# geloescht/mxnet-maintenance

Hardware: AMD Instinct MI355X
Metric: images/sec (whole node) ResNet-50 fp16 batch 256/GPU at 1/2/4/8 MI355X (higher is better)
Workload: dtype fp16; 1 GPU; model=ResNet-50 v1b, global_batch=256, per_gpu_batch=256, image_size=224, parallelism=dp1, layout=NHWC, optimizer=mp-SGD momentum 0.9, lr 0.1 (linear warm-up 40 steps), hip_graph=True, deterministic=True

## Files before the change

mxnet_maintenance_amd/_state.py:

```python
import threading


class _State(threading.local):
    def __init__(self):
        super().__init__()
        self.recording = False
        self.training = False
        self.np_shape = False
        self.np_array = False
        self.tape_leaves = {}


STATE = _State()

DIRECT_GRAD = [0]


def is_recording():
    return STATE.recording


def is_training():
    return STATE.training

GRAPH_RNG = [None]


GRAD_TOUCHED = set()
```

mxnet_maintenance_amd/autograd.py:

```python
from contextlib import contextmanager


import torch

from . import _state
from .base import MXNetError

__all__ = ['record', 'pause', 'train_mode', 'predict_mode', 'is_recording', 'is_training',
           'set_recording', 'set_training', 'mark_variables', 'backward', 'grad', 'Function',
           'get_symbol']


def set_recording(is_recording):
    prev = _state.STATE.recording
    _state.STATE.recording = bool(is_recording)
    return prev


def set_training(train_mode):
    prev = _state.STATE.training
    _state.STATE.training = bool(train_mode)
    return prev


# ... 105 lines not shown
            continue
        if not getattr(t, '_mxamd_touch_hook', False):
            _add_touch_hook(v, t)
        gbuf = v._grad._data
        if t.grad is not gbuf:
            t.grad = gbuf
        if v._grad_req == 'write':
            a = v._arena
            if a is not None and a.all_write:
                arenas.setdefault(id(a), (a, []))[1].append(gbuf)
            else:
                zero.append(gbuf)
    with torch.no_grad():
        for a, bufs in arenas.values():
            if len(bufs) == len(a.params):
                a.g.zero_()
            else:
                zero.extend(bufs)
        if zero:
            torch._foreach_zero_(zero)


def _finish_leaves(leaves):
    touched = _state.GRAD_TOUCHED
    for v in leaves:
        t = v._data
        if v._grad is None:
            continue
        g = t.grad
        if g is not None and g is not v._grad._data:
            v._grad._data = g
            t.grad = g
        if id(v) in touched or not getattr(t, '_mxamd_touch_hook', False):
            v._fresh_grad = True
        else:
            _state.STATE.tape_leaves.setdefault(id(v), v)
    touched.clear()


def _head_grad(g, t):
    if g.shape == t.shape:
        return g
    if g.numel() == t.numel() or (g.numel() > t.numel() and g.dim() == t.dim()
                                  and g.shape[1:] == t.shape[1:]):
        return g.reshape(-1)[:t.numel()].reshape(t.shape)
    try:
        return g.expand(t.shape)
    except RuntimeError:
        pass
    raise MXNetError(f'head gradient of shape {tuple(g.shape)} does not match output shape {tuple(t.shape)}')


def backward(heads, head_grads=None, retain_graph=False, train_mode=True, create_graph=False):
    from .ndarray.ndarray import NDArray
    if isinstance(heads, NDArray):
        heads = [heads]
    if head_grads is not None and isinstance(head_grads, NDArray):
        head_grads = [head_grads]
    tensors, grads = [], []
    for i, h in enumerate(heads):
        t = h._data
        if not t.requires_grad:
            continue
        tensors.append(t)
        hg = None if head_grads is None else head_grads[i]
        grads.append(torch.ones_like(t) if hg is None else _head_grad(hg._data.to(t.dtype), t))
    if not tensors and heads and all(getattr(h, '_recorded', False) for h in heads):
        _zero_marked_grads()
        return
    if not tensors:
        raise MXNetError('Cannot differentiate node because it is not in a computational graph. '
                         'You need to set is_recording to true or use autograd.record() to save '
                         'computational graphs for backward.')
    for h in heads:
        if getattr(getattr(h, '_data', None), _RELEASED_ATTR, False):
            raise MXNetError('Check failed: the graph of this output was already freed by a backward pass '
                             'without retain_graph=True; record it again or pass retain_graph=True')
    if not (retain_graph or create_graph):
        for h in heads:
            if getattr(h, '_data', None) is not None and h._data.grad_fn is not None:
                setattr(h._data, _RELEASED_ATTR, True)
    leaves = _collect_leaves(retain_graph)
    _prepare_leaves(leaves)
    prev_train = set_training(train_mode)
    prev_rec = set_recording(False)
    direct = not create_graph
    if direct:
        _state.DIRECT_GRAD[0] += 1
    try:
        with torch.enable_grad() if create_graph else torch.no_grad():
            torch.autograd.backward(tensors, grads, retain_graph=retain_graph or create_graph,
                                    create_graph=create_graph)
    finally:
        set_training(prev_train)
        set_recording(prev_rec)
        if direct:
            _state.DIRECT_GRAD[0] -= 1
    _finish_leaves(leaves)


def grad(heads, variables, head_grads=None, retain_graph=None, create_graph=False, train_mode=True):
    from .ndarray.ndarray import NDArray
    if isinstance(heads, NDArray):
        heads = [heads]
    if isinstance(variables, NDArray):
        variables = [variables]
    if head_grads is not None and isinstance(head_grads, NDArray):
        head_grads = [head_grads]
    hts = [h._data for h in heads]
    if head_grads is None:
        hgs = [torch.ones_like(h) for h in hts]
    else:
        hgs = [torch.ones_like(h) if g is None else g._data for h, g in zip(hts, head_grads)]
    if retain_graph is None:
        retain_graph = create_graph
    live = [(h, g) for h, g in zip(hts, hgs) if h.requires_grad]
    gs = [None] * len(variables)
    if live:
        prev_train = set_training(train_mode)
        prev_rec = set_recording(create_graph)
        try:
            with torch.enable_grad():
                gs = torch.autograd.grad([h for h, _ in live], [v._data for v in variables],
                                         grad_outputs=[g for _, g in live], retain_graph=retain_graph,
                                         create_graph=create_graph, allow_unused=True)
        finally:
            set_training(prev_train)
            set_recording(prev_rec)

    def dense(g, v):
        if g is None or g._is_zerotensor():
            return torch.zeros_like(v._data)
        return g
    return [NDArray(dense(g, v)) for g, v in zip(gs, variables)]


def get_symbol(x):
    sym = getattr(x, '_symbol', None)
    if isinstance(sym, tuple):
        block, i = sym
        return block._recorded_symbols()[i]
    if sym is not None:
        return sym
    if getattr(x, '_hist', None) is None:
        raise MXNetError('get_symbol: the array was not produced by a recorded operator')
    from .symbol.symbol import _op_func, var
    memo, nvars = {}, [0]

    def build(a):
        key = id(a)
        if key in memo:
            return memo[key]
        h = getattr(a, '_hist', None)
        if h is None:
            s = var('var%d' % nvars[0])
            nvars[0] += 1
        else:
            (opname, attrs, ins), i = h
            kw = {k: v for k, v in attrs.items() if v is not None}
            node = _op_func(opname)(*[build(b) for b in ins if b is not None], **kw)
            s = node[i] if len(node.list_outputs()) > 1 else node
        memo[key] = s
        return s
    return build(x)


# ... 57 lines not shown
```

mxnet_maintenance_amd/executor.py:

```python
import os

import numpy as np
import torch

from . import _state
from . import profiler as _profiler
from .ops import amp_dispatch as _amp
from .base import MXNetError, AsyncOpError
from .ops import registry


def _call_monitor(cb, name, arr):
    from .base import _HANDLES, NDArrayHandle
    key = id(arr)
    _HANDLES[key] = arr
    try:
        cb(name, NDArrayHandle(key))
    finally:
        _HANDLES.pop(key, None)


class GraphProgram:

    def __init__(self, sym):
        from .symbol.symbol import _aux_var_ids
        order = sym._topo()
        self.symbol = sym
        slot = {}
        nslots = 0
        self.var_names = []
        self.var_slots = []
        aux = _aux_var_ids(order)
        self.arg_names = []
        self.aux_names = []
        for n in order:
            if n.op is None:
                slot[(id(n), 0)] = nslots
                self.var_names.append(n.name)
                self.var_slots.append(nslots)
                (self.aux_names if id(n) in aux else self.arg_names).append(n.name)
                nslots += 1
        self.steps = []
        for n in order:
            if n.op is None:
                continue
            op = n.opdef()
            parsed = dict(n.parsed())
            k = op.get_num_outputs(parsed)
            outs = []
            for i in range(k):
                slot[(id(n), i)] = nslots
                outs.append(nslots)
                nslots += 1
            ins = [slot[(id(a), j)] for a, j in n.inputs]
            self.steps.append((op.fn, ins, parsed, outs, n.name, op.name))
        self.out_slots = [slot[(id(n), j)] for n, j in sym._outputs]
        self.nslots = nslots
        self._var_of_slot = {s: n for n, s in zip(self.var_names, self.var_slots)}
        self.name_to_slot = dict(zip(self.var_names, self.var_slots))

    _POSITIONAL_INPUTS = ('SoftmaxActivation', 'Activation')

    @staticmethod
    def _input_names(opname, attrs, n):
        op = registry.get(opname)
        if op.name in GraphProgram._POSITIONAL_INPUTS:
            return ['input%d' % j for j in range(n)]
        names = op.get_arg_names(attrs) + op.get_aux_names(attrs)
        return [names[j] if j < len(names) else 'input%d' % j for j in range(n)]

    def run(self, feed, monitor=None, monitor_all=False, record=None, int_dtypes=None):
        vals = [None] * self.nslots
        for name, s in self.name_to_slot.items():
            vals[s] = feed.get(name)
        islot = {}
        if int_dtypes:
            islot = {self.name_to_slot[n]: d for n, d in int_dtypes.items() if n in self.name_to_slot}
        self.failure = None
        sched = self._stream_sched(vals) if _GRAPH_STREAMS > 1 else None
        try:
            for si, (fn, ins, attrs, outs, name, opname) in enumerate(self.steps):
                args = [vals[i] for i in ins]
                if sched is not None:
                    sched.before(si, args)
                if _amp.active:
                    args = _amp.cast_inputs(opname, args, attrs)
                if record is not None:
                    record.append((name, args))
                if monitor is not None and monitor_all:
                    argn = self._input_names(opname, attrs, len(args))
                    for j, a in enumerate(args):
                        if a is None:
                            continue
                        var = self._var_of_slot.get(ins[j])
                        if var is not None:
                            monitor(var, a)
                        monitor('%s_%s' % (name, argn[j]), a)
                try:
                    if (islot and any(i in islot for i in ins)) or (attrs.get('dtype') is not None and
                                                                     _int_dtype_attr(attrs) and torch.is_grad_enabled()):
                        r = self._run_shadow(fn, args, attrs, ins, outs, islot, opname)
                    elif _profiler.active_symbolic:
                        with _profiler.op_span(_profiler.current_scope() + opname, symbolic=True):
                            r = fn(*args, **attrs)
                    else:
                        r = fn(*args, **attrs)
                except AsyncOpError as e:
                    from .ndarray.register import _placeholder
                    if self.failure is None:
                        self.failure = AsyncOpError('Error in operator %s (%s): %s' % (name, opname, e))
                    r = _placeholder(attrs, [])
                except MXNetError:
                    if self.failure is None:
                        raise
                    from .ndarray.register import _placeholder
                    r = _placeholder(attrs, [])
                except (RuntimeError, IndexError) as e:
                    if self.failure is not None:
                        from .ndarray.register import _placeholder
                        r = _placeholder(attrs, [])
                    else:
                        raise MXNetError('Error in operator %s (%s): %s' % (name, opname, e)) from e
                if sched is not None:
                    sched.after(si)
                if len(outs) == 1:
                    vals[outs[0]] = r[0] if isinstance(r, (tuple, list)) else r
                else:
                    for o, t in zip(outs, r):
                        vals[o] = t
                if monitor is not None:
                    op = registry.get(opname)
                    onames = op.output_names or (['output'] if len(outs) == 1 else
                                                 ['output%d' % k for k in range(len(outs))])
                    for o, on in zip(outs, onames):
                        if vals[o] is not None:
                            monitor('%s_%s' % (name, on), vals[o])
        finally:
            if sched is not None:
                torch.cuda.set_stream(sched.main)
        self.out_idts = [islot.get(s) for s in self.out_slots] if islot else None
        if sched is not None:
            sched.finish([vals[s] for s in self.out_slots])
        return [vals[s] for s in self.out_slots]

    def _stream_plan(self, nstreams):
        producer = {}
        for i, st in enumerate(self.steps):
            for o in st[3]:
                producer[o] = i
        n = len(self.steps)
        stream_of = [0] * n
        tail = [-1] * nstreams
        waits = [()] * n
        need_ev = set()
        rr = 1
        for i, (_fn, ins, _attrs, _outs, _name, opname) in enumerate(self.steps):
            prods = sorted({producer[x] for x in ins if x in producer})
            cands = prods or [-1]
            live = [stream_of[p] if p >= 0 else 0 for p in cands if tail[stream_of[p] if p >= 0 else 0] == p]
            choice = min(live) if live else None
            if choice is None:
                if opname in _BRANCH_OPS and nstreams > 1:
                    choice = rr
                    rr = 1 + rr % (nstreams - 1)
                else:
                    choice = stream_of[prods[-1]] if prods else 0
            stream_of[i] = choice
            tail[choice] = i
            w = tuple(p for p in prods if stream_of[p] != choice)
            waits[i] = w
            need_ev.update(w)
        return stream_of, waits, need_ev

    def _stream_sched(self, vals):
        dev = next((v.device for v in vals if isinstance(v, torch.Tensor) and v.is_cuda), None)
        if dev is None or torch.cuda.is_current_stream_capturing() and not _GRAPH_STREAMS_CAPTURE:
            return None
        plan = getattr(self, '_splan', None)
        if plan is None:
            plan = self._splan = self._stream_plan(_GRAPH_STREAMS)
        if max(plan[0], default=0) == 0:
            return None
        return _StreamSched(plan, dev)
    @staticmethod
    def _run_shadow(fn, args, attrs, ins, outs, islot, opname=None):
        from .ndarray.register import _merge_shadow, INT_ZERO_GRAD
        true_args = [a.detach().to(islot[i]) if (i in islot and a is not None) else a for a, i in zip(args, ins)]
        with torch.no_grad():
            res_t = fn(*true_args, **attrs)
        multi = isinstance(res_t, (tuple, list))
        if not torch.is_grad_enabled() or not any(a is not None and a.requires_grad for a in args) or \
                opname in INT_ZERO_GRAD:
            for o in outs:
                islot.pop(o, None)
            return res_t
        kw_f = dict(attrs, dtype='float64') if _int_dtype_attr(attrs) else attrs
        res_f = fn(*args, **kw_f)
        pairs = [_merge_shadow(f, t) for f, t in zip(res_f, res_t)] if multi else [_merge_shadow(res_f, res_t)]
        for o, (_, d) in zip(outs, pairs):
            if d is not None:
                islot[o] = d
            else:
                islot.pop(o, None)
        return [p[0] for p in pairs] if multi else pairs[0][0]


_GRAPH_STREAMS = int(os.environ.get('MXNET_GRAPH_STREAMS', '1') or 1)
_GRAPH_STREAMS_CAPTURE = os.environ.get('MXNET_GRAPH_STREAMS_CAPTURE', '0') == '1'
_BRANCH_OPS = frozenset(('Convolution', 'Deconvolution', 'FullyConnected', '_contrib_DeformableConvolution',
                         '_contrib_ModulatedDeformableConvolution', 'Pooling', 'dot', 'batch_dot', '_npi_matmul',
                         'RNN', '_FusedOp'))
_SIDE_STREAMS = {}


def _side_streams(dev, n):
    lst = _SIDE_STREAMS.get(dev)
    if lst is None or len(lst) < n:
        lst = _SIDE_STREAMS[dev] = [torch.cuda.Stream(device=dev) for _ in range(n)]
    return lst


class _StreamSched:
# ... 436 lines not shown
```

mxnet_maintenance_amd/gluon/model_zoo/vision/resnet.py:

```python
from ... import nn
from ...block import HybridBlock
from ...nn.basic_layers import _BatchNorm
from ....context import cpu

__all__ = ['ResNetV1', 'ResNetV2', 'BasicBlockV1', 'BasicBlockV2', 'BottleneckV1', 'BottleneckV2',
           'BottleneckV1b', 'resnet18_v1', 'resnet34_v1', 'resnet50_v1', 'resnet101_v1', 'resnet152_v1',
           'resnet18_v2', 'resnet34_v2', 'resnet50_v2', 'resnet101_v2', 'resnet152_v2', 'resnet50_v1b',
           'resnet101_v1b', 'resnet152_v1b', 'resnet18_v1b', 'resnet34_v1b', 'get_resnet']


def _bn_axis(layout):
    return 3 if layout == 'NHWC' else 1


def _conv(channels, k, stride, pad, in_channels, layout, use_bias=False):
    return nn.Conv2D(channels, kernel_size=k, strides=stride, padding=pad, use_bias=use_bias,
                     in_channels=in_channels, layout=layout)


def _bn(layout, relu=False, fuse=False, **kw):
    if relu and fuse:
        return nn.BatchNormReLU(axis=_bn_axis(layout), **kw)
    return nn.BatchNorm(axis=_bn_axis(layout), **kw)


class _StemBNReLUPool(nn.BatchNormReLU):

    def hybrid_forward(self, F, x, gamma, beta, running_mean, running_var):
        return F.contrib.BatchNormReLUMaxPool(x, gamma, beta, running_mean, running_var, name='fwd',
                                              kernel=(3, 3), stride=(2, 2), pad=(1, 1), **self._kwargs)


def _stem_tail(features, layout, fuse):
    if fuse and layout == 'NHWC':
        features.add(_StemBNReLUPool(axis=_bn_axis(layout)))
        return
    features.add(_bn(layout, True, fuse))
    if not fuse:
        features.add(nn.Activation('relu'))
    features.add(nn.MaxPool2D(3, 2, 1, layout=layout))


class _ResidualTail(_BatchNorm):

    def __init__(self, layout, fuse, **kwargs):
        super().__init__(axis=_bn_axis(layout), **kwargs)
        self._fuse_add = fuse

    def _alias(self):
        return 'batchnorm'

    def hybrid_forward(self, F, x, shortcut, gamma, beta, running_mean, running_var):
        if self._fuse_add:
            return F.contrib.BatchNormAddReLU(x, shortcut, gamma, beta, running_mean, running_var, name='fwd',
                                              **self._kwargs)
        return F.BatchNorm(x, gamma, beta, running_mean, running_var, name='fwd', **self._kwargs)


def _finish(F, tail, out, shortcut):
    y = tail(out, shortcut)
    return y if tail._fuse_add else F.Activation(y + shortcut, act_type='relu')


class BasicBlockV1(HybridBlock):

    def __init__(self, channels, stride, downsample=False, in_channels=0, layout='NCHW', fuse=False, **kwargs):
        super().__init__(**kwargs)
        self.body = nn.HybridSequential(prefix='')
        self.body.add(_conv(channels, 3, stride, 1, in_channels, layout),
                      _bn(layout, True, fuse))
        if not fuse:
            self.body.add(nn.Activation('relu'))
        self.body.add(_conv(channels, 3, 1, 1, channels, layout))
        self.tail = _ResidualTail(layout, fuse)
        self.downsample = None
        if downsample:
            self.downsample = nn.HybridSequential(prefix='')
            self.downsample.add(_conv(channels, 1, stride, 0, in_channels, layout), _bn(layout))

    def hybrid_forward(self, F, x):
        shortcut = self.downsample(x) if self.downsample is not None else x
        return _finish(F, self.tail, self.body(x), shortcut)


class BottleneckV1(HybridBlock):

    def __init__(self, channels, stride, downsample=False, in_channels=0, layout='NCHW', fuse=False,
                 stride_on_3x3=False, **kwargs):
        super().__init__(**kwargs)
        mid = channels // 4
        s1, s3 = (1, stride) if stride_on_3x3 else (stride, 1)
        self.body = nn.HybridSequential(prefix='')
        self.body.add(_conv(mid, 1, s1, 0, in_channels, layout), _bn(layout, True, fuse))
        if not fuse:
            self.body.add(nn.Activation('relu'))
        self.body.add(_conv(mid, 3, s3, 1, mid, layout), _bn(layout, True, fuse))
        if not fuse:
            self.body.add(nn.Activation('relu'))
        self.body.add(_conv(channels, 1, 1, 0, mid, layout))
        self.tail = _ResidualTail(layout, fuse)
        self.downsample = None
        if downsample:
            self.downsample = nn.HybridSequential(prefix='')
            self.downsample.add(_conv(channels, 1, stride, 0, in_channels, layout), _bn(layout))
        self._tee = fuse and s1 == 1 and layout == 'NHWC'
        if self._tee:
            self.body[0]._tee = True

    def hybrid_forward(self, F, x):
        if self._tee:
            blocks = list(self.body._children.values())
            out, passthrough = blocks[0](x)
            for b in blocks[1:]:
                out = b(out)
            shortcut = self.downsample(passthrough) if self.downsample is not None else passthrough
            return _finish(F, self.tail, out, shortcut)
        shortcut = self.downsample(x) if self.downsample is not None else x
        return _finish(F, self.tail, self.body(x), shortcut)


class BottleneckV1b(BottleneckV1):
    def __init__(self, channels, stride, downsample=False, in_channels=0, layout='NCHW', fuse=False, **kwargs):
        super().__init__(channels, stride, downsample, in_channels, layout, fuse, stride_on_3x3=True, **kwargs)


class BasicBlockV2(HybridBlock):

    def __init__(self, channels, stride, downsample=False, in_channels=0, layout='NCHW', fuse=False, **kwargs):
        super().__init__(**kwargs)
        self.bn1 = _bn(layout, True, fuse)
        self.conv1 = _conv(channels, 3, stride, 1, in_channels, layout)
        self.bn2 = _bn(layout, True, fuse)
        self.conv2 = _conv(channels, 3, 1, 1, channels, layout)
        self._fused = fuse
        self.downsample = _conv(channels, 1, stride, 0, in_channels, layout) if downsample else None

    def _act(self, F, x, bn):
        x = bn(x)
        return x if self._fused else F.Activation(x, act_type='relu')

    def hybrid_forward(self, F, x):
        shortcut = x
        x = self._act(F, x, self.bn1)
        if self.downsample is not None:
            shortcut = self.downsample(x)
        x = self.conv1(x)
        x = self.conv2(self._act(F, x, self.bn2))
        return x + shortcut


class BottleneckV2(HybridBlock):

    def __init__(self, channels, stride, downsample=False, in_channels=0, layout='NCHW', fuse=False, **kwargs):
        super().__init__(**kwargs)
        mid = channels // 4
        self.bn1 = _bn(layout, True, fuse)
        self.conv1 = _conv(mid, 1, 1, 0, 0, layout)
        self.bn2 = _bn(layout, True, fuse)
        self.conv2 = _conv(mid, 3, stride, 1, mid, layout)
        self.bn3 = _bn(layout, True, fuse)
        self.conv3 = _conv(channels, 1, 1, 0, 0, layout)
        self._fused = fuse
        self.downsample = _conv(channels, 1, stride, 0, in_channels, layout) if downsample else None

    def _act(self, F, x, bn):
        x = bn(x)
        return x if self._fused else F.Activation(x, act_type='relu')

    def hybrid_forward(self, F, x):
        shortcut = x
        x = self._act(F, x, self.bn1)
        if self.downsample is not None:
            shortcut = self.downsample(x)
        x = self.conv1(x)
        x = self.conv2(self._act(F, x, self.bn2))
        x = self.conv3(self._act(F, x, self.bn3))
        return x + shortcut


class _ResNetBase(HybridBlock):
    def _stage(self, block, n, channels, stride, index, in_channels, layout, fuse):
        stage = nn.HybridSequential(prefix='stage%d_' % index)
        with stage.name_scope():
            stage.add(block(channels, stride, channels != in_channels, in_channels=in_channels, layout=layout,
                            fuse=fuse, prefix=''))
            for _ in range(n - 1):
                stage.add(block(channels, 1, False, in_channels=channels, layout=layout, fuse=fuse, prefix=''))
        return stage


class ResNetV1(_ResNetBase):

    def __init__(self, block, layers, channels, classes=1000, thumbnail=False, layout='NCHW', fuse=False,
                 **kwargs):
        super().__init__(**kwargs)
        assert len(layers) == len(channels) - 1
        self._layout = layout
        with self.name_scope():
            self.features = nn.HybridSequential(prefix='')
            if thumbnail:
                self.features.add(_conv(channels[0], 3, 1, 1, 0, layout))
            else:
                self.features.add(_conv(channels[0], 7, 2, 3, 0, layout))
                _stem_tail(self.features, layout, fuse)
            for i, n in enumerate(layers):
                self.features.add(self._stage(block, n, channels[i + 1], 1 if i == 0 else 2, i + 1,
                                              channels[i], layout, fuse))
            self.features.add(nn.GlobalAvgPool2D(layout=layout))
            self.output = nn.Dense(classes, in_units=channels[-1])

    def hybrid_forward(self, F, x):
        return self.output(self.features(x))


class ResNetV2(_ResNetBase):

    def __init__(self, block, layers, channels, classes=1000, thumbnail=False, layout='NCHW', fuse=False,
                 **kwargs):
        super().__init__(**kwargs)
        assert len(layers) == len(channels) - 1
        with self.name_scope():
            self.features = nn.HybridSequential(prefix='')
            self.features.add(nn.BatchNorm(scale=False, center=False, axis=_bn_axis(layout)))
            if thumbnail:
                self.features.add(_conv(channels[0], 3, 1, 1, 0, layout))
            else:
                self.features.add(_conv(channels[0], 7, 2, 3, 0, layout))
                _stem_tail(self.features, layout, fuse)
            in_channels = channels[0]
            for i, n in enumerate(layers):
                self.features.add(self._stage(block, n, channels[i + 1], 1 if i == 0 else 2, i + 1,
                                              in_channels, layout, fuse))
                in_channels = channels[i + 1]
            self.features.add(_bn(layout, True, fuse))
            if not fuse:
                self.features.add(nn.Activation('relu'))
            self.features.add(nn.GlobalAvgPool2D(layout=layout))
            self.features.add(nn.Flatten())
            self.output = nn.Dense(classes, in_units=in_channels)

    def hybrid_forward(self, F, x):
        return self.output(self.features(x))


resnet_spec = {18: ('basic_block', [2, 2, 2, 2], [64, 64, 128, 256, 512]),
               34: ('basic_block', [3, 4, 6, 3], [64, 64, 128, 256, 512]),
               50: ('bottle_neck', [3, 4, 6, 3], [64, 256, 512, 1024, 2048]),
               101: ('bottle_neck', [3, 4, 23, 3], [64, 256, 512, 1024, 2048]),
               152: ('bottle_neck', [3, 8, 36, 3], [64, 256, 512, 1024, 2048])}
resnet_net_versions = [ResNetV1, ResNetV2]
resnet_block_versions = [{'basic_block': BasicBlockV1, 'bottle_neck': BottleneckV1},
                         {'basic_block': BasicBlockV2, 'bottle_neck': BottleneckV2}]


def get_resnet(version, num_layers, pretrained=False, ctx=cpu(), root='~/.mxnet/models', v1b=False, **kwargs):
    assert num_layers in resnet_spec, 'Invalid number of layers: %d. Options are %s' % (
        num_layers, str(resnet_spec.keys()))
    block_type, layers, channels = resnet_spec[num_layers]
    assert 1 <= version <= 2, 'Invalid resnet version: %d. Options are 1 and 2.' % version
    resnet_class = resnet_net_versions[version - 1]
    block_class = resnet_block_versions[version - 1][block_type]
    if v1b and block_type == 'bottle_neck':
        block_class = BottleneckV1b
    net = resnet_class(block_class, layers, channels, **kwargs)
    if pretrained:
        from ..model_store import get_model_file
        net.load_parameters(get_model_file('resnet%d_v%d' % (num_layers, version), root=root), ctx=ctx)
    return net


def resnet18_v1(**kwargs):
    return get_resnet(1, 18, **kwargs)


def resnet34_v1(**kwargs):
    return get_resnet(1, 34, **kwargs)


def resnet50_v1(**kwargs):
    return get_resnet(1, 50, **kwargs)


def resnet101_v1(**kwargs):
    return get_resnet(1, 101, **kwargs)


def resnet152_v1(**kwargs):
    return get_resnet(1, 152, **kwargs)


# ... 39 lines not shown
```

mxnet_maintenance_amd/ndarray/ndarray.py:

```python
import ctypes

import numpy as np
import torch

from .. import _state
from .. import engine as _engine
from ..base import (MXNetError, numeric_types, integer_types, torch_dtype, np_dtype,
                    dtype_name)
from ..context import Context, current_context, context_from_torch

def _shares_storage(a, b):
    try:
        return a.untyped_storage().data_ptr() == b.untyped_storage().data_ptr()
    except RuntimeError:
        return False


_STORAGE_TYPE_UNDEFINED = -1
_STORAGE_TYPE_DEFAULT = 0
_STORAGE_TYPE_ROW_SPARSE = 1
_STORAGE_TYPE_CSR = 2
_STORAGE_TYPE_STR_TO_ID = {'undefined': _STORAGE_TYPE_UNDEFINED, 'default': _STORAGE_TYPE_DEFAULT,
                           'row_sparse': _STORAGE_TYPE_ROW_SPARSE, 'csr': _STORAGE_TYPE_CSR}
_STORAGE_TYPE_ID_TO_STR = {v: k for k, v in _STORAGE_TYPE_STR_TO_ID.items()}
# ... 125 lines not shown
        shape_info = 'x'.join(str(x) for x in self.shape)
        return '\n%s\n<%s %s @%s>' % (str(self.asnumpy()), self.__class__.__name__, shape_info, self.context)

    def __str__(self):
        return self.__repr__()

    def __hash__(self):
        return id(self)

    def __bool__(self):
        n = self.size
        if n == 0:
            return False
        if n == 1:
            return bool(self._data.reshape(-1)[0].item())
        raise ValueError('The truth value of an NDArray with multiple elements is ambiguous.')

    __nonzero__ = __bool__

    def __float__(self):
        return float(self.asscalar())

    def __int__(self):
        return int(self.asscalar())

    def __index__(self):
        return int(self.asscalar())

    def __iter__(self):
        if self.ndim == 1:
            for i in range(self.shape[0]):
                yield self[i]
        else:
            box = getattr(self, '_exc', None)
            for i in range(self.shape[0]):
                v = NDArray(self._data[i])
                if box is not None:
                    v._exc = box
                yield v

    def __array__(self, dtype=None, copy=None):
        a = self.asnumpy()
        return a.astype(dtype) if dtype is not None else a

    def __getstate__(self):
        return {'data': self.asnumpy(), 'ctx': self.context}

    def __setstate__(self, state):
        if 'handle' in state:
            from .utils import _Reader, _read_array
            self._data = _read_array(_Reader(bytes(state['handle'])))._data
        else:
            self._data = torch.from_numpy(np.ascontiguousarray(state['data']))
        self._grad = None
        self._grad_req = None
        self._stype = 'default'
        self._fresh_grad = False
        self._arena = None

    def __reduce__(self):
        return (_rebuild, (self.asnumpy(),))

    def _rethrow(self):
        box = getattr(self, '_exc', None)
        if box is not None and box[0] is not None:
            from .. import engine
            engine.rethrow(box)

    def wait_to_read(self):
        _engine.join_workers()
        var = getattr(self, '_engine_var', None)
        if var is not None:
            from .. import engine
            engine.wait_for_var(var)
        if self._data.is_cuda:
            torch.cuda.current_stream(self._data.device).synchronize()
        self._rethrow()

    wait_to_write = wait_to_read

    def asnumpy(self):
        _engine.join_workers()
        self._rethrow()
        t = self._data.detach()
        idt = getattr(self, '_idt', None)
        if idt is not None:
            t = t.to(idt)
        if t.dtype == torch.bfloat16:
            t = t.float()
        return t.cpu().numpy().copy() if t.device.type == 'cpu' else t.cpu().numpy()

    def asscalar(self):
        if self.size != 1:
            raise ValueError('The current array is not a scalar')
        return self.asnumpy().reshape(-1)[0]

    def item(self):
        return self.asscalar()

    def tolist(self):
        return self.asnumpy().tolist()

    def astype(self, dtype, copy=True):
        td = torch_dtype(dtype)
        if not copy and td == self._data.dtype:
            return self
        return _invoke_unary(lambda t: t.to(td) if t.dtype != td else t.clone(), self)

    def copy(self):
        if self._stype != 'default' and type(self) is NDArray:
            from . import sparse
            cls = sparse.RowSparseNDArray if self._stype == 'row_sparse' else sparse.CSRNDArray
            return _tag_host_ctx(cls(self._data.detach().clone()), getattr(self, '_host_ctx', None))
        return _invoke_unary(lambda t: t.clone(), self)

    def __copy__(self):
        return self.copy()

    def __deepcopy__(self, memo):
        return NDArray(self._data.detach().clone())

    def copyto(self, other):
        _engine.join_workers()
        if isinstance(other, NDArray):
            if other is self:
                return other
            src = self._data.detach() if not _state.STATE.recording else self._data
            if other.shape != self.shape:
                raise MXNetError('copyto: shape mismatch %s vs %s' % (self.shape, other.shape))
            if _engine_copy(src, other._data.device) and other._data.is_contiguous() \
                    and other._data.dtype == src.dtype:
                from .. import engine
                _, other._engine_var = engine.host_to_device(src, other._data.device, out=other._data,
                                                             var=getattr(other, '_engine_var', None), name='copyto')
            else:
                with torch.no_grad():
                    other._data.copy_(src)
            _share_failure(self, other)
            return other
        if isinstance(other, Context):
            if _engine_copy(self._data, other.torch_device):
                return _share_failure(self, _async_upload(self._data, other))
            return _share_failure(self, _tag_host_ctx(NDArray(self._data.to(other.torch_device, copy=True)), other))
        raise TypeError('copyto does not support type ' + str(type(other)))

    def as_in_context(self, context):
        if self.context == context:
            return self
        _engine.join_workers()
        if context.device_typeid == 3:
            t = self._data.detach().cpu()
            if torch.cuda.is_available():
                return NDArray(t.pin_memory())
            out = NDArray(t.clone() if t.data_ptr() == self._data.data_ptr() else t)
            out._host_ctx = context
            return out
        if _engine_copy(self._data, context.torch_device):
            return _share_failure(self, _async_upload(self._data, context))
        return _tag_host_ctx(_invoke_unary(lambda t: t.to(context.torch_device), self), context)

    as_in_ctx = as_in_context

    def to_device(self, device):
        return self.as_in_context(device)

    def detach(self):
# ... 850 lines not shown
```

mxnet_maintenance_amd/ndarray/register.py:

```python
import contextlib

import sys

import torch

from .. import _state
from .. import engine as _engine
from .. import profiler as _profiler
from ..ops import amp_dispatch as _amp
from ..base import MXNetError, AsyncOpError
from ..ops import registry
from .ndarray import NDArray

_SKIP_KW = ('name', 'attr', 'out')
_NULL_CTX = contextlib.nullcontext()
_NP_CLS = [None]


def _np_wrap(inputs, outs):
    cls = _NP_CLS[0]
    if cls is None:
        return outs
    has_inputs = any(x is not None for x in inputs)
    if (_state.STATE.np_array and not has_inputs) or any(x is not None and x.__class__ is cls for x in inputs):
# ... 72 lines not shown

def _failed_input(inputs):
    for x in inputs:
        box = getattr(x, '_exc', None) if x is not None else None
        if box is not None and box[0] is not None:
            return box
    return None


_SAMPLER_NAMES = frozenset(('_npi_normal', '_npi_uniform', '_npi_gamma', '_npi_exponential', '_npi_multinomial',
                            '_shuffle', '_npi_bernoulli', '_npi_sampler', '_npi_uniform_like', '_npi_normal_like',
                            '_npi_choice', '_npi_shuffle', '_npi_laplace', '_npi_logistic', '_npi_gumbel',
                            '_npi_pareto', '_npi_power', '_npi_rayleigh', '_npi_weibull', '_npi_chisquare',
                            '_npi_f', '_npi_beta', '_npi_lognormal', '_npi_poisson'))


def _is_sampler(name):
    return name.startswith(('_random_', '_sample_', '_npi_random', 'random_', 'sample_')) or name in _SAMPLER_NAMES


def _placeholder(attrs, inputs):
    from ..base import torch_dtype
    shape = attrs.get('shape') or attrs.get('size') or (1,)
    shape = (shape,) if isinstance(shape, int) else tuple(shape)
    dt = attrs.get('dtype')
    try:
        td = torch_dtype(dt if dt not in (None, 'None') else 'float32')
    except Exception:
        td = torch.float32
    ctx = attrs.get('ctx')
    dev = getattr(ctx, 'torch_device', None)
    if dev is None:
        dev = next((x._data.device for x in inputs if x is not None), torch.device('cpu'))
    return torch.zeros(shape, dtype=td, device=dev)


def _int_dtype_attr(attrs):
    dt = attrs.get('dtype')
    return dt is not None and str(dt).replace('torch.', '').startswith(('int', 'uint', 'bool'))


def _shadowed(arrays, attrs=None):
    if any(x is not None and getattr(x, '_idt', None) is not None for x in arrays):
        return True
    return attrs is not None and _state.STATE.recording and _int_dtype_attr(attrs) and \
        any(x is not None and x._data.requires_grad for x in arrays)


def _true_inputs(arrays):
    return [None if x is None else (x._data.detach().to(x._idt) if getattr(x, '_idt', None) is not None
                                    else x._data) for x in arrays]


def _merge_shadow(res_f, res_t):
    if not isinstance(res_f, torch.Tensor) or not res_f.requires_grad or not res_f.is_floating_point():
        return res_t, None
    if res_t.is_floating_point() or res_t.is_complex():
        return res_f.to(res_t.dtype) + (res_t - res_f.to(res_t.dtype)).detach(), None
    return res_f + (res_t.to(res_f.dtype) - res_f).detach(), res_t.dtype


INT_ZERO_GRAD = frozenset(('_npi_mod', '_npi_mod_scalar', '_npi_fmod', '_npi_fmod_scalar', '_mod', 'broadcast_mod',
                           '_mod_scalar', '_rmod_scalar'))


def _run_shadow(fn, inputs, kw, opname=None):
    with torch.no_grad():
        res_t = fn(*_true_inputs(inputs), **kw)
    if not _state.STATE.recording or opname in INT_ZERO_GRAD:
        return res_t, None
    kw_f = kw
    if _int_dtype_attr(kw):
        kw_f = dict(kw, dtype='float64')
    res_f = _run(fn, [None if x is None else x._data for x in inputs], kw_f)
    if isinstance(res_t, (tuple, list)):
        pairs = [_merge_shadow(f, t) for f, t in zip(res_f, res_t)]
        return type(res_t)(p[0] for p in pairs), [p[1] for p in pairs]
    r, idt = _merge_shadow(res_f, res_t)
    return r, idt


def invoke(op, inputs, attrs, out=None):
    tin = [None if x is None else x._data for x in inputs]
    if _engine._JOIN_HOOKS and not _engine._workers.depth:
        _engine.run_join_hooks()
    _note_leaves(inputs)
    if _amp.active:
        tin = _amp.cast_inputs(op.name, tin, attrs)
    if op.name in _BN_OPS:
        _check_storage(op.name, [getattr(x, 'stype', 'default') for x in inputs], attrs)
    box = _failed_input(inputs)
    sampler = _is_sampler(op.name)
    if sampler and box is None:
        from .. import engine
        box = engine.rng_failure()
    idts = None
    ws_sid = ws_stream = None
    sctx = _NULL_CTX
    if _engine.GPU_WORKERS > 1 and not _engine._workers.depth:
        ws_sid, ws_stream = _engine.op_stream(tin)
        if ws_stream is not None:
            sctx = torch.cuda.stream(ws_stream)
            _engine._workers.depth += 1
    try:
        with sctx:
            if _shadowed(inputs, attrs) and not _amp.active:
                res, idts = _run_shadow(op.fn, inputs, attrs, op.name)
            elif _profiler.active_imperative:
                with _profiler.op_span(_profiler.current_scope() + op.name):
                    res = _run(op.fn, tin, attrs)
            else:
                res = _run(op.fn, tin, attrs)
    except AsyncOpError as e:
        from .. import engine
        if box is None:
            box = engine.record_failure(e)
        if sampler:
            engine.set_rng_failure(box)
        res = _placeholder(attrs, inputs)
    except MXNetError:
        if box is None:
            raise
        res = _placeholder(attrs, inputs)
    except (RuntimeError, IndexError) as e:
        if isinstance(e, IndexError):
            from ..base import MXNetIndexError
            raise MXNetIndexError('Error in operator %s: %s' % (op.name, e)) from e
        raise MXNetError('Error in operator %s: %s' % (op.name, e)) from e
    finally:
        if ws_stream is not None:
            _engine._workers.depth -= 1
            if sys.exc_info()[0] is not None:
                _engine._workers.pending.pop()
    nvis = op.get_num_visible_outputs(attrs)
    if isinstance(res, (tuple, list)):
        outs = [NDArray(r) for r in res[:nvis]]
    else:
        outs = [NDArray(res)]
    if ws_sid is not None:
        _engine.op_done([o._data for o in outs], ws_sid)
    st = _kept_stype(op.name, inputs, attrs) if out is None else None
    if st is not None and not _state.STATE.recording:
        from . import sparse
        outs = [sparse.cast_storage(o, st) for o in outs]
    _np_wrap(inputs, outs)
    if idts is not None:
        for o, d in zip(outs, idts if isinstance(idts, list) else [idts]):
            if d is not None:
                o._idt = d
    if _state.STATE.recording:
        hist = (op.name, attrs, list(inputs))
        for i, o in enumerate(outs):
            o._recorded = True
            o._hist = (hist, i)
    if _profiler.active_memory and out is None:
        for o in outs:
            _profiler.memory_alloc(o)
    if box is not None:
        for o in outs:
            o._exc = box
    hctx = attrs.get('ctx') if 'ctx' in attrs else next(
        (x._host_ctx for x in inputs if x is not None and getattr(x, '_host_ctx', None) is not None), None)
    if hctx is not None:
        from .ndarray import _tag_host_ctx
        for o in outs:
            _tag_host_ctx(o, hctx)
# ... 101 lines not shown
```

mxnet_maintenance_amd/ops/hip_ops.py:

```python
import os

import torch
import torch.nn.functional as F

from ..base import MXNetError
from . import kernels as _K

_ALLOW_FALLBACK = os.environ.get('MXAMD_ALLOW_TORCH_FALLBACK', '0') == '1'


def _acc(t):
    return t if t.dtype == torch.float64 else t.float()


def _use_hip(t):
    if not t.is_cuda:
        return False
    if _K.available():
        return _K.enabled()
    if _ALLOW_FALLBACK:
        return False
    raise MXNetError('HIP kernel extension not loaded on a GPU device: %s' % _K.load_error())


def _nd_to_ncx(x):
    nd = x.dim()
    return x.permute(0, nd - 1, *range(1, nd - 1))


def _ncx_to_nd(x):
    nd = x.dim()
    return x.permute(0, *range(2, nd), 1)



def linear(data, weight, bias):
    if _use_hip(data) and _K.gemm_ok(data, weight):
        return _K.Linear.apply(data, weight, bias)
    if data.dim() == 2:
        return F.linear(data, weight, bias)
    return F.linear(data, weight, bias)


def embedding(data, weight):
    if _use_hip(weight) and _K.embedding_ok(data, weight):
        return _K.Embedding.apply(data, weight)
    return None


def _as_nhwc_view(t):
    v = t.permute(0, 2, 3, 1)
    return v if v.is_contiguous() else v.contiguous()


def _nchw_on_hip(data):
    return (data.dim() == 4 and data.dtype in (torch.float16, torch.bfloat16) and _use_hip(data)
            and _NCHW_VIA_NHWC)


_NCHW_VIA_NHWC = os.environ.get('MXAMD_NCHW_VIA_NHWC', '1') == '1'


def _nhwc_weight(w):
    if w.shape[2] == 1 and w.shape[3] == 1 and w.is_contiguous():
        return w.view(w.shape[0], 1, 1, w.shape[1])
    return w.permute(0, 2, 3, 1).contiguous()


def conv(data, weight, bias, stride, pad, dilate, groups, channel_last):
    nsp = data.dim() - 2
    if groups > 1 and nsp == 2 and _use_hip(data):
        from .conv_dw import dw_ok, ConvDwNHWC
        xl = data if channel_last else (_as_nhwc_view(data) if _nchw_on_hip(data) else None)
        if xl is not None and dw_ok(xl, weight, groups, dilate):
            rs = tuple(weight.shape[1:3]) if channel_last else tuple(weight.shape[2:4])
            y = ConvDwNHWC.apply(xl, weight, bias, rs, tuple(stride), tuple(pad), tuple(dilate))
            return y if channel_last else y.permute(0, 3, 1, 2)
    if not channel_last and nsp == 2 and _nchw_on_hip(data):
        xl = _as_nhwc_view(data)
        wl = _nhwc_weight(weight)
        if _K.conv_ok(xl, wl, stride, pad, dilate, groups):
            if _K.kpad_ok(xl, wl):
                return _K.conv_kpad(xl, wl, bias, stride, pad, dilate).permute(0, 3, 1, 2)
            return _K.ConvNHWC.apply(xl, wl, bias, tuple(stride), tuple(pad), tuple(dilate)).permute(0, 3, 1, 2)
    if channel_last and _use_hip(data) and _K.conv_ok(data, weight, stride, pad, dilate, groups):
        if _K.kpad_ok(data, weight):
            return _K.conv_kpad(data, weight, bias, stride, pad, dilate)
        return _K.ConvNHWC.apply(data, weight, bias, tuple(stride), tuple(pad), tuple(dilate))
    if nsp == 2 and groups == 1 and _use_hip(data) and tuple(dilate) != (1, 1):
        xl = data if channel_last else (_as_nhwc_view(data) if _nchw_on_hip(data) else None)
        if xl is not None:
            wl = weight if channel_last else _nhwc_weight(weight)
            if _K.dil_ok(xl, wl, dilate):
                y = _K.ConvDilNHWC.apply(xl, wl, bias, tuple(stride), tuple(pad), tuple(dilate))
                return y if channel_last else y.permute(0, 3, 1, 2)
    if _use_hip(data):
        from . import conv_gen
        y = conv_gen.conv(data, weight, bias, tuple(stride), tuple(pad), tuple(dilate), groups, channel_last)
        if y is not None:
            return y
    if channel_last:
        x = _nd_to_ncx(data)
        w = _nd_to_ncx(weight)
    else:
        x, w = data, weight
    fn = {1: F.conv1d, 2: F.conv2d, 3: F.conv3d}[nsp]
    y = fn(x, w, bias, stride=stride, padding=pad, dilation=dilate, groups=groups)
    return _ncx_to_nd(y) if channel_last else y


def conv_tee(data, weight, inplace_grad=False):
    if _use_hip(data) and hasattr(_K, 'ConvTeeNHWC') and _K.conv_tee_ok(data, weight):
        return _K.ConvTeeNHWC.apply(data, weight, bool(inplace_grad))
    return conv(data, weight, None, (1, 1), (0, 0), (1, 1), 1, True), data



def batch_norm_relu_maxpool(data, gamma, beta, moving_mean, moving_var, eps, momentum, fix_gamma, training,
                            axis, kernel, stride, pad, invstd_out=False):
    nd = data.dim()
    if (nd == 4 and axis % nd == 3 and _use_hip(data) and _K.bnrelu_pool_ok(data, kernel, stride, pad)):
        g = torch.ones_like(gamma) if fix_gamma else gamma
        return _K.BatchNormNHWC.apply(data, g, beta, None, eps, training, True, moving_mean, moving_var, momentum,
                                      invstd_out, (tuple(kernel), tuple(stride), tuple(pad)))
    out, m, v = batch_norm(data, gamma, beta, moving_mean, moving_var, eps, momentum, fix_gamma, training, axis,
                           'relu', invstd_out=invstd_out)
    return pool(out, 'max', tuple(kernel), tuple(stride), tuple(pad), 'valid', True, axis % nd == nd - 1), m, v


def batch_norm(data, gamma, beta, moving_mean, moving_var, eps, momentum, fix_gamma, training,
               axis, act_type, addend=None, invstd_out=False):
    nd = data.dim()
    axis = axis % nd
    channel_last = (axis == nd - 1) and nd > 2
    g = torch.ones_like(gamma) if fix_gamma else gamma
    if axis == 1 and _nchw_on_hip(data) and data.permute(0, 2, 3, 1).is_contiguous():
        xl = data.permute(0, 2, 3, 1)
        al = _as_nhwc_view(addend) if addend is not None else None
        if _K.bn_ok(xl):
            out, m, v = _K.BatchNormNHWC.apply(xl, g, beta, al, eps, training, act_type == 'relu',
                                                moving_mean, moving_var, momentum, invstd_out)
            return out.permute(0, 3, 1, 2), m, v
    if channel_last and _use_hip(data) and _K.bn_ok(data):
        return _K.BatchNormNHWC.apply(data, g, beta, addend, eps, training, act_type == 'relu',
                                      moving_mean, moving_var, momentum, invstd_out)
    if channel_last:
        x = _nd_to_ncx(data)
    elif axis != 1:
        others = [i for i in range(nd) if i != axis]
        perm = [others[0], axis] + others[1:]
        x = data.permute(*perm)
    else:
        x = data
    if training:
        out, smean, sinvstd = torch.ops.aten.native_batch_norm(x, g, beta, None, None, True, 0.0, eps)
        with torch.no_grad():
            var = (1.0 / (sinvstd.float() ** 2) - eps).clamp_(min=0.0) if sinvstd.numel() else sinvstd
            moving_mean.mul_(momentum).add_(smean.detach().to(moving_mean.dtype), alpha=1 - momentum)
            moving_var.mul_(momentum).add_(var.to(moving_var.dtype), alpha=1 - momentum)
        mean_out, var_out = smean, (sinvstd if invstd_out else var)
    else:
        out = F.batch_norm(x, moving_mean, moving_var, g, beta, False, 0.0, eps)
        mean_out, var_out = moving_mean, moving_var
    if channel_last:
        out = _ncx_to_nd(out)
    elif axis != 1:
        inv = [0] * nd
        others = [i for i in range(nd) if i != axis]
        perm = [others[0], axis] + others[1:]
        for i, p in enumerate(perm):
            inv[p] = i
        out = out.permute(*inv)
    if addend is not None:
        out = out + addend
    if act_type == 'relu':
        out = torch.relu(out)
    return out, mean_out, var_out



def global_pool(data, pool_type, channel_last):
    nsp = data.dim() - 2
    if not channel_last and pool_type == 'avg' and _nchw_on_hip(data) and data.permute(0, 2, 3, 1).is_contiguous():
        xl = data.permute(0, 2, 3, 1)
        if _K.gap_ok(xl):
            return _K.GlobalAvgPoolNHWC.apply(xl).permute(0, 3, 1, 2)
    if channel_last:
        if _use_hip(data) and nsp == 2 and pool_type == 'avg' and _K.gap_ok(data):
            return _K.GlobalAvgPoolNHWC.apply(data)
        dims = tuple(range(1, 1 + nsp))
    else:
        dims = tuple(range(2, 2 + nsp))
    if pool_type == 'max':
        return torch.amax(data, dim=dims, keepdim=True)
    if pool_type == 'sum':
        return torch.sum(data, dim=dims, keepdim=True)
    if pool_type == 'lp':
        return torch.sqrt(torch.sum(data * data, dim=dims, keepdim=True))
    return torch.mean(data, dim=dims, keepdim=True)


def _pool_out(n, k, s, p, conv):
    if conv == 'full':
        return int(-(-(n + 2 * p - k) // s)) + 1
    return (n + 2 * p - k) // s + 1


def pool(data, pool_type, kernel, stride, pad, convention, count_include_pad, channel_last, p_value=None):
    nsp = data.dim() - 2
    if not channel_last and nsp == 2 and pool_type in ('max', 'avg') and convention != 'same' \
            and _nchw_on_hip(data) and data.permute(0, 2, 3, 1).is_contiguous():
        xl = data.permute(0, 2, 3, 1)
        if _K.pool_ok(xl, kernel, stride, pad):
            return _K.PoolNHWC.apply(xl, pool_type, tuple(kernel), tuple(stride), tuple(pad),
                                     convention == 'full', bool(count_include_pad)).permute(0, 3, 1, 2)
    if channel_last and _use_hip(data) and nsp == 2 and pool_type in ('max', 'avg') \
            and _K.pool_ok(data, kernel, stride, pad):
        return _K.PoolNHWC.apply(data, pool_type, tuple(kernel), tuple(stride), tuple(pad),
                                 convention == 'full', bool(count_include_pad))
    x = _nd_to_ncx(data) if channel_last else data
    if channel_last and x.is_cuda and pool_type != 'max':
        x = x.contiguous()
    ceil = convention == 'full'
    pad_r = list(pad)
    if convention == 'same':
        ceil = False
        for i in range(nsp):
            n = x.shape[2 + i]
# ... 93 lines not shown
```

mxnet_maintenance_amd/ops/kernel_fns.py:

```python
import os

import torch

from . import kernels as _K
from .. import _state
from ..utils import env as _env

__all__ = ['BatchNormNHWC', 'SoftmaxCE', 'GlobalAvgPoolNHWC', 'flat_sgd']

_DT = {torch.float32: 0, torch.float16: 1, torch.bfloat16: 2}


def _stream():
    return torch.cuda.current_stream().cuda_stream


def _p(t):
    return 0 if t is None else t.data_ptr()


def _f32(t):
    if t.dtype == torch.float32 and t.is_contiguous():
        return t
    m = getattr(t, '_mxamd_master', None)
    if m is not None and m[1] == t._version and m[0].shape == t.shape:
        return m[0]
    return t.float().contiguous()



def bn_ok(x):
    C = x.shape[-1] if x.dim() else 0
    return (x.dtype in _DT and x.dim() >= 2 and x.is_contiguous() and C % 8 == 0
            and x.numel() > 0 and x.data_ptr() % 16 == 0)


def ce_ok(x):
    return x.dim() == 2 and x.dtype in _DT and x.is_contiguous()




def _leaf_grad(t, numel=None, dtype=torch.float32):
    if t is None or _state.DIRECT_GRAD[0] <= 0 or torch.is_grad_enabled() or not t.is_leaf or not t.requires_grad:
        return None
    gb = t.grad
    if gb is None or gb.dtype != dtype or not gb.is_contiguous() or gb.shape != t.shape:
        return None
    if numel is not None and gb.numel() != numel:
        return None
    return gb


_RELU_FROM_X = [True]
_BN_BWD_FUSE = [os.environ.get('MXAMD_BN_BWD_FUSE', '1') != '0']
_BN_TAIL_DS = [os.environ.get('MXAMD_BN_TAIL_DS', '1') != '0']
_BN_POOL_BWD = [True]
_ZEROS = {}


def _zeros_f32(n, dev):
    z = _ZEROS.get((n, dev))
    if z is None:
        z = _ZEROS[(n, dev)] = torch.zeros(n, dtype=torch.float32, device=dev)
    return z


class _BnToken:
    __slots__ = ('lazy',)

    def __init__(self):
        self.lazy = None


class BatchNormNHWC(torch.autograd.Function):

    @staticmethod
    def forward(ctx, x, gamma, beta, addend, eps, training, relu, moving_mean, moving_var, momentum=None,
                invstd_out=False, pool=None):
        lib = _K.lib()
        C = x.shape[-1]
        R = x.numel() // C
        dev = x.device
        g = _f32(gamma)
        b = _f32(beta)
        mm = _f32(moving_mean)
        assert pool is None or (relu and addend is None)
        y = torch.empty_like(x) if pool is None else None
        if addend is not None:
            assert addend.shape == x.shape and addend.dtype == x.dtype
            addend = addend.contiguous()
        ext_nblk = 0
        center = mm
        if training:
            ext = getattr(x, '_mxamd_bn_part', None)
            if ext is not None and ext[0].numel() == 2 * C * ext[1] and ext[0].device == dev:
                part, ext_nblk = ext
                center = _zeros_f32(C, dev)
            else:
                nblk = lib.bn_partials_rows(R, C)
                part = torch.empty(2 * nblk * C, dtype=torch.float32, device=dev)
            stats = torch.empty(5, C, dtype=torch.float32, device=dev)
            mean, invstd, var, scale, shift = stats.unbind(0)
        else:
            part = None
            mean = mm
            invstd = torch.rsqrt(_f32(moving_var) + eps)
            var = _f32(moving_var)
            scale = g * invstd
            shift = b - mean * scale
        upd = (training and momentum is not None and mm is moving_mean and moving_var.dtype == torch.float32
               and moving_var.is_contiguous())
        mask = (torch.empty(x.numel() // 8, dtype=torch.uint8, device=dev)
                if (addend is not None and relu and _RELU_FROM_X[0]) else None)
        lib.bn_nhwc_forward(_DT[x.dtype], x.data_ptr(), _p(addend), _p(y), _p(mask), g.data_ptr(),
                            b.data_ptr(),
                            center.data_ptr(), _p(part), mean.data_ptr(), invstd.data_ptr(), var.data_ptr(),
                            scale.data_ptr(), shift.data_ptr(), R, C, float(eps), int(bool(training)),
                            int(bool(relu)), 0, float(momentum or 0.0), moving_mean.data_ptr() if upd else 0,
                            moving_var.data_ptr() if upd else 0, int(ext_nblk), _stream())
        if training and momentum is not None and not upd:
            with torch.no_grad():
                moving_mean.mul_(momentum).add_(mean.to(moving_mean.dtype), alpha=1 - momentum)
                moving_var.mul_(momentum).add_(var.to(moving_var.dtype), alpha=1 - momentum)
        ctx.pool = None
        if pool is not None:
            (kh, kw), (sh, sw), (ph, pw) = pool
            N, H, W = x.shape[:3]
            Ho, Wo = _pool_out(H, kh, sh, ph, False), _pool_out(W, kw, sw, pw, False)
            y = torch.empty((N, Ho, Wo, C), dtype=x.dtype, device=dev)
            arg = torch.empty((N, Ho, Wo, C), dtype=torch.uint8, device=dev)
            ctx.pool = (N, H, W, C, Ho, Wo, kh, kw, sh, sw, ph, pw, 1)
            lib.pool_nhwc_forward_bnrelu(_DT[x.dtype], x.data_ptr(), y.data_ptr(), arg.data_ptr(), *ctx.pool,
                                         _stream(), scale.data_ptr(), shift.data_ptr())
            mask = arg
        relu_mode = 0 if not relu else (1 if not _RELU_FROM_X[0] else (3 if addend is not None else 2))
        if pool is not None:
            relu_mode = 2
        ctx.save_for_backward(x, y if relu_mode == 1 else mask, g, mean, invstd,
                              scale if relu_mode == 2 else None, shift if relu_mode == 2 else None)
        ctx.cfg = (relu_mode, bool(training), addend is not None, gamma.dtype, beta.dtype)
        ctx.tee_key = getattr(addend, '_mxamd_tee_key', None) if (addend is not None and relu_mode == 3) else None
        ctx.bn_token = None
        if training and relu_mode in (0, 2, 3) and _BN_BWD_FUSE[0] and pool is None:
            ctx.bn_token = _BnToken()
            y._mxamd_bn_src = (x, mean, scale if relu_mode == 2 else None, shift if relu_mode == 2 else None,
                               mask if relu_mode == 3 else None, relu_mode, ctx.bn_token)
        ctx.refs = (gamma, beta)
        ctx.add_src = None
        if relu_mode == 3 and training and _BN_BWD_FUSE[0] and _BN_TAIL_DS[0]:
            src = getattr(addend, '_mxamd_bn_src', None)
            if (src is not None and src[5] == 0 and tuple(src[0].shape) == tuple(x.shape)
                    and src[0].dtype == x.dtype and src[0].is_contiguous()):
                ctx.add_src = src
        third = invstd if (invstd_out and training) else var
        ctx.mark_non_differentiable(mean, third)
        ctx.set_materialize_grads(False)
        return y, mean, third

    @staticmethod
    def backward(ctx, gy, _gm, _gv):
        lib = _K.lib()
        x, y, g, mean, invstd, fscale, fshift = ctx.saved_tensors
        relu_mode, training, has_add, gdt, bdt = ctx.cfg
        gamma_ref, beta_ref = ctx.refs
        if gy is None:
            return (None,) * 12
        gy = gy.contiguous()
        C = x.shape[-1]
        R = x.numel() // C
        dev = x.device
        fused_pool = False
        if ctx.pool is not None:
            fused_pool = (x.dtype in (torch.float16, torch.bfloat16) and 256 % (C // 8) == 0
                          and hasattr(lib, 'bn_pool_backward') and _BN_POOL_BWD[0])
            if not fused_pool:
                gyd = torch.empty_like(x)
                lib.pool_nhwc_backward(_DT[x.dtype], 1, gy.data_ptr(), y.data_ptr(), gyd.data_ptr(), *ctx.pool,
                                       _stream())
                gy, y = gyd, None
        lazy_mask = None
        tok = ctx.bn_token
        if tok is not None and tok.lazy is not None:
            dy_l, mask_l, ver_l = tok.lazy
            tok.lazy = None
            if gy is dy_l and gy._version == ver_l and relu_mode == 0 and not has_add and ctx.pool is None:
                lazy_mask = mask_l
            else:
                gy = (gy - dy_l + _materialize_dz(dy_l, mask_l)).contiguous()
        dx = torch.empty_like(x)
        dz = torch.empty_like(x) if has_add else None
        ext = getattr(gy, '_mxamd_bn_bwd', None)
        ext_nblk = 0
        if (ext is not None and ctx.bn_token is not None and ext[2] is ctx.bn_token
                and ext[3] == gy._version):
            part, ext_nblk = ext[0], ext[1]
        else:
            nblk = lib.bn_partials_rows(R, C)
            part = torch.empty(2 * nblk * C, dtype=torch.float32, device=dev)
        out = torch.empty(5, C, dtype=torch.float32, device=dev)
        need_g, need_b = ctx.needs_input_grad[1], ctx.needs_input_grad[2]
        tg = _leaf_grad(gamma_ref, C) if need_g else None
        tb = _leaf_grad(beta_ref, C) if need_b else None
        direct = tb is not None and (tg is not None or not need_g) and (tg is not None or tb is not None)
        if direct:
            dg_buf = tg if tg is not None else torch.zeros(C, dtype=torch.float32, device=dev)
            dg_ptr, db_ptr, accum = dg_buf.data_ptr(), tb.data_ptr(), 1
        else:
            dg_ptr, db_ptr, accum = out[0].data_ptr(), out[1].data_ptr(), 0
        if fused_pool:
            N_, H_, W_, C_, Ho_, Wo_, kh, kw, sh, sw, ph, pw, _ = ctx.pool
            ppart = torch.empty(2 * lib.bn_pool_bwd_blocks() * C, dtype=torch.float32, device=dev)
            lib.bn_pool_backward(_DT[x.dtype], x.data_ptr(), gy.data_ptr(), y.data_ptr(), dx.data_ptr(), g.data_ptr(),
                                 mean.data_ptr(), invstd.data_ptr(), fscale.data_ptr(), fshift.data_ptr(),
                                 ppart.data_ptr(), dg_ptr, db_ptr, out[2].data_ptr(), N_, H_, W_, C_, Ho_, Wo_, kh, kw,
                                 sh, sw, ph, pw, 0, int(training), accum, _stream())
            if direct:
                return dx, None, None, None, None, None, None, None, None, None, None, None
            return (dx, out[0].to(gdt) if need_g else None, out[1].to(bdt) if need_b else None,
                    None, None, None, None, None, None, None, None, None)
        ymask = y if relu_mode == 3 else None
        y = y if relu_mode == 1 else None
        ds = ctx.add_src if dz is not None else None
        lazy = (dz is not None and ds is None and ymask is not None and ctx.tee_key is not None
                and lazy_shortcut_ok(ctx.tee_key))
        lazy_ds = (dz is not None and ds is not None and ymask is not None and _LAZY_DZ[0]
                   and isinstance(ds[6], _BnToken))
        if lazy or lazy_ds:
            dz = None
        kmode = relu_mode
        if lazy_mask is not None:
            kmode, ymask = 3, lazy_mask
        dkw = {}
        if ds is not None:
            ds_nblk = lib.bn_tail_ds_rows(R, C)
            ds_part = torch.empty(2 * ds_nblk * C, dtype=torch.float32, device=dev)
            dkw = dict(ds_z=ds[0].data_ptr(), ds_mean=ds[1].data_ptr(), ds_part=ds_part.data_ptr())
        lib.bn_nhwc_backward(_DT[x.dtype], x.data_ptr(), gy.data_ptr(), _p(y), _p(ymask), dx.data_ptr(), _p(dz),
                             g.data_ptr(),
                             mean.data_ptr(), invstd.data_ptr(), _p(fscale), _p(fshift), part.data_ptr(), dg_ptr,
                             db_ptr, out[2].data_ptr(), R, C, kmode, 0, int(training), accum, _stream(),
                             ext_nblk, **dkw)
        if ds is not None:
            if lazy_ds:
                gy._mxamd_bn_bwd = (ds_part, ds_nblk, ds[6], gy._version)
                ds[6].lazy = (gy, ymask, gy._version)
                dz = gy
            else:
                dz._mxamd_bn_bwd = (ds_part, ds_nblk, ds[6], dz._version)
        if lazy:
            gy._mxamd_lazy_mask = (ymask, gy._version)
            dz = gy
        if direct:
            dgamma = None
            dbeta = None
        else:
            dgamma = out[0].to(gdt) if need_g else None
            dbeta = out[1].to(bdt) if need_b else None
        return dx, dgamma, dbeta, dz, None, None, None, None, None, None, None, None


def bnrelu_pool_ok(x, kernel, stride, pad):
    return (bn_ok(x) and tuple(kernel) == (3, 3) and pool_ok(x, kernel, stride, pad)
            and x.numel() + 256 * 32 * 256 * 8 < 2 ** 31 and hasattr(_K.lib(), 'pool_nhwc_forward_bnrelu'))


class SoftmaxCE(torch.autograd.Function):

    @staticmethod
    def forward(ctx, logits, label):
        lib = _K.lib()
        N, K = logits.shape
        lab = label.reshape(-1)
        is_int = not lab.is_floating_point()
        lab = lab.to(torch.int64).contiguous() if is_int else lab.float().contiguous()
        loss = torch.empty(N, dtype=torch.float32, device=logits.device)
        lse = torch.empty(N, dtype=torch.float32, device=logits.device)
        lib.softmax_ce_forward(_DT[logits.dtype], int(is_int), logits.data_ptr(), lab.data_ptr(), loss.data_ptr(),
                               lse.data_ptr(), N, K, _stream())
        ctx.save_for_backward(logits, lab, lse)
        ctx.is_int = is_int
        return loss

    @staticmethod
    def backward(ctx, gout):
        lib = _K.lib()
        logits, lab, lse = ctx.saved_tensors
        N, K = logits.shape
        g = gout.float().contiguous()
        dl = torch.empty_like(logits)
        lib.softmax_ce_backward(_DT[logits.dtype], int(ctx.is_int), logits.data_ptr(), lab.data_ptr(),
                                lse.data_ptr(), g.data_ptr(), dl.data_ptr(), N, K, _stream())
        return dl, None


class GlobalAvgPoolNHWC(torch.autograd.Function):
    @staticmethod
    def forward(ctx, x):
        lib = _K.lib()
        x = x.contiguous()
        N, C = x.shape[0], x.shape[-1]
        HW = x.numel() // (N * C)
        y = torch.empty((N,) + (1,) * (x.dim() - 2) + (C,), dtype=x.dtype, device=x.device)
        lib.gap_nhwc_forward(_DT[x.dtype], x.data_ptr(), y.data_ptr(), N, HW, C, _stream())
        ctx.shape = x.shape
        return y

    @staticmethod
    def backward(ctx, gy):
        lib = _K.lib()
        shape = ctx.shape
        N, C = shape[0], shape[-1]
        HW = int(torch.tensor(shape[1:-1]).prod())
        gy = gy.contiguous()
        dx = torch.empty(shape, dtype=gy.dtype, device=gy.device)
        lib.gap_nhwc_backward(_DT[gy.dtype], gy.data_ptr(), dx.data_ptr(), N, HW, C, _stream())
        return dx


def gap_ok(x):
    return x.dtype in _DT and x.is_contiguous() and x.shape[-1] % 8 == 0


class ReluHip(torch.autograd.Function):

    @staticmethod
    def forward(ctx, x):
        x = x.contiguous()
        y = torch.empty_like(x)
        _K.lib().relu_forward(_DT[x.dtype], x.data_ptr(), y.data_ptr(), x.numel(), _stream())
        ctx.save_for_backward(y)
        return y

    @staticmethod
    def backward(ctx, gy):
        y, = ctx.saved_tensors
        gy = gy.contiguous()
        dx = torch.empty_like(y)
        _K.lib().relu_backward(_DT[y.dtype], y.data_ptr(), gy.data_ptr(), dx.data_ptr(), y.numel(), _stream())
        return dx


# ... 622 lines not shown

_FILE_ALGO = {}
_FILE_STATE = {'loaded': False}


def _tuning_file():
    return os.environ.get('MXAMD_AUTOTUNE_FILE', '')


def _load_tuning_file():
    if _FILE_STATE['loaded']:
        return
    _FILE_STATE['loaded'] = True
    path = _tuning_file()
    if path and os.path.exists(path):
        import json
        try:
            with open(path) as f:
                _FILE_ALGO.update(json.load(f))
        except (OSError, ValueError):
            pass


def _save_tuning_file(key, name):
    path = _tuning_file()
    if not path or name is None:
        return
    from ..parallel import dist
    if dist.rank() != 0:
        return
    import json
    _FILE_ALGO[repr(key)] = name
    tmp = path + '.tmp'
    try:
        with open(tmp, 'w') as f:
            json.dump(_FILE_ALGO, f, indent=0, sort_keys=True)
        os.replace(tmp, path)
    except OSError:
        pass


def _select(key, cands, default, timing=None):
    key = _akey(key)
    cands = _det_filter(cands)
    timing = _det_filter(timing)
    _load_tuning_file()
    name = _ALGO.get(key)
    if name is None:
        name = _FILE_ALGO.get(repr(key))
        if name is not None and name in dict(cands):
            _ALGO[key] = name
    if name is None:
        if _AUTOTUNE and not torch.cuda.is_current_stream_capturing() and len(cands) > 1:
            name, out = _time_candidates(timing or cands, key=key)
            _ALGO[key] = name
            _save_tuning_file(key, name)
            return out
        name = default
    table = dict(cands)
    return (table[name] if name in table else cands[0][1])()


_NCU = {}


def _num_cus(dev):
    n = _NCU.get(dev)
    if n is None:
        n = _NCU[dev] = torch.cuda.get_device_properties(dev).multi_processor_count
    return n


def pw_ok(x, kin, nout):
    return (_CONV_HIP and x.is_cuda and x.dtype in (torch.float16, torch.bfloat16) and x.is_contiguous()
            and x.data_ptr() % 16 == 0 and hasattr(_K.lib(), 'conv_pw_stream')
            and bool(_K.lib().conv_pw_stream_ok(int(kin), int(nout))))


def pw_bnb_ok(kin, nout, add, bn_src):
    return (bn_src is not None and int(bn_src[5]) in (2, 3) and hasattr(_K.lib(), 'conv_pw_stream_bnb_ok')
            and bool(_K.lib().conv_pw_stream_bnb_ok(int(kin), int(nout), int(bool(add)), int(bn_src[5]))))


def conv_pw(x, w2, bn_stats=False, addend=None, bn_bwd=None, addend_mask=None):
    C = x.shape[-1]
    K = w2.shape[0]
    M = x.numel() // C
    wt = int(w2.dim() == 2 and w2.stride() == (1, K) and not w2.is_contiguous() and w2.data_ptr() % 16 == 0
             and K % 8 == 0)
    if not wt:
        w2 = w2.contiguous()
    y = torch.empty(x.shape[:-1] + (K,), dtype=x.dtype, device=x.device)
    if addend is not None:
        addend = addend.contiguous()
        if tuple(addend.shape) != tuple(y.shape) or addend.dtype != y.dtype or addend.data_ptr() % 16:
            raise ValueError('conv_pw: addend must match the output (shape, dtype, 16-byte alignment)')
    lib = _K.lib()
    grid = lib.conv_pw_stream_grid(M, C, K, _num_cus(x.device), int(addend is not None or bn_bwd is not None))
    nparts = grid // max(1, lib.conv_pw_stream_slices(C, K))
    part = torch.empty(2 * K * nparts, dtype=torch.float32, device=x.device) if (bn_stats or bn_bwd) else None
    bkw = {}
    if bn_bwd is not None:
        assert not bn_stats, 'conv_pw: forward and backward statistics are exclusive'
        z, bmean, bscale, bshift, bmask, bmode, _token = bn_bwd
        assert z.shape == y.shape and z.dtype == y.dtype and z.is_contiguous() and z.data_ptr() % 16 == 0
        bkw = dict(bn_z=z.data_ptr(), bn_mask=_p(bmask), bn_mean=bmean.data_ptr(), bn_scale=_p(bscale),
                   bn_shift=_p(bshift), bn_mode=int(bmode))
    if addend_mask is not None:
        assert bn_bwd is not None and addend is not None and addend_mask.dtype == torch.uint8
        assert addend_mask.numel() * 8 == addend.numel() and addend_mask.is_contiguous()
        bkw['addend_mask'] = addend_mask.data_ptr()
    lib.conv_pw_stream(_DT[x.dtype], x.data_ptr(), w2.data_ptr(), y.data_ptr(), _zero_page(x.device).data_ptr(), M, C,
                       K, _p(part), grid, _stream(), _p(addend), wt, **bkw)
    if bn_bwd is not None:
        y._mxamd_bn_bwd = (part, nparts, bn_bwd[6], y._version)
    elif part is not None:
        y._mxamd_bn_part = (part, nparts)
    return y


def _fwd_candidates(x, w, stride, pad, bias):
    c = []
    K, R, S, C = w.shape
    if (R == 1 and S == 1 and tuple(stride) == (1, 1) and tuple(pad) == (0, 0) and bias is None
            and pw_ok(x, C, K)):
        c.append(('pw', lambda: conv_pw(x, w.reshape(K, C), bn_stats=bool(_state.STATE.training))))
    if stem_ok(x, w, stride, pad, bias):
        c.append(('stem', lambda: conv_stem_fwd(x, w, pad, bn_stats=bool(_state.STATE.training))))
    if bias is None and halo_ok(x, w, stride, pad):
        c.append(('halo', lambda: conv_halo(x, w, bn_stats=bool(_state.STATE.training))))
    if conv_ok_shape(x, w, stride, pad):
        c.append(('hip', lambda: conv_fwd(x, w, stride, pad, bias)))
        stats = bool(_state.STATE.training)
        for v in _fwd_variants(C, K, bias is not None, ktot=R * S * C):
            c.append(('hip%d' % v, lambda v=v: conv_fwd(x, w, stride, pad, bias, v, bn_stats=stats)))
    if R == 1 and S == 1 and tuple(stride) == (1, 1) and tuple(pad) == (0, 0):
        x2, w2 = x.reshape(-1, C), w.reshape(K, C)
        for name, fn in _gemm().candidates(x2, w2, bias=bias):
            c.append((name, lambda fn=fn: fn().view(x.shape[0], x.shape[1], x.shape[2], K)))

        def mm():
            y = torch.mm(x.reshape(-1, C), w.reshape(K, C).t())
            if bias is not None:
                y = y + bias.to(y.dtype)
            return y.view(x.shape[0], x.shape[1], x.shape[2], K)
        c.append(('mm', mm))

    def miopen():
        y = torch.nn.functional.conv2d(x.permute(0, 3, 1, 2), w.permute(0, 3, 1, 2), bias, tuple(stride), tuple(pad))
        return y.permute(0, 2, 3, 1).contiguous()
    c.append(('miopen', miopen))
    return c


_STATS_SCRATCH = {}


def _bn_stats_pass(y):
    C = y.shape[-1]
    R = y.numel() // C
    lib = _K.lib()
    n = 2 * lib.bn_partials_rows(R, C) * C
    buf = _STATS_SCRATCH.get(y.device)
    if buf is None or buf.numel() < n:
        buf = _STATS_SCRATCH[y.device] = torch.empty(n, dtype=torch.float32, device=y.device)
    lib.bn_nhwc_stats(_DT[y.dtype], y.data_ptr(), _zeros_f32(C, y.device).data_ptr(), buf.data_ptr(), R, C,
                      _stream())


def _fwd_timing(cands):
    if not _state.STATE.training:
        return None

    def charged(fn):
        def run():
            y = fn()
            if getattr(y, '_mxamd_bn_part', None) is None and y.shape[-1] % 8 == 0 and y.is_contiguous():
                _bn_stats_pass(y)
            return y
        return run
    return [(n, charged(fn)) for n, fn in cands]


def _fwd_default(x, w, stride):
    K, R, S, C = w.shape
    if C <= 4 and K == 64 and tuple(stride) == (2, 2) and R <= 8 and S <= 8:
        return 'stem'
    if R == 1 and S == 1 and tuple(stride) == (1, 1) and (K >= 256 or x.shape[1] * x.shape[2] <= 784):
        return 'mm'
    return 'hip'


def _dgrad_candidates(dy, x, w, stride, pad):
    c = []
# ... 150 lines not shown


def _bmm_f32(a, b):
    if _BMM_OUT_DTYPE[0] is not False:
        try:
            r = torch.bmm(a, b, out_dtype=torch.float32)
            _BMM_OUT_DTYPE[0] = True
            return r
        except (RuntimeError, TypeError):
            _BMM_OUT_DTYPE[0] = False
    return torch.bmm(a, b).float()


def _wgrad(dy, x, w, w_ref, stride, pad):
    key = ('wgrad', tuple(x.shape), tuple(w.shape), tuple(stride), tuple(pad), x.dtype)
    algo = _ALGO.get(_akey(key))
    if algo == 'stem':
        tgt = _leaf_grad(w_ref, dtype=w.dtype)
        if tgt is not None:
            conv_stem_wgrad(x, dy, w.shape, pad, out=tgt, accum=True)
            return None
    if algo in ('hip', 'hipreg') or (algo or '').startswith('ring'):
        tgt = _leaf_grad(w_ref, dtype=w.dtype)
        if tgt is not None:
            conv_wgrad(x, dy, w.shape, stride, pad, out=tgt, accum=True, dma=algo == 'hip',
                       ring=int(algo[4:]) if algo.startswith('ring') else 0)
            return None
    elif algo is not None and algo.startswith('splitk'):
        tgt = _leaf_grad(w_ref, dtype=w.dtype)
        if tgt is not None:
            _splitk_wgrad(dy, x, int(algo[6:]), out=tgt)
            return None
    default = 'stem' if stem_ok(x, w, stride, pad) else ('hip' if conv_wgrad_ok(x, w) else 'miopen')
    dw = _select(key, _wgrad_candidates(dy, x, w, stride, pad), default)
    if dw.dtype != w.dtype:
        tgt = _leaf_grad(w_ref, dtype=w.dtype)
        if tgt is not None:
            tgt.add_(dw)
            return None
        dw = dw.to(w.dtype)
    return dw


_WGRAD_SIDE = [os.environ.get('MXAMD_WGRAD_STREAM', '0') == '1']
_SIDE_STREAMS = {}
_SIDE_KEEP = []
_SIDE_DIRTY = set()


def join_side_streams():
    if not _SIDE_DIRTY:
        return
    for dev in list(_SIDE_DIRTY):
        torch.cuda.current_stream(dev).wait_stream(_SIDE_STREAMS[dev])
    _SIDE_DIRTY.clear()
    del _SIDE_KEEP[:]


def _wgrad_maybe_side(dy, x, w, w_ref, stride, pad):
    if not (_WGRAD_SIDE[0] and dy.is_cuda):
        return _wgrad(dy, x, w, w_ref, stride, pad)
    dev = dy.device.index
    side = _SIDE_STREAMS.get(dev)
    if side is None:
        side = _SIDE_STREAMS[dev] = torch.cuda.Stream(device=dev)
        from .. import engine
        engine.add_join_hook(join_side_streams)
    main = torch.cuda.current_stream(dev)
    side.wait_stream(main)
    with torch.cuda.stream(side):
        dw = _wgrad(dy, x, w, w_ref, stride, pad)
    _SIDE_KEEP.append((dy, x))
    _SIDE_DIRTY.add(dev)
    if dw is not None:
        main.wait_stream(side)
        dw.record_stream(main)
    return dw


class ConvNHWC(torch.autograd.Function):

    @staticmethod
    def forward(ctx, x, w, bias, stride, pad, dilate):
        key = ('fwd', tuple(x.shape), tuple(w.shape), tuple(stride), tuple(pad), x.dtype, bias is not None)
        cands = _fwd_candidates(x, w, stride, pad, bias)
        y = _select(key, cands, _fwd_default(x, w, stride), timing=_fwd_timing(cands))
        ctx.save_for_backward(x, w)
        ctx.stride, ctx.pad = stride, pad
        ctx.has_bias = bias is not None
        ctx.b_ref = bias
        ctx.w_ref = w
        ctx.bn_src = getattr(x, '_mxamd_bn_src', None)
        return y

    @staticmethod
    def backward(ctx, dy):
        x, w = ctx.saved_tensors
        dy = dy.contiguous()
        stride, pad = ctx.stride, ctx.pad
        dx = dw = db = None
        if ctx.needs_input_grad[1] and _WGRAD_SIDE[0]:
            dw = _wgrad_maybe_side(dy, x, w, ctx.w_ref, stride, pad)
        if ctx.needs_input_grad[0]:
            key = ('dgrad', tuple(x.shape), tuple(w.shape), tuple(stride), tuple(pad), x.dtype)
            if _bn_bwd_fusable(ctx.bn_src, x.shape):
                cands, timing = _dgrad_bn_candidates(dy, x, w, stride, pad, ctx.bn_src)
                dx = _select(key + ('bnbwd',), cands, _dgrad_default(w, stride), timing=timing)
            else:
                dx = _select(key, _dgrad_candidates(dy, x, w, stride, pad), _dgrad_default(w, stride))
        if ctx.needs_input_grad[1] and not _WGRAD_SIDE[0]:
            dw = _wgrad(dy, x, w, ctx.w_ref, stride, pad)
        if ctx.has_bias and ctx.needs_input_grad[2]:
            db = _conv_bias_grad(dy, ctx.b_ref)
        return dx, dw, db, None, None, None


def _conv_bias_grad(dy, b_ref):
    from .nlp_fns import bias_grad
    return bias_grad(dy.reshape(-1, dy.shape[-1]), b_ref, b_ref.dtype)


class ConvTeeNHWC(torch.autograd.Function):

    @staticmethod
    def forward(ctx, x, w, inplace_grad=False):
        stride, pad = (1, 1), (0, 0)
        key = ('fwd', tuple(x.shape), tuple(w.shape), stride, pad, x.dtype, False)
        cands = _fwd_candidates(x, w, stride, pad, None)
        y = _select(key, cands, _fwd_default(x, w, stride), timing=_fwd_timing(cands))
        ctx.save_for_backward(x, w)
        ctx.w_ref = w
        ctx.inplace_grad = inplace_grad
        ctx.bn_src = getattr(x, '_mxamd_bn_src', None)
        xp = x.view_as(x)
        xp._mxamd_tee_key = _tee_key(x, w, ctx.bn_src)
        return y, xp

    @staticmethod
    def backward(ctx, gy, gpass):
        x, w = ctx.saved_tensors
        K, C = w.shape[0], w.shape[3]
        dx = dw = None
        if gy is None:
            return gpass, None, None
        gy = gy.contiguous()
        if ctx.needs_input_grad[1] and _WGRAD_SIDE[0]:
            dw = _wgrad_maybe_side(gy, x, w, ctx.w_ref, (1, 1), (0, 0))
        if ctx.needs_input_grad[0]:
            dx = _tee_dgrad(gy, x, w, gpass, ctx.inplace_grad, ctx.bn_src)
        if ctx.needs_input_grad[1] and not _WGRAD_SIDE[0]:
            dw = _wgrad(gy, x, w, ctx.w_ref, (1, 1), (0, 0))
        return dx, dw, None


def _tee_key(x, w, bn_src):
    return ('teedgrad', tuple(x.shape), tuple(w.shape), x.dtype) + (('bnbwd',) if _bn_bwd_fusable(bn_src, x.shape)
                                                                     else ())


_LAZY_DZ = [os.environ.get('MXAMD_LAZY_SHORTCUT_GRAD', '1') != '0']
_LAZY_USED = [0]


def lazy_shortcut_ok(tee_key):
    return _LAZY_DZ[0] and tee_key is not None and _ALGO.get(_akey(tee_key)) == 'pw+bn'


def _unpack_lazy_dz(gpass):
    lz = getattr(gpass, '_mxamd_lazy_mask', None) if gpass is not None else None
    if lz is None or lz[1] != gpass._version:
        return None
    return lz[0]


def _materialize_dz(gpass, mask):
    bits = (mask.view(-1, 1) >> torch.arange(8, device=mask.device, dtype=torch.uint8)) & 1
    return gpass * bits.view(gpass.shape).to(gpass.dtype)


def _tee_dgrad(gy, x, w, gpass, inplace, bn_src=None):
    K, C = w.shape[0], w.shape[3]
    g2 = gy.reshape(-1, K)
    w2 = w.reshape(K, C)
    amask = _unpack_lazy_dz(gpass)
    if amask is not None:
        key = _tee_key(x, w, bn_src)
        if (_ALGO.get(_akey(key)) == 'pw+bn' and _bn_bwd_fusable(bn_src, x.shape) and pw_ok(gy, K, C)
                and pw_bnb_ok(K, C, True, bn_src) and gpass.is_contiguous() and gpass.data_ptr() % 16 == 0):
            _LAZY_USED[0] += 1
            return conv_pw(gy, w2.t(), addend=gpass, bn_bwd=bn_src, addend_mask=amask)
        gpass, inplace = _materialize_dz(gpass, amask), True

    def mm():
        if gpass is not None and inplace and gpass.is_contiguous():
            return gpass.view(-1, C).addmm_(g2, w2).view(x.shape)
        if gpass is not None:
            return torch.addmm(gpass.contiguous().reshape(-1, C), g2, w2).view(x.shape)
        return torch.mm(g2, w2).view(x.shape)

    cands = []
    fused = []
    fuse_bn = _bn_bwd_fusable(bn_src, x.shape)
    if _CONV_HIP and K % 64 == 0 and gy.dtype in (torch.float16, torch.bfloat16) and gy.numel() < 2 ** 31:
        wt = None
        for v, (bco, _bpix) in sorted(_BIG_VARIANTS.items()):
            if C % bco or (v in _BIG_SKINNY and not (_SKINNY_ON and K == 64)):
                continue
            if wt is None:
                wt = _dgrad_weight(w.contiguous())

            def big(v=v, wt=wt, bn=None):
                add = gpass.contiguous() if gpass is not None else None
# ... 173 lines not shown
```

mxnet_maintenance_amd/ops/nn.py:

```python
import math
import os

import torch
import torch.nn.functional as F

from .. import _state
from ..base import torch_dtype, MXNetError
from .registry import register
from . import hip_ops



def _acc(t):
    return t if t.dtype == torch.float64 else t.float()


def _is_channel_last(layout):
    return layout is not None and layout.endswith('C') and len(layout) > 2


def _to_ncx(x, layout):
    if _is_channel_last(layout):
        nd = x.dim()
        return x.permute(0, nd - 1, *range(1, nd - 1))
# ... 134 lines not shown
    pad = list(_tup(pad, nsp, 0))
    adj = list(_tup(adj, nsp, 0))
    x = _to_ncx(data, layout)
    w = _to_ncx(weight, layout)
    if target_shape:
        for i in range(nsp):
            full = (x.shape[2 + i] - 1) * stride[i] + dilate[i] * (kernel[i] - 1) + 1
            tot = full - target_shape[i]
            pad[i] = (tot + 1) // 2
            adj[i] = tot % 2
    if data.is_cuda and hip_ops._use_hip(data):
        from . import conv_gen
        y = conv_gen.deconv(data, weight, bias, stride, pad, dilate, adj, num_group, _is_channel_last(layout))
        if y is not None:
            return y
    fn = {1: F.conv_transpose1d, 2: F.conv_transpose2d, 3: F.conv_transpose3d}[nsp]
    y = fn(x, w, bias, stride=stride, padding=pad, output_padding=adj, groups=num_group, dilation=dilate)
    return _from_ncx(y, layout)



def _bn_infer(in_shapes, a):
    d = in_shapes[0]
    if d is None:
        return {}
    c = d[a.get('axis', 1) % len(d)]
    return {1: (c,), 2: (c,), 3: (c,), 4: (c,)}


_BN_PARAMS = {'eps': ('float', 1e-3), 'momentum': ('float', 0.9), 'fix_gamma': ('bool', True),
              'use_global_stats': ('bool', False), 'output_mean_var': ('bool', False),
              'axis': ('int', 1), 'cudnn_off': ('bool', False), 'act_type': ('str?', None),
              'min_calib_range': ('float?', None), 'max_calib_range': ('float?', None)}


def _bn_nvis(a):
    o = a.get('output_mean_var', False)
    o = o if isinstance(o, bool) else str(o) in ('True', 'true', '1')
    return 3 if o else 1


@register('BatchNorm', aliases=('BatchNorm_v1', 'CuDNNBatchNorm'),
          arg_names=('data', 'gamma', 'beta'), aux_names=('moving_mean', 'moving_var'),
          num_outputs=3, num_visible_outputs=_bn_nvis, infer_params=_bn_infer, params=_BN_PARAMS,
          output_names=('output', 'mean', 'var'))
def batch_norm(data, gamma, beta, moving_mean, moving_var, eps=1e-3, momentum=0.9, fix_gamma=True,
               use_global_stats=False, output_mean_var=False, axis=1, cudnn_off=False, act_type=None,
               min_calib_range=None, max_calib_range=None):
    training = _state.STATE.training and not use_global_stats
    return hip_ops.batch_norm(data, gamma, beta, moving_mean, moving_var, eps, momentum, fix_gamma,
                              training, axis, act_type, invstd_out=True)


@register('_contrib_BatchNormWithReLU', aliases=('BatchNormWithReLU',),
          arg_names=('data', 'gamma', 'beta'), aux_names=('moving_mean', 'moving_var'),
          num_outputs=3, num_visible_outputs=_bn_nvis, infer_params=_bn_infer, params=_BN_PARAMS)
def batch_norm_relu(data, gamma, beta, moving_mean, moving_var, eps=1e-3, momentum=0.9, fix_gamma=True,
                    use_global_stats=False, output_mean_var=False, axis=1, cudnn_off=False, act_type=None,
                    min_calib_range=None, max_calib_range=None):
    training = _state.STATE.training and not use_global_stats
    return hip_ops.batch_norm(data, gamma, beta, moving_mean, moving_var, eps, momentum, fix_gamma,
                              training, axis, 'relu', invstd_out=True)


_BNPOOL_PARAMS = dict(_BN_PARAMS, kernel=('shape', (3, 3)), stride=('shape', (2, 2)), pad=('shape', (1, 1)))


@register('_contrib_BatchNormReLUMaxPool', aliases=('BatchNormReLUMaxPool',),
          arg_names=('data', 'gamma', 'beta'), aux_names=('moving_mean', 'moving_var'),
          num_outputs=3, num_visible_outputs=_bn_nvis, infer_params=_bn_infer, params=_BNPOOL_PARAMS)
def batch_norm_relu_maxpool(data, gamma, beta, moving_mean, moving_var, eps=1e-3, momentum=0.9, fix_gamma=True,
                            use_global_stats=False, output_mean_var=False, axis=1, cudnn_off=False, act_type=None,
                            min_calib_range=None, max_calib_range=None, kernel=(3, 3), stride=(2, 2), pad=(1, 1)):
    training = _state.STATE.training and not use_global_stats
    return hip_ops.batch_norm_relu_maxpool(data, gamma, beta, moving_mean, moving_var, eps, momentum, fix_gamma,
                                           training, axis, _tup(kernel, 2, 1), _tup(stride, 2, 1), _tup(pad, 2, 0),
                                           invstd_out=True)


@register('_contrib_BatchNormAddReLU', aliases=('BatchNormAddReLU',),
          arg_names=('data', 'addend', 'gamma', 'beta'), aux_names=('moving_mean', 'moving_var'),
          num_outputs=3, num_visible_outputs=_bn_nvis,
          infer_params=lambda s, a: {k + 1: v for k, v in _bn_infer(s, a).items() if k + 1 <= 5 and k > 0},
          params=_BN_PARAMS)
def batch_norm_add_relu(data, addend, gamma, beta, moving_mean, moving_var, eps=1e-3, momentum=0.9,
                        fix_gamma=True, use_global_stats=False, output_mean_var=False, axis=1,
                        cudnn_off=False, act_type=None, min_calib_range=None, max_calib_range=None):
    training = _state.STATE.training and not use_global_stats
    return hip_ops.batch_norm(data, gamma, beta, moving_mean, moving_var, eps, momentum, fix_gamma,
                              training, axis, 'relu', addend=addend)



_POOL_PARAMS = {'kernel': ('shape', ()), 'pool_type': ('str', 'max'), 'global_pool': ('bool', False),
                'cudnn_off': ('bool', False), 'pooling_convention': ('str', 'valid'),
                'stride': ('shape', ()), 'pad': ('shape', ()), 'p_value': ('int?', None),
                'count_include_pad': ('bool?', None), 'layout': ('str?', None)}


@register('Pooling', aliases=('Pooling_v1',), params=_POOL_PARAMS)
def pooling(data, kernel=(), pool_type='max', global_pool=False, cudnn_off=False,
            pooling_convention='valid', stride=(), pad=(), p_value=None, count_include_pad=None,
            layout=None):
    nsp = data.dim() - 2
    if count_include_pad is None:
        count_include_pad = True
    if global_pool:
        return hip_ops.global_pool(data, pool_type, _is_channel_last(layout))
    kernel = _tup(kernel, nsp, 1)
    stride = _tup(stride, nsp, 1)
    if pooling_convention == 'same':
        if any(int(p) != 0 for p in (pad or ())):
            raise MXNetError('Pooling: pad must be 0 with pooling_convention=same, got %s' % (tuple(pad),))
        pad = (0,) * nsp
    pad = _tup(pad, nsp, 0)
    return hip_ops.pool(data, pool_type, kernel, stride, pad, pooling_convention,
                        count_include_pad, _is_channel_last(layout), p_value)


@register('_contrib_AdaptiveAvgPooling2D', aliases=('AdaptiveAvgPooling2D',), params={'output_size': ('shape', ())})
def adaptive_avg_pool2d(data, output_size=()):
    os_ = tuple(output_size) if output_size else (1, 1)
    if len(os_) == 1:
        os_ = os_ * 2
    return F.adaptive_avg_pool2d(data, os_)


@register('_contrib_BilinearResize2D', aliases=('BilinearResize2D',), arg_names=lambda a: ['data'] if a.get('mode', 'size') != 'like' else ['data', 'like'],
          params={'height': ('int', 1), 'width': ('int', 1), 'scale_height': ('float?', None),
                  'scale_width': ('float?', None), 'mode': ('str', 'size'), 'align_corners': ('bool', True)})
def bilinear_resize2d(data, like=None, height=1, width=1, scale_height=None, scale_width=None, mode='size',
                      align_corners=True):
    if mode == 'like' and like is not None:
        height, width = like.shape[2], like.shape[3]
    elif scale_height is not None:
        height, width = int(data.shape[2] * scale_height), int(data.shape[3] * (scale_width or scale_height))
    elif mode == 'odd_scale':
        pass
    return F.interpolate(data, size=(height, width), mode='bilinear', align_corners=align_corners)



_ACTS = {
    'relu': torch.relu, 'sigmoid': torch.sigmoid, 'tanh': torch.tanh,
    'softrelu': F.softplus, 'softsign': F.softsign, 'log_sigmoid': F.logsigmoid,
    'mish': F.mish,
}


@register('Activation', params={'act_type': ('str', 'relu')})
def activation(data, act_type='relu'):
    if act_type == 'relu':
        return hip_ops.relu(data)
    return _ACTS[act_type](data)


def _lrelu_args(a):
    return ['data', 'gamma'] if a.get('act_type', 'leaky') == 'prelu' else ['data']


def _lrelu_infer(in_shapes, a):
    if a.get('act_type') != 'prelu' or in_shapes[0] is None:
        return {}
    d = in_shapes[0]
    return {1: (d[1] if len(d) > 1 else 1,)}


@register('LeakyReLU', arg_names=_lrelu_args, infer_params=_lrelu_infer, num_outputs=1,
          params={'act_type': ('str', 'leaky'), 'slope': ('float', 0.25), 'lower_bound': ('float', 0.125),
                  'upper_bound': ('float', 0.334)})
def leaky_relu(data, gamma=None, act_type='leaky', slope=0.25, lower_bound=0.125, upper_bound=0.334):
    if act_type == 'leaky':
        return F.leaky_relu(data, slope)
# ... 847 lines not shown
```

mxnet_maintenance_amd/symbol/symbol.py:

```python
import copy
import json
import math
import warnings

import numpy as np
import torch

from ..attribute import AttrScope
from ..base import NotImplementedForSymbol, MXNetError, numeric_types, torch_dtype, np_dtype, dtype_name
from ..name import NameManager
from ..ops import registry

__all__ = ['Symbol', 'var', 'Variable', 'Group', 'load', 'load_json', 'zeros', 'ones', 'full', 'arange',
           'pow', 'power', 'maximum', 'minimum', 'hypot', 'eye', 'linspace', 'histogram', 'split_v2']

_MXNET_VERSION = 10901


class _Node:
    __slots__ = ('op', 'name', 'attrs', 'inputs', '_parsed', '__weakref__')

    def __init__(self, op, name, attrs=None, inputs=None):
        self.op = op
        self.name = name
        self.attrs = dict(attrs or {})
        self.inputs = list(inputs or [])
        self._parsed = None

    def is_var(self):
        return self.op is None

    def opdef(self):
        return registry.get(self.op)

    def parsed(self):
        if self._parsed is None:
            op = self.opdef()
            params = {k: v for k, v in self.attrs.items()
                      if k in op.params or (op.extra_params and not (k.startswith('__') and k.endswith('__')))}
            self._parsed = op.parse_attrs(params)
        return self._parsed

    def num_outputs(self):
        if self.op is None:
            return 1
        return self.opdef().get_num_outputs(self.parsed())

    def num_visible_outputs(self):
        if self.op is None:
            return 1
        return self.opdef().get_num_visible_outputs(self.parsed())


def _topo(entries):
    order, seen = [], set()
    stack = [(e[0], False) for e in reversed(entries)]
    while stack:
        node, done = stack.pop()
        if done:
            order.append(node)
            continue
        if id(node) in seen:
            continue
        seen.add(id(node))
        stack.append((node, True))
        for inp, _ in reversed(node.inputs):
            if id(inp) not in seen:
                stack.append((inp, False))
    return order


def _aux_var_ids(order):
    aux = set()
    for n in order:
        if n.op is None:
            continue
        if n.op == '_CachedOp':
            for i in (int(x) for x in n.attrs.get('aux_indices', '').split(',') if x != ''):
                if i < len(n.inputs) and n.inputs[i][0].op is None:
                    aux.add(id(n.inputs[i][0]))
            continue
        op = n.opdef()
        nargs = len(op.get_arg_names(n.parsed()))
        for i, (inp, _) in enumerate(n.inputs):
            if i >= nargs and inp.op is None:
                aux.add(id(inp))
    return aux


def _attr_lookup(attrs, key):
    if key in attrs:
        return attrs[key]
    dk = '__%s__' % key
    if dk in attrs:
        return attrs[dk]
    if key.startswith('__') and key.endswith('__') and key[2:-2] in attrs:
        return attrs[key[2:-2]]
    return None


class Symbol:
    __array_priority__ = 1000.0

    def __init__(self, outputs):
        import ctypes
        if isinstance(outputs, ctypes.c_void_p):
            from ..base import _handle_object
            outputs = _handle_object(outputs)._outputs
        self._outputs = list(outputs)

    @property
    def name(self):
        if len(self._outputs) != 1:
            return None
        node, idx = self._outputs[0]
        return node.name

    @property
    def handle(self):
        return self

    def __repr__(self):
        name = self.name
        if name is None:
            return '<Symbol group [%s]>' % ', '.join(s.name for s in self)
        return '<Symbol %s>' % name

    def __iter__(self):
        return (Symbol([o]) for o in self._outputs)

    def __len__(self):
        return len(self._outputs)

    def __copy__(self):
        return self.__deepcopy__(None)

    def __deepcopy__(self, memo):
        return load_json(self.tojson())

    def __getstate__(self):
        return {'json': self.tojson()}

    def __setstate__(self, state):
        self._outputs = load_json(state['json'])._outputs

    def _output(self, i):
        return Symbol([self._outputs[i]])

    def __getitem__(self, index):
        if isinstance(index, str):
            names = self.list_outputs()
            idx = [i for i, n in enumerate(names) if n == index]
            if len(idx) != 1:
                raise ValueError('There are multiple outputs with name "%s"' % index if idx else
                                 'Cannot find output that matches name "%s"' % index)
            index = idx[0]
        from .. import util as _util
        if (_util.is_np_array() and not getattr(self, '_legacy', False)
                and (not isinstance(index, (int, np.integer)) or len(self._outputs) == 1)):
            from ..ops.tensor import encode_basic_index
            return _create('_npi_basic_index', [self], {'key': encode_basic_index(index)})
        if isinstance(index, slice):
            return Symbol(self._outputs[index])
        return Symbol([self._outputs[index]])

    def _topo(self):
        return _topo(self._outputs)

    def list_arguments(self):
        order = self._topo()
        aux = _aux_var_ids(order)
        return [n.name for n in order if n.op is None and id(n) not in aux]

    def list_auxiliary_states(self):
        order = self._topo()
        aux = _aux_var_ids(order)
        return [n.name for n in order if n.op is None and id(n) in aux]

    def list_inputs(self):
        return [n.name for n in self._topo() if n.op is None]

    def list_outputs(self):
# ... 201 lines not shown
                    'slice', 'swapaxes', 'diag'):
            opname = {'reshape': 'Reshape', 'flatten': 'Flatten', 'astype': 'Cast', 'split': 'SliceChannel'}.get(name, name)
            if name != 'astype' and registry.has(name) and registry.get(name) is registry.get(opname):
                opname = name

            from .. import util as _util
            if name == 'flatten' and _util.is_np_array() and not getattr(self, '_legacy', False):
                return lambda *a, **k: _op_func('_npi_ravel')(self)

            def f(*a, **k):
                if name == 'reshape' and a:
                    k['shape'] = a[0] if len(a) == 1 and isinstance(a[0], (tuple, list)) else a
                    a = ()
                if name == 'transpose' and a:
                    k['axes'] = a[0] if len(a) == 1 and isinstance(a[0], (tuple, list)) else a
                    a = ()
                if name == 'astype' and a:
                    k['dtype'] = a[0]
                    a = ()
                return _op_func(opname)(self, *a, **k)
            return f
        if name.startswith('_'):
            raise AttributeError(name)
        if not vars(self).get('_legacy', False):
            from .. import numpy as _mnp
            meth = _mnp.ndarray.__dict__.get(name)
            fn = getattr(_mnp, name, None) if callable(meth) and not isinstance(meth, property) else None
            if callable(fn) and not isinstance(fn, type):
                return lambda *a, **k: fn(self, *a, **k)
        raise AttributeError("'Symbol' object has no attribute '%s'" % name)

    def infer_shape(self, *args, **kwargs):
        res = self._infer(args, kwargs, partial=False, what='shape')
        return res

    def infer_shape_partial(self, *args, **kwargs):
        return self._infer(args, kwargs, partial=True, what='shape')

    def infer_type(self, *args, **kwargs):
        return self._infer(args, kwargs, partial=False, what='type')

    def infer_type_partial(self, *args, **kwargs):
        return self._infer(args, kwargs, partial=True, what='type')

    def _infer(self, args, kwargs, partial, what):
        arg_names = self.list_arguments()
        known = {}
        if args:
            for n, v in zip(arg_names, args):
                if v is not None:
                    known[n] = v
        names = set(arg_names) | set(self.list_auxiliary_states())
        for k, v in kwargs.items():
            if v is not None and k in names:
                known[k] = v
        if what == 'shape':
            shapes, dtypes = {k: tuple(v) for k, v in known.items()}, {}
        else:
            shapes, dtypes = {}, {k: torch_dtype(v) for k, v in known.items()}
        res = infer_graph(self, shapes, dtypes, what=what, partial=partial)
        arg_res, out_res, aux_res = res
        if what == 'shape':
            complete = all(s is not None for s in arg_res + out_res + aux_res)
            if not complete and not partial:
                warnings.warn('Cannot decide shape for some arguments', stacklevel=2)
                return None, None, None
            from ..util import is_np_shape
            empty = None if is_np_shape() else ()
            fix = lambda l: [s if s is not None else empty for s in l]
            return fix(arg_res), fix(out_res), fix(aux_res)
        complete = all(s is not None for s in arg_res + out_res + aux_res)
        if not complete and not partial:
            return None, None, None
        conv = lambda l: [np_dtype(d) if d is not None else None for d in l]
        return conv(arg_res), conv(out_res), conv(aux_res)

    def tojson(self, remove_amp_cast=True):
        order = self._topo()
        index = {id(n): i for i, n in enumerate(order)}
        nodes, arg_nodes, row_ptr = [], [], [0]
        for i, n in enumerate(order):
            d = {'op': 'null' if n.op is None else n.op, 'name': n.name,
                 'inputs': [[index[id(a)], j, 0] for a, j in n.inputs]}
            if n.attrs:
                d['attrs'] = {k: str(v) for k, v in n.attrs.items()}
            nodes.append(d)
            if n.op is None:
                arg_nodes.append(i)
            row_ptr.append(row_ptr[-1] + (n.num_outputs() if n.op is not None else 1))
        heads = [[index[id(n)], j, 0] for n, j in self._outputs]
        from ..util import is_np_shape
        gattrs = {'mxnet_version': ['int', _MXNET_VERSION]}
        if is_np_shape():
            gattrs['is_np_shape'] = ['int', 1]
        return json.dumps({'nodes': nodes, 'arg_nodes': arg_nodes, 'node_row_ptr': row_ptr,
                           'heads': heads, 'attrs': gattrs}, indent=2)

    def save(self, fname, remove_amp_cast=True):
        with open(fname, 'w') as f:
            f.write(self.tojson())

    def bind(self, ctx, args, args_grad=None, grad_req='write', aux_states=None, group2ctx=None,
             shared_exec=None):
        from ..executor import Executor
        from . import subgraph
        return Executor(subgraph.env_partition(self), ctx, args, args_grad, grad_req, aux_states)

    def _bind(self, *a, **k):
        return self.bind(*a, **k)

    def simple_bind(self, ctx, grad_req='write', type_dict=None, stype_dict=None, group2ctx=None,
                    shared_arg_names=None, shared_exec=None, shared_buffer=None, force_rebind=False, **kwargs):
        from ..executor import Executor
        from .. import ndarray as nd
        arg_shapes, _, aux_shapes = self.infer_shape(**kwargs)
        if arg_shapes is None:
            raise MXNetError('simple_bind: cannot infer shapes from %s' % kwargs)
        arg_names = self.list_arguments()
        type_dict = type_dict or {}
        arg_types, _, aux_types = self.infer_type(**{k: v for k, v in type_dict.items() if k in arg_names})
        if arg_types is None:
            arg_types = [np.float32] * len(arg_names)
            aux_types = [np.float32] * len(aux_shapes)
        args = []
        var_nodes = self._var_nodes()

        def place(name):
            va = var_nodes[name].attrs if name in var_nodes else {}
            g = va.get('__ctx_group__', va.get('ctx_group'))
            return group2ctx[g] if (group2ctx and g in group2ctx) else ctx
        for n, s, t in zip(arg_names, arg_shapes, arg_types):
            if shared_buffer is not None and n in shared_buffer and shared_buffer[n].shape == tuple(s):
                args.append(shared_buffer[n])
            else:
                st = (stype_dict or {}).get(n, 'default')
                a = nd.zeros(s, ctx=place(n), dtype=t or np.float32, stype=st) if st != 'default' else \
                    nd.zeros(s, ctx=place(n), dtype=t or np.float32)
                if shared_buffer is not None:
                    shared_buffer[n] = a
                args.append(a)
        if isinstance(grad_req, str):
            reqs = {n: grad_req for n in arg_names}
        elif isinstance(grad_req, (list, tuple)):
            reqs = dict(zip(arg_names, grad_req))
        else:
            reqs = {n: grad_req.get(n, 'null') for n in arg_names}
        rsp_grads = self._row_sparse_grad_args()
        grads = {n: (nd.zeros(s, ctx=place(n), dtype=t or np.float32, stype='row_sparse') if n in rsp_grads else
                     nd.zeros(s, ctx=place(n), dtype=t or np.float32))
                 for n, s, t in zip(arg_names, arg_shapes, arg_types) if reqs.get(n, 'null') != 'null'}
        aux = [nd.zeros(s, ctx=ctx, dtype=t or np.float32) for s, t in zip(aux_shapes, aux_types)]
        from . import subgraph
        return Executor(subgraph.env_partition(self), ctx, args, grads, reqs, aux)

    def _row_sparse_grad_args(self):
        rsp, dense = set(), set()
        for n in self._topo():
            if n.op is None:
                continue
            sparse_w = n.op in ('Embedding', '_contrib_SparseEmbedding') and \
                (n.op == '_contrib_SparseEmbedding' or str(n.attrs.get('sparse_grad', 'False')) in ('True', 'true', '1'))
            for k, (src, _j) in enumerate(n.inputs):
                if src.op is not None:
                    continue
                (rsp if (sparse_w and k == 1) else dense).add(src.name)
        return rsp - dense

    def eval(self, ctx=None, **kwargs):
# ... 870 lines not shown
```

src/kernels/bindings.cc:

```cpp
#include <hip/hip_runtime.h>
#include <pybind11/pybind11.h>
#include <pybind11/stl.h>

#include <cstdint>
#include <stdexcept>
#include <vector>

namespace py = pybind11;

namespace mxamd {
void bn_nhwc_forward(int dtype, const void* x, const void* addend, void* y, uint8_t* mask, const float* gamma,
                     const float* beta,
                     const float* center, float* part, float* mean, float* invstd, float* var, float* scale,
                     float* shift, int64_t R, int C, float eps, int training, int relu, int fix_gamma,
                     float momentum, float* mm_upd, float* mv_upd, int ext_nblk, hipStream_t s);
void bn_nhwc_backward(int dtype, const void* x, const void* dy, const void* y, const uint8_t* mask, void* dx,
                      void* dz,
                      const float* gamma, const float* mean, const float* invstd, const float* fscale,
                      const float* fshift, float* part, float* dgamma, float* dbeta, float* coef, int64_t R, int C,
                      int relu_mode, int fix_gamma, int training, int accum, hipStream_t s, int ext_nblk, const void* ds_z, const float* ds_mean, float* ds_part);
int bn_partials_rows(int64_t R, int C);
int bn_tail_ds_rows(int64_t R, int C);
void gemm_nt(int dtype, const void* a, const void* b, const void* bias, const void* addend, void* c, int out_f32,
             int M, int N, int K, int lda, int ldb, int ldc, int act, int cfg, int splits, float* ws, hipStream_t s,
// ... 83 lines not shown
                            float p, uint64_t seed, const uint64_t* seed_base, hipStream_t s);
void add_dropout_ln_backward(int dtype, const void* s_in, const void* dy, const void* gamma, int pt, const float* mean,
                             const float* rstd, const uint8_t* mask, float p, void* ds, void* dh, float* part,
                             float* hpart, void* dgamma, void* dbeta, int gdtype, int accum, int M, int D,
                             hipStream_t s);
void column_sum_partials(int gdtype, const float* part, int nb, int ncol, void* out, int accum, hipStream_t s);
void gelu_forward(int dtype, const void* x, void* y, int64_t n, hipStream_t s);
void gelu_backward(int dtype, const void* x, const void* dy, void* dx, int64_t n, hipStream_t s);
void gelu_backward_colpart(int dtype, const void* x, const void* dy, void* dx, float* part, int M, int N,
                           hipStream_t s);
int gelu_colpart_blocks(int M, int N);
void softmax_forward(int dtype, int log, const void* x, void* y, int M, int L, float scale, hipStream_t s);
void softmax_backward(int dtype, int log, const void* y, const void* dy, void* dx, int M, int L, float scale,
                      hipStream_t s);
void dropout_forward(int dtype, const void* x, void* y, uint8_t* mask, int64_t n, float p, uint64_t seed,
                     const uint64_t* seed_base, hipStream_t s);
void dropout_backward(int dtype, const void* dy, const uint8_t* mask, void* dx, int64_t n, float p, hipStream_t s);
int attention_max_seq();
void attention_forward(int dtype, const void* qkv, const float* kmask, void* out, float* lse, int S, int B, int H,
                       int D, float scale, float p, uint64_t seed, const uint64_t* seed_base, hipStream_t s);
void attention_backward(int dtype, const void* qkv, const float* kmask, const void* out, const void* dout,
                        const float* lse, float* delta, void* dqkv, int S, int B, int H, int D, float scale, float p,
                        uint64_t seed, const uint64_t* seed_base, hipStream_t s);
void flat_adam(int dtype, int mode, void* w, const void* g, float* mean, float* var, float* w32, int64_t n, float lr,
               float beta1, float beta2, float eps, float wd, float eta, float rescale, float clip, const float* hp,
               hipStream_t s);
void lamb_update(int dtype, void* w, const void* g, float* mean, float* var, float* w32, float* upd,
                 const void* chunks, int nchunks, float* nrm, int nseg, float lr, float beta1, float beta2, float eps,
                 float bc1, float bc2, float wd, float rescale, float clip, float lb, float ub, const float* hp,
                 hipStream_t s);
void seg_sumsq(int dtype, const void* x, const void* chunks, int nchunks, float* out, int nseg, hipStream_t s);
void all_finite(int dtype, const void* x, int64_t n, float scale, int* flag, int init, hipStream_t s);
void pool_nhwc_forward(int dtype, int is_max, const void* x, void* y, uint8_t* arg, int N, int H, int W, int C,
                       int Ho, int Wo, int kh, int kw, int sh, int sw, int ph, int pw, int cip, hipStream_t s,
                       const float* scale, const float* shift);
int bn_pool_bwd_blocks();
void bn_pool_backward(int dtype, const void* x, const void* dy, const uint8_t* arg, void* dx, const float* gamma,
                      const float* mean, const float* invstd, const float* fscale, const float* fshift, float* part,
                      float* dgamma, float* dbeta, float* coef, int N, int H, int W, int C, int Ho, int Wo, int kh,
                      int kw, int sh, int sw, int ph, int pw, int fix_gamma, int training, int accum,
                      hipStream_t s);
void pool_nhwc_backward(int dtype, int is_max, const void* dy, const uint8_t* arg, void* dx, int N, int H, int W,
                        int C, int Ho, int Wo, int kh, int kw, int sh, int sw, int ph, int pw, int cip,
                        hipStream_t s);
void deform_im2col(int dtype, const void* x, const void* off, const void* msk, void* cols, int N, int C, int H, int W,
                   int Ho, int Wo, int kh, int kw, int sh, int sw, int ph, int pw, int dh, int dw, int dg,
                   int rows, hipStream_t s);
void deform_col2im(int dtype, const void* off, const void* msk, const void* gcols, float* gx, int N, int C, int H,
                   int W, int Ho, int Wo, int kh, int kw, int sh, int sw, int ph, int pw, int dh, int dw, int dg,
                   int rows, hipStream_t s);
void deform_col2im_coord(int dtype, const void* x, const void* off, const void* msk, const void* gcols, void* goff,
                         void* gmsk, int N, int C, int H, int W, int Ho, int Wo, int kh, int kw, int sh, int sw,
                         int ph, int pw, int dh, int dw, int dg, int rows, hipStream_t s);
void deform_im2col_nhwc(int dtype, const void* x, const void* off, const void* msk, void* cols, const int* g,
                        int ld_off, int ld_msk, hipStream_t s);
void deform_bwd_nhwc(int dtype, const void* x, const void* off, const void* msk, const void* gcols, float* gx,
                     void* goff, void* gmsk, const int* g, int ld_off, int ld_msk, hipStream_t s);
void conv_dw_fwd(int dtype, const void* x, const void* wt, const float* bias, void* y, const int* gm, hipStream_t s);
void conv_dw_dgrad(int dtype, const void* dy, const void* wt, void* dx, const int* gm, hipStream_t s);
void conv_dw_wgrad(int dtype, const void* x, const void* dy, float* slab, int nslice, int out_dtype, void* out,
                   int accum, const int* gm, hipStream_t s);
int ssd_loss_blocks(int rows);
void ssd_loss_fwd(int dtype, const void* cls, const void* loc, const float* cls_t, const float* loc_t,
                  const float* loc_m, int rows, int C1, float lambd, float* part, float* out, hipStream_t s);
void ssd_loss_bwd(int dtype, const void* cls, const void* loc, const float* cls_t, const float* loc_t,
                  const float* loc_m, const float* stats, const float* gout, int rows, int C1, float lambd, void* dcls,
                  void* dloc, hipStream_t s);
void multibox_target(int dtype, const float* anchors, const float* labels, const void* cls_pred, float* loc_target,
                     float* loc_mask, float* cls_target, float* match_iou, int* match_gt, uint32_t* key, int B, int A,
                     int L, int W, int C, float thr, float ignore_label, float neg_ratio, float neg_thresh,
                     int min_neg, float v0, float v1, float v2, float v3, hipStream_t s);
void slab_reduce(int out_dtype, float* slab, int splits, int64_t n, void* out, int accum, hipStream_t s);
void twobit_quantize(int dtype, const void* g, float* res, void* packed, int64_t n, float thr, hipStream_t s);
void twobit_dequantize_sum(const void* packed, int64_t row_bytes, int nrows, int64_t n, float thr, float* out,
                           hipStream_t s);
int conv_pw_stream_ok(int kin, int nout);
int conv_pw_stream_grid(int M, int kin, int nout, int ncu, int add);
int conv_pw_stream_slices(int kin, int nout);
void weight_taps_t(int elem_bytes, const void* w, void* out, int K, int RS, int C, int n, const int* src,
                   const int64_t* base, const int64_t* rstride, hipStream_t s);
void conv_pw_stream(int dtype, const void* x, const void* w, void* y, const void* zero, int M, int kin, int nout,
                    float* part, int grid, hipStream_t s, const void* addend, int wt, const void* bn_z,
                    const uint8_t* bn_mask, const float* bn_mean, const float* bn_scale, const float* bn_shift,
                    int bn_mode, const uint8_t* addend_mask);
int conv_pw_stream_bnb_ok(int kin, int nout, int add, int mode);
void conv_gen(int dtype, int mode, const void* src, const void* wsrc, const float* bias, void* dst, const int* geom,
              int splits, hipStream_t s);
void rnn_fwd_seq(int dtype, int mode, const float* gx, const void* h0, const float* c0, const void* whh,
                 const float* bhh, void* out, int ldo, float* cseq, float* save, int Tn, int N, int H, int reverse,
                 hipStream_t s);
void rnn_bwd_seq(int dtype, int mode, const void* whhT, const void* dy, int ldy, const float* dhT,
                 const float* save, const float* cseq, const float* c0, const void* h0, const void* out, int ldo,
                 void* dgh, void* dgx, float* dc, float* dhd, float* dh0, int Tn, int N, int H, int reverse,
                 hipStream_t s);
}

using namespace mxamd;

template <typename T>
static inline T* P(uintptr_t p) {
  return reinterpret_cast<T*>(p);
}
static inline hipStream_t S(uintptr_t s) { return reinterpret_cast<hipStream_t>(s); }
static inline hipStream_t S_(uintptr_t s) { return reinterpret_cast<hipStream_t>(s); }

static void check_launch(const char* name) {
  hipError_t e = hipGetLastError();
  if (e != hipSuccess) throw std::runtime_error(std::string(name) + ": " + hipGetErrorString(e));
}

PYBIND11_MODULE(_hip_kernels, m) {
  m.doc() = "gfx950 HIP kernels for mxnet_maintenance_amd";
  m.attr("arch") = "gfx950";

  m.def("bn_partials_rows", &bn_partials_rows);
  m.def("bn_tail_ds_rows", &bn_tail_ds_rows);
  m.def("bn_nhwc_stats", [](int dt, uintptr_t x, uintptr_t center, uintptr_t part, int64_t R, int C, uintptr_t s) {
    int nblk = bn_nhwc_stats(dt, P<const void>(x), P<const float>(center), P<float>(part), R, C, S(s), 512);
    check_launch("bn_nhwc_stats");
    return nblk;
  });
  m.def("embedding_forward", [](int dt, int it, uintptr_t idx, uintptr_t w, uintptr_t y, int64_t n, int V, int C,
                                uintptr_t s) {
    embedding_forward(dt, it, P<const void>(idx), P<const void>(w), P<void>(y), n, V, C, S(s));
    check_launch("embedding_forward");
  });
  m.def("embedding_backward", [](int dt, int it, uintptr_t idx, uintptr_t dy, uintptr_t acc, uintptr_t touched,
                                 int odt, uintptr_t grad, int accum, int64_t n, int V, int C, uintptr_t s) {
    embedding_backward(dt, it, P<const void>(idx), P<const void>(dy), P<float>(acc), P<uint8_t>(touched), odt,
                       P<void>(grad), accum, n, V, C, S(s));
    check_launch("embedding_backward");
  });
  m.def("csr_dot_dense", [](int dt, uintptr_t indptr, uintptr_t indices, uintptr_t vals, uintptr_t rhs, uintptr_t out,
                            int64_t M, int64_t K, int N, uintptr_t s) {
    csr_dot_dense(dt, P<const int64_t>(indptr), P<const int64_t>(indices), P<const void>(vals), P<const void>(rhs),
                  P<void>(out), M, K, N, S(s));
    check_launch("csr_dot_dense");
  });
  m.def("csrT_dot_dense", [](int dt, uintptr_t indptr, uintptr_t indices, uintptr_t vals, uintptr_t rhs,
                             uintptr_t slot, uintptr_t out32, int64_t M, int64_t K, int N, uintptr_t s) {
    csrT_dot_dense(dt, P<const int64_t>(indptr), P<const int64_t>(indices), P<const void>(vals), P<const void>(rhs),
                   P<const int64_t>(slot), P<float>(out32), M, K, N, S(s));
    check_launch("csrT_dot_dense");
  });
  m.def("int8_gemm", [](uintptr_t a, uintptr_t b, uintptr_t c, int M, int N, int K, uintptr_t s) {
    int8_gemm(P<const int8_t>(a), P<const int8_t>(b), P<int32_t>(c), M, N, K, S(s));
    check_launch("int8_gemm");
  });
  m.def("colsum_partials", [](int64_t R, int C) { return colsum_partials(R, C); });
  m.def("colsum_rows", [](int dt, uintptr_t x, uintptr_t zeros, uintptr_t part, int64_t R, int C, int odt,
                          uintptr_t out, int accum, uintptr_t s) {
    colsum_rows(dt, P<const void>(x), P<const float>(zeros), P<float>(part), R, C, odt, P<void>(out), accum, S(s));
    check_launch("colsum_rows");
  });
  m.def("twobit_quantize", [](int dt, uintptr_t g, uintptr_t res, uintptr_t packed, int64_t n, float thr,
                              uintptr_t s) {
    twobit_quantize(dt, P<void>(g), P<float>(res), P<void>(packed), n, thr, S(s));
    check_launch("twobit_quantize");
  });
  m.def("twobit_dequantize_sum", [](uintptr_t packed, int64_t row_bytes, int nrows, int64_t n, float thr,
                                    uintptr_t out, uintptr_t s) {
    twobit_dequantize_sum(P<void>(packed), row_bytes, nrows, n, thr, P<float>(out), S(s));
    check_launch("twobit_dequantize_sum");
  });
  m.def("gemm_nt", [](int dt, uintptr_t a, uintptr_t b, uintptr_t bias, uintptr_t addend, uintptr_t c, int out_f32,
                      int M, int N, int K, int lda, int ldb, int ldc, int act, int cfg, int splits, uintptr_t ws,
                      uintptr_t s, int bias_lowp) {
    gemm_nt(dt, P<void>(a), P<void>(b), P<void>(bias), P<void>(addend), P<void>(c), out_f32, M, N, K, lda, ldb, ldc,
            act, cfg, splits, P<float>(ws), S(s), bias_lowp);
    check_launch("gemm_nt");
  }, py::arg("dt"), py::arg("a"), py::arg("b"), py::arg("bias"), py::arg("addend"), py::arg("c"), py::arg("out_f32"),
     py::arg("M"), py::arg("N"), py::arg("K"), py::arg("lda"), py::arg("ldb"), py::arg("ldc"), py::arg("act"),
     py::arg("cfg"), py::arg("splits"), py::arg("ws"), py::arg("s"), py::arg("bias_lowp") = 0);
  m.def("weight_taps_t", [](int eb, uintptr_t w, uintptr_t out, int K, int RS, int C, std::vector<int> src,
                            std::vector<int64_t> base, std::vector<int64_t> rstride, uintptr_t s) {
    if (src.size() != base.size() || src.size() != rstride.size()) throw std::runtime_error("weight_taps_t: table sizes");
    weight_taps_t(eb, P<const void>(w), P<void>(out), K, RS, C, static_cast<int>(src.size()), src.data(), base.data(),
                  rstride.data(), S(s));
    check_launch("weight_taps_t");
  });
  m.def("conv_pw_stream_ok", &conv_pw_stream_ok);
  m.def("conv_pw_stream_slices", &conv_pw_stream_slices);
  m.def("conv_pw_stream_grid", [](int M, int kin, int nout, int ncu, int add) {
    return conv_pw_stream_grid(M, kin, nout, ncu, add);
  }, pybind11::arg("M"), pybind11::arg("kin"), pybind11::arg("nout"), pybind11::arg("ncu"), pybind11::arg("add") = 0);
  m.def("conv_pw_stream", [](int dt, uintptr_t x, uintptr_t w, uintptr_t y, uintptr_t zero, int M, int kin, int nout,
                             uintptr_t part, int grid, uintptr_t s, uintptr_t addend, int wt, uintptr_t bn_z,
                             uintptr_t bn_mask, uintptr_t bn_mean, uintptr_t bn_scale, uintptr_t bn_shift, int bn_mode,
                             uintptr_t addend_mask) {
    conv_pw_stream(dt, P<const void>(x), P<const void>(w), P<void>(y), P<const void>(zero), M, kin, nout,
                   P<float>(part), grid, S(s), P<const void>(addend), wt, P<const void>(bn_z), P<const uint8_t>(bn_mask),
                   P<const float>(bn_mean), P<const float>(bn_scale), P<const float>(bn_shift), bn_mode,
                   P<const uint8_t>(addend_mask));
    check_launch("conv_pw_stream");
  }, pybind11::arg("dt"), pybind11::arg("x"), pybind11::arg("w"), pybind11::arg("y"), pybind11::arg("zero"),
     pybind11::arg("M"), pybind11::arg("kin"), pybind11::arg("nout"), pybind11::arg("part"), pybind11::arg("grid"),
     pybind11::arg("s"), pybind11::arg("addend"), pybind11::arg("wt") = 0, pybind11::arg("bn_z") = 0,
     pybind11::arg("bn_mask") = 0, pybind11::arg("bn_mean") = 0, pybind11::arg("bn_scale") = 0,
     pybind11::arg("bn_shift") = 0, pybind11::arg("bn_mode") = 0, pybind11::arg("addend_mask") = 0);
  m.def("conv_pw_stream_bnb_ok", &conv_pw_stream_bnb_ok);
  m.def("conv_gen", [](int dt, int mode, uintptr_t src, uintptr_t wsrc, uintptr_t bias, uintptr_t dst,
                       std::vector<int> geom, int splits, uintptr_t s) {
    if (geom.size() != 22) throw std::runtime_error("conv_gen: geometry needs 22 ints");
    conv_gen(dt, mode, P<const void>(src), P<const void>(wsrc), P<const float>(bias), P<void>(dst), geom.data(),
             splits, S(s));
    check_launch("conv_gen");
  });
  m.def("rnn_fwd_seq", [](int dt, int mode, uintptr_t gx, uintptr_t h0, uintptr_t c0, uintptr_t whh, uintptr_t bhh,
                          uintptr_t out, int ldo, uintptr_t cseq, uintptr_t save, int T, int N, int H, int reverse,
                          uintptr_t s) {
    rnn_fwd_seq(dt, mode, P<const float>(gx), P<const void>(h0), P<const float>(c0), P<const void>(whh),
                P<const float>(bhh), P<void>(out), ldo, P<float>(cseq), P<float>(save), T, N, H, reverse, S(s));
    check_launch("rnn_fwd_seq");
  });
  m.def("rnn_bwd_seq", [](int dt, int mode, uintptr_t whhT, uintptr_t dy, int ldy, uintptr_t dhT, uintptr_t save,
                          uintptr_t cseq, uintptr_t c0, uintptr_t h0, uintptr_t out, int ldo, uintptr_t dgh,
                          uintptr_t dgx, uintptr_t dc, uintptr_t dhd, uintptr_t dh0, int T, int N, int H, int reverse,
                          uintptr_t s) {
    rnn_bwd_seq(dt, mode, P<const void>(whhT), P<const void>(dy), ldy, P<const float>(dhT), P<const float>(save),
                P<const float>(cseq), P<const float>(c0), P<const void>(h0), P<const void>(out), ldo, P<void>(dgh),
                P<void>(dgx), P<float>(dc), P<float>(dhd), P<float>(dh0), T, N, H, reverse, S(s));
    check_launch("rnn_bwd_seq");
  });
  m.def("gemm_nt_tile_n", &gemm_nt_tile_n);
  m.def("gemm_nt_tile_m", &gemm_nt_tile_m);
  m.def("slab_reduce", [](int odt, uintptr_t slab, int splits, int64_t n, uintptr_t out, int accum, uintptr_t s) {
    slab_reduce(odt, P<float>(slab), splits, n, P<void>(out), accum, S(s));
    check_launch("slab_reduce");
  });
  m.def("deform_im2col", [](int dt, uintptr_t x, uintptr_t off, uintptr_t msk, uintptr_t cols, std::vector<int> g,
                            uintptr_t s) {
    if (g.size() != 15 && g.size() != 16) throw std::runtime_error("deform_im2col: geometry needs 15 or 16 ints");
    const int rows = g.size() == 16 ? g[15] : 0;
    deform_im2col(dt, P<void>(x), P<void>(off), P<void>(msk), P<void>(cols), g[0], g[1], g[2], g[3], g[4], g[5], g[6],
                  g[7], g[8], g[9], g[10], g[11], g[12], g[13], g[14], rows, S(s));
    check_launch("deform_im2col");
  });
  m.def("deform_col2im", [](int dt, uintptr_t off, uintptr_t msk, uintptr_t gcols, uintptr_t gx, std::vector<int> g,
                            uintptr_t s) {
    if (g.size() != 15 && g.size() != 16) throw std::runtime_error("deform_col2im: geometry needs 15 or 16 ints");
    const int rows = g.size() == 16 ? g[15] : 0;
    deform_col2im(dt, P<void>(off), P<void>(msk), P<void>(gcols), P<float>(gx), g[0], g[1], g[2], g[3], g[4], g[5],
                  g[6], g[7], g[8], g[9], g[10], g[11], g[12], g[13], g[14], rows, S(s));
    check_launch("deform_col2im");
  });
  m.def("deform_col2im_coord", [](int dt, uintptr_t x, uintptr_t off, uintptr_t msk, uintptr_t gcols, uintptr_t goff,
                                  uintptr_t gmsk, std::vector<int> g, uintptr_t s) {
    if (g.size() != 15 && g.size() != 16) throw std::runtime_error("deform_col2im_coord: geometry needs 15 or 16 ints");
    const int rows = g.size() == 16 ? g[15] : 0;
    deform_col2im_coord(dt, P<void>(x), P<void>(off), P<void>(msk), P<void>(gcols), P<void>(goff), P<void>(gmsk),
                        g[0], g[1], g[2], g[3], g[4], g[5], g[6], g[7], g[8], g[9], g[10], g[11], g[12], g[13], g[14],
                        rows, S(s));
    check_launch("deform_col2im_coord");
  });
  m.def("deform_im2col_nhwc", [](int dt, uintptr_t x, uintptr_t off, uintptr_t msk, uintptr_t cols, std::vector<int> g,
                                 int ld_off, int ld_msk, uintptr_t s) {
    if (g.size() != 15) throw std::runtime_error("deform_im2col_nhwc: geometry needs 15 ints");
    deform_im2col_nhwc(dt, P<void>(x), P<void>(off), P<void>(msk), P<void>(cols), g.data(), ld_off, ld_msk, S(s));
    check_launch("deform_im2col_nhwc");
  });
  m.def("deform_bwd_nhwc", [](int dt, uintptr_t x, uintptr_t off, uintptr_t msk, uintptr_t gcols, uintptr_t gx,
                              uintptr_t goff, uintptr_t gmsk, std::vector<int> g, int ld_off, int ld_msk, uintptr_t s) {
    if (g.size() != 15) throw std::runtime_error("deform_bwd_nhwc: geometry needs 15 ints");
    deform_bwd_nhwc(dt, P<void>(x), P<void>(off), P<void>(msk), P<void>(gcols), P<float>(gx), P<void>(goff),
                    P<void>(gmsk), g.data(), ld_off, ld_msk, S(s));
    check_launch("deform_bwd_nhwc");
  });
  m.def("conv_dw_fwd", [](int dt, uintptr_t x, uintptr_t wt, uintptr_t bias, uintptr_t y, std::vector<int> g,
                          uintptr_t s) {
    if (g.size() != 14) throw std::runtime_error("conv_dw_fwd: geometry needs 14 ints");
    conv_dw_fwd(dt, P<void>(x), P<void>(wt), P<float>(bias), P<void>(y), g.data(), S(s));
    check_launch("conv_dw_fwd");
  });
  m.def("conv_dw_dgrad", [](int dt, uintptr_t dy, uintptr_t wt, uintptr_t dx, std::vector<int> g, uintptr_t s) {
    if (g.size() != 14) throw std::runtime_error("conv_dw_dgrad: geometry needs 14 ints");
    conv_dw_dgrad(dt, P<void>(dy), P<void>(wt), P<void>(dx), g.data(), S(s));
    check_launch("conv_dw_dgrad");
  });
  m.def("conv_dw_wgrad", [](int dt, uintptr_t x, uintptr_t dy, uintptr_t slab, int nslice, int out_dt, uintptr_t out,
                            int accum, std::vector<int> g, uintptr_t s) {
    if (g.size() != 14) throw std::runtime_error("conv_dw_wgrad: geometry needs 14 ints");
    conv_dw_wgrad(dt, P<void>(x), P<void>(dy), P<float>(slab), nslice, out_dt, P<void>(out), accum, g.data(), S(s));
    check_launch("conv_dw_wgrad");
// ... 388 lines not shown
```

src/kernels/bn_nhwc.hip:

```cpp
#include <cstdlib>
#include <stdexcept>

#include <algorithm>

#include "common.h"

namespace mxamd {

constexpr int kBnThreads = 256;

struct BnGeom {
  int tpr;
  int cb;
  int rpi;
};

static inline BnGeom bn_geom(int C) {
  BnGeom g;
  int v = C / 8;
  g.tpr = v;
  if (v > kBnThreads)
    for (g.tpr = kBnThreads; v % g.tpr != 0; --g.tpr) {
    }
  g.cb = g.tpr * 8;
  g.rpi = kBnThreads / g.tpr;
  return g;
}

constexpr int kReluNone = 0;
constexpr int kReluFromY = 1;
constexpr int kReluFromX = 2;
constexpr int kReluFromMask = 3;

template <typename T, int MODE, int RELU>
__global__ void __launch_bounds__(kBnThreads) bn_reduce_kernel(
    const T* __restrict__ x, const T* __restrict__ dy, const T* __restrict__ y, const uint8_t* __restrict__ mask,
    const float* __restrict__ center, const float* __restrict__ fscale, const float* __restrict__ fshift,
    float* __restrict__ part1, float* __restrict__ part2, int64_t R, int C, int tpr, int rpi,
    int64_t rows_per_block) {
  const int tid = threadIdx.x;
  const int lane_c = tid % tpr;
  const int lane_r = tid / tpr;
  const int cbase = blockIdx.y * tpr * 8 + lane_c * 8;
  float s1[8], s2[8], k[8], fs[8], fh[8];
#pragma unroll
  for (int i = 0; i < 8; ++i) {
    s1[i] = 0.f;
    s2[i] = 0.f;
    k[i] = center[cbase + i];
    if (RELU == kReluFromX) {
      fs[i] = fscale[cbase + i];
      fh[i] = fshift[cbase + i];
    }
  }
  const int64_t r0 = static_cast<int64_t>(blockIdx.x) * rows_per_block;
  int64_t r1 = r0 + rows_per_block;
  if (r1 > R) r1 = R;
  const bool spare = lane_r >= rpi;
  if (spare) r1 = r0;
  constexpr int UNR = 4;
  auto accum = [&](const Vec8<T>& vx, const Vec8<T>& vdy, const Vec8<T>& vy, uint32_t mb) {
#pragma unroll
    for (int i = 0; i < 8; ++i) {
      if (MODE == 0) {
        float d = vx.get(i) - k[i];
        s1[i] += d;
        s2[i] += d * d;
      } else {
        float dz = vdy.get(i);
        const float xi = vx.get(i);
        if (RELU == kReluFromY) dz = vy.get(i) > 0.f ? dz : 0.f;
        if (RELU == kReluFromX) dz = fmaf(xi, fs[i], fh[i]) > 0.f ? dz : 0.f;
        if (RELU == kReluFromMask) dz = ((mb >> i) & 1u) ? dz : 0.f;
        s1[i] += dz;
        s2[i] += dz * (xi - k[i]);
      }
    }
  };
  int64_t r = r0 + lane_r;
  for (; r + (UNR - 1) * rpi < r1; r += UNR * rpi) {
    Vec8<T> vx[UNR], vdy[UNR], vy[UNR];
    uint32_t vm[UNR];
#pragma unroll
    for (int u = 0; u < UNR; ++u) {
      const int64_t off = (r + u * rpi) * C + cbase;
      vx[u].load(x + off);
      if (MODE == 1) vdy[u].load(dy + off);
// ... 70 lines not shown
  const double n = static_cast<double>(R);
  const float g = fix_gamma ? 1.f : gamma[c];
  if (MODE == 0) {
    double m1 = a / n;
    double var = b / n - m1 * m1;
    if (var < 0) var = 0;
    double mean = center[c] + m1;
    float inv = static_cast<float>(1.0 / sqrt(var + eps));
    o0[c] = static_cast<float>(mean);
    o1[c] = inv;
    o2[c] = static_cast<float>(var);
    float sc = g * inv;
    o3[c] = sc;
    o4[c] = beta[c] - static_cast<float>(mean) * sc;
    if (mm_upd) mm_upd[c] = mm_upd[c] * momentum + static_cast<float>(mean) * (1.f - momentum);
    if (mv_upd) mv_upd[c] = mv_upd[c] * momentum + static_cast<float>(var) * (1.f - momentum);
  } else {
    const float inv = invstd_in[c];
    const double dbeta = a;
    const double dgamma = b * inv;
    if (accum) {
      o0[c] += static_cast<float>(dgamma);
      o1[c] += static_cast<float>(dbeta);
    } else {
      o0[c] = static_cast<float>(dgamma);
      o1[c] = static_cast<float>(dbeta);
    }
    const double A = static_cast<double>(g) * inv;
    const double B = training ? -A * inv * dgamma / n : 0.0;
    const double Cc = training ? A * (static_cast<double>(center[c]) * inv * dgamma / n - dbeta / n) : 0.0;
    o2[c] = static_cast<float>(A);
    o3[c] = static_cast<float>(B);
    o4[c] = static_cast<float>(Cc);
  }
}

typedef unsigned int bn_u32x4 __attribute__((ext_vector_type(4)));

template <typename T>
__device__ __forceinline__ void vload(Vec8<T>& v, const T* p, int nt) {
  if constexpr (sizeof(T) == 2) {
    if (nt) {
      const bn_u32x4 r = __builtin_nontemporal_load(reinterpret_cast<const bn_u32x4*>(p));
      v.raw = make_uint4(r.x, r.y, r.z, r.w);
      return;
    }
  }
  v.load(p);
}

template <typename T>
__device__ __forceinline__ void vstore(const Vec8<T>& v, T* p, int nt) {
  if constexpr (sizeof(T) == 2) {
    if (nt > 1) {
      const bn_u32x4 r = {v.raw.x, v.raw.y, v.raw.z, v.raw.w};
      __builtin_nontemporal_store(r, reinterpret_cast<bn_u32x4*>(p));
      return;
    }
  }
  v.store(p);
}

__device__ __forceinline__ void load8f(const float* __restrict__ p, float* o) {
  const float4 a = *reinterpret_cast<const float4*>(p);
  const float4 b = *reinterpret_cast<const float4*>(p + 4);
  o[0] = a.x; o[1] = a.y; o[2] = a.z; o[3] = a.w; o[4] = b.x; o[5] = b.y; o[6] = b.z; o[7] = b.w;
}


template <typename T, bool ADD, bool RELU, bool MASK>
__global__ void __launch_bounds__(kBnThreads) bn_apply_kernel(
    const T* __restrict__ x, const T* __restrict__ addend, const float* __restrict__ scale,
    const float* __restrict__ shift, T* __restrict__ y, uint8_t* __restrict__ mask, int64_t nvec, int C, int nt) {
  const int64_t stride = static_cast<int64_t>(gridDim.x) * blockDim.x;
  int64_t v = static_cast<int64_t>(blockIdx.x) * blockDim.x + threadIdx.x;
  int c = static_cast<int>((v * 8) % C);
  const int cstep = static_cast<int>((stride * 8) % C);
  float sc[8], sh[8];
  auto compute = [&](const Vec8<T>& vx, const Vec8<T>& va, int64_t vv) {
    Vec8<T> out;
    uint32_t bits = 0;
#pragma unroll
    for (int i = 0; i < 8; ++i) {
      float r = vx.get(i) * sc[i] + sh[i];
      if (ADD) r += va.get(i);
      if (MASK) bits |= (r > 0.f ? 1u : 0u) << i;
      if (RELU) r = r > 0.f ? r : 0.f;
      out.set(i, r);
    }
    vstore(out, y + vv * 8, nt == 2 ? 2 : 0);
    if (MASK) mask[vv] = static_cast<uint8_t>(bits);
  };
  if (cstep == 0) {
    load8f(scale + c, sc);
    load8f(shift + c, sh);
    for (; v + stride < nvec; v += 2 * stride) {
      Vec8<T> vx0, vx1, va0, va1;
      vload(vx0, x + v * 8, nt);
      vload(vx1, x + (v + stride) * 8, nt);
      if (ADD) {
        vload(va0, addend + v * 8, nt);
        vload(va1, addend + (v + stride) * 8, nt);
      }
      compute(vx0, va0, v);
      compute(vx1, va1, v + stride);
    }
    if (v < nvec) {
      Vec8<T> vx, va;
      vload(vx, x + v * 8, nt);
      if (ADD) vload(va, addend + v * 8, nt);
      compute(vx, va, v);
    }
    return;
  }
  for (; v < nvec; v += stride, c = (c + cstep >= C) ? c + cstep - C : c + cstep) {
    Vec8<T> vx, va;
    vload(vx, x + v * 8, nt);
    if (ADD) vload(va, addend + v * 8, nt);
    load8f(scale + c, sc);
    load8f(shift + c, sh);
    compute(vx, va, v);
  }
}

template <typename T, int RELU, bool WRITE_DZ>
__global__ void __launch_bounds__(kBnThreads) bn_bwd_apply_kernel(
    const T* __restrict__ x, const T* __restrict__ dy, const T* __restrict__ y, const uint8_t* __restrict__ mask,
    const float* __restrict__ A, const float* __restrict__ B, const float* __restrict__ Cc,
    const float* __restrict__ fscale, const float* __restrict__ fshift,
    T* __restrict__ dx, T* __restrict__ dz_out, int64_t nvec, int C, int nt) {
  const int64_t stride = static_cast<int64_t>(gridDim.x) * blockDim.x;
  int64_t v = static_cast<int64_t>(blockIdx.x) * blockDim.x + threadIdx.x;
  int c = static_cast<int>((v * 8) % C);
  const int cstep = static_cast<int>((stride * 8) % C);
  float fs[8], fh[8], ka[8], kb[8], kc[8];
  auto coef = [&](int cc) {
    if (RELU == kReluFromX) {
      load8f(fscale + cc, fs);
      load8f(fshift + cc, fh);
    }
    load8f(A + cc, ka);
    load8f(B + cc, kb);
    load8f(Cc + cc, kc);
  };
  struct In {
    Vec8<T> x, dy, y;
    uint32_t mb;
  };
  auto load = [&](In& in, int64_t vv) {
    vload(in.x, x + vv * 8, nt);
    vload(in.dy, dy + vv * 8, nt);
    if (RELU == kReluFromY) vload(in.y, y + vv * 8, nt);
    in.mb = RELU == kReluFromMask ? mask[vv] : 0u;
  };
  auto compute = [&](const In& in, int64_t vv) {
    Vec8<T> out, dz;
#pragma unroll
    for (int i = 0; i < 8; ++i) {
      float d = in.dy.get(i);
      if (RELU == kReluFromY) d = in.y.get(i) > 0.f ? d : 0.f;
      if (RELU == kReluFromX) d = fmaf(in.x.get(i), fs[i], fh[i]) > 0.f ? d : 0.f;
      if (RELU == kReluFromMask) d = ((in.mb >> i) & 1u) ? d : 0.f;
      if (WRITE_DZ) dz.set(i, d);
      out.set(i, ka[i] * d + kb[i] * in.x.get(i) + kc[i]);
    }
    vstore(out, dx + vv * 8, nt == 2 ? 2 : 0);
    if (WRITE_DZ) vstore(dz, dz_out + vv * 8, nt >= 2 ? 2 : 0);
  };
  if (cstep == 0) {
    coef(c);
    for (; v + stride < nvec; v += 2 * stride) {
// ... 430 lines not shown
```

src/kernels/conv_pw.hip:

```cpp
#include <stdexcept>

#include "common.h"
#include "mfma.h"

namespace mxamd {

namespace {

typedef _Float16 half8_t __attribute__((ext_vector_type(8)));
typedef __bf16 bf16x8_t __attribute__((ext_vector_type(8)));
typedef float f4_t __attribute__((ext_vector_type(4)));
typedef uint32_t u32x4 __attribute__((ext_vector_type(4)));
typedef __attribute__((address_space(3))) void lds_void;
typedef __attribute__((address_space(1))) void gbl_void;

template <typename T>
struct PwM : mfma::Op<T> {
  template <typename V>
  static __device__ __forceinline__ f4_t mma(const V& a, const V& b, f4_t c) {
    return mfma::Op<T>::run(a, b, c);
  }
};

template <int N>
__device__ __forceinline__ void vm_wait() {
  static_assert(N >= 0 && N < 64, "vmcnt range");
  __builtin_amdgcn_s_waitcnt((N & 15) | (7 << 4) | (15 << 8) | ((N >> 4) << 14));
}

__device__ __forceinline__ void lds_barrier() { asm volatile("s_waitcnt lgkmcnt(0)\n\ts_barrier" ::: "memory"); }

__device__ __forceinline__ uint32_t lds_byte(const char* p) {
  const uintptr_t a = reinterpret_cast<uintptr_t>(p);
  return (*reinterpret_cast<const uint32_t*>(a & ~static_cast<uintptr_t>(3)) >> ((a & 3u) * 8)) & 0xffu;
}

constexpr int pw_bm(int kin, int nout, bool add) {
  const int in_rows = (8192 / kin) > 16 ? (8192 / kin) : 16;
  const int bm0 = (16384 / nout) < in_rows ? (16384 / nout) : in_rows;
  if (!add) return bm0;
  const int wp = 8 / ((nout / 16) < 8 ? (nout / 16) : 8);
  int bm = bm0 < 32 ? bm0 : 32;
  if (bm > 8192 / nout) bm = 8192 / nout;
  if (bm < 16 * wp) bm = 16 * wp;
  return bm;
}

constexpr int kPwBnbNone = 0;
constexpr int kPwBnbPlain = 1;
constexpr int kPwBnbFromZ = 2;
constexpr int kPwBnbMask = 3;

struct PwBnb {
  const void* z;
  const uint8_t* mask;
  const float* mean;
  const float* scale;
  const float* shift;
  const uint8_t* amask;
};

template <int KIN, int NOUT, int WPC = 2, bool ADD = false, int BNB = kPwBnbNone, bool AMK = false>
struct PwCfg {
  static constexpr bool EXT = ADD || BNB != kPwBnbNone;
  static constexpr int BM = pw_bm(KIN, NOUT, EXT);
  static constexpr int WC = NOUT / 16 < 8 ? NOUT / 16 : 8;
  static constexpr int WP = 8 / WC;
  static constexpr int FC = NOUT / WC / 16;
  static constexpr int FP = BM / WP / 16;
  static constexpr int KS = KIN / 32;
  static constexpr int ROWB = KIN * 2;
  static constexpr int STAGE_IN = BM * ROWB;
  static constexpr int STAGE_ADD = ADD ? BM * NOUT * 2 : 0;
  static constexpr int STAGE_Z = BNB ? BM * NOUT * 2 : 0;
  static constexpr int STAGE_M = BNB == kPwBnbMask ? (BM * NOUT / 8 + 1023) / 1024 * 1024 : 0;
  static constexpr int STAGE_AM = AMK ? (BM * NOUT / 8 + 1023) / 1024 * 1024 : 0;
  static constexpr int STAGE = STAGE_IN + STAGE_ADD + STAGE_Z + STAGE_M + STAGE_AM;
  static constexpr int LPT = STAGE_IN / (512 * 16);
  static constexpr int APT = STAGE_ADD / (512 * 16);
  static constexpr int TI = STAGE_IN / 1024;
  static constexpr int TA = STAGE_ADD / 1024;
  static constexpr int TZ = STAGE_Z / 1024;
  static constexpr int TM = STAGE_M / 1024;
  static constexpr int TAM = STAGE_AM / 1024;
  static constexpr int PITCH = NOUT * 2 + 16;
  static constexpr int EPI = BM * PITCH;
  static constexpr int OCH = NOUT / 8;
  static constexpr int SPT = (BM * OCH + 511) / 512;
  static constexpr int LDS = WPC == 1 ? 156 * 1024 : 80 * 1024;
  static constexpr int NMAX = EXT ? 6 : 4;
  static constexpr int NST = (NMAX * STAGE + EPI <= LDS) ? NMAX
                           : ((NMAX - 1) * STAGE + EPI <= LDS) ? NMAX - 1
                           : ((NMAX - 2) * STAGE + EPI <= LDS) ? NMAX - 2 : 2;
  static constexpr int D = NST - 1;
  static constexpr int SMEM = NST * STAGE + EPI;
  static_assert(FC >= 1 && FP >= 1, "at least one fragment pair per wave");
  static_assert(EXT || (LPT >= 1 && STAGE_IN % (512 * 16) == 0), "whole LDS-DMA instructions per tile");
  static_assert(!EXT || (STAGE_IN % 1024 == 0 && STAGE_ADD % 1024 == 0 && STAGE_Z % 1024 == 0),
                "whole 1 KB LDS-DMA instructions");
  static_assert(!EXT || WPC == 1, "the extra stages need the LDS of a whole CU");
  static_assert(BNB != kPwBnbMask || (NOUT / 8) % 16 == 0, "mask rows of whole 16-byte chunks");
  static_assert((BM * OCH) % 512 == 0 || BM * OCH < 512, "whole store rounds, or a single partial one");
  static_assert(512 % OCH == 0, "a thread keeps one output chunk");
  static_assert(D * ((TI + 7) / 8 + (TA + 7) / 8 + (TZ + 7) / 8 + (TM + 7) / 8 + (TAM + 7) / 8 + SPT) <
                    (EXT ? 40 : 64),
                "vmcnt range (vm_wait_n covers < 40)");
  static_assert(!AMK || (ADD && (NOUT / 8) % 16 == 0), "the addend mask rides with an addend, whole 16-byte rows");
  static_assert(FC * KS * 4 <= (WPC == 1 ? 128 : 64), "resident weights exceed the register budget");
  static_assert(ROWB % 128 == 0, "rows of whole 128-byte swizzle groups");
};

__device__ __forceinline__ void vm_wait_n(int n) {
  switch (n) {
#define MXAMD_VMW(K) \
  case K:            \
    vm_wait<K>();    \
    break;
    MXAMD_VMW(0) MXAMD_VMW(1) MXAMD_VMW(2) MXAMD_VMW(3) MXAMD_VMW(4) MXAMD_VMW(5) MXAMD_VMW(6) MXAMD_VMW(7)
    MXAMD_VMW(8) MXAMD_VMW(9) MXAMD_VMW(10) MXAMD_VMW(11) MXAMD_VMW(12) MXAMD_VMW(13) MXAMD_VMW(14) MXAMD_VMW(15)
    MXAMD_VMW(16) MXAMD_VMW(17) MXAMD_VMW(18) MXAMD_VMW(19) MXAMD_VMW(20) MXAMD_VMW(21) MXAMD_VMW(22)
    MXAMD_VMW(23) MXAMD_VMW(24) MXAMD_VMW(25) MXAMD_VMW(26) MXAMD_VMW(27) MXAMD_VMW(28) MXAMD_VMW(29)
    MXAMD_VMW(30) MXAMD_VMW(31) MXAMD_VMW(32) MXAMD_VMW(33) MXAMD_VMW(34) MXAMD_VMW(35) MXAMD_VMW(36)
    MXAMD_VMW(37) MXAMD_VMW(38) MXAMD_VMW(39)
#undef MXAMD_VMW
    default:
      vm_wait<39>();
  }
}

__device__ __forceinline__ void vm_wait_le(int n) {
  if (n >= 48) vm_wait<48>();
  else if (n >= 32) vm_wait<32>();
  else if (n >= 24) vm_wait<24>();
  else if (n >= 16) vm_wait<16>();
  else if (n >= 12) vm_wait<12>();
  else if (n >= 8) vm_wait<8>();
  else if (n >= 6) vm_wait<6>();
  else if (n >= 4) vm_wait<4>();
  else if (n >= 3) vm_wait<3>();
  else if (n >= 2) vm_wait<2>();
  else if (n >= 1) vm_wait<1>();
  else vm_wait<0>();
}

template <typename T, int KIN, int NOUT, bool STATS, bool ADD, int WPC, int S, int BNB, bool AMK = false>
__global__ void __launch_bounds__(512) __attribute__((amdgpu_waves_per_eu(2 * WPC))) conv_pw_stream_kernel(
    const T* __restrict__ x, const T* __restrict__ w, T* __restrict__ y, const T* __restrict__ zero, int M, int ntiles,
    float* __restrict__ part, const T* __restrict__ addend, int wt, PwBnb bnb) {
  using C = PwCfg<KIN, NOUT, WPC, ADD, BNB, AMK>;
  constexpr bool EXT = C::EXT;
  extern __shared__ __attribute__((aligned(1024))) char smem[];
  const int tid = threadIdx.x;
  const int lane = tid & 63;
  const int wid = tid >> 6;
  const int wc = wid % C::WC, wp = wid / C::WC;
  const int grid = gridDim.x;
  const int xcd = blockIdx.x & 7;
  const int q8 = grid >> 3, r8 = grid & 7;
  const int wg0 = (xcd < r8 ? xcd * (q8 + 1) : r8 * (q8 + 1) + (xcd - r8) * q8) + (blockIdx.x >> 3);
  constexpr int NT = NOUT * S;
  const int slice = S > 1 ? wg0 % S : 0;
  const int wg = S > 1 ? wg0 / S : wg0;
  const int gs = grid / S;

  u32x4 wa[C::FC][C::KS];
  if (!wt) {
#pragma unroll
    for (int f = 0; f < C::FC; ++f)
#pragma unroll
      for (int s = 0; s < C::KS; ++s) {
        const int co = slice * NOUT + wc * C::FC * 16 + f * 16 + (lane & 15);
        wa[f][s] = *reinterpret_cast<const u32x4*>(w + static_cast<int64_t>(co) * KIN + s * 32 + (lane >> 4) * 8);
      }
  } else {
#pragma unroll
    for (int f = 0; f < C::FC; ++f)
#pragma unroll
      for (int s = 0; s < C::KS; ++s) {
        const int k = s * 32 + (lane >> 1);
        const int co = slice * NOUT + wc * C::FC * 16 + f * 16 + (lane & 1) * 8;
        wa[f][s] = *reinterpret_cast<const u32x4*>(w + static_cast<int64_t>(k) * NT + co);
      }
  }

  vm_wait<0>();
  if (wt) {
    uint16_t* scr = reinterpret_cast<uint16_t*>(smem + wid * 1280);
#pragma unroll
    for (int f = 0; f < C::FC; ++f)
#pragma unroll
      for (int s = 0; s < C::KS; ++s) {
        const uint4 v = __builtin_bit_cast(uint4, wa[f][s]);
        const uint32_t wv[4] = {v.x, v.y, v.z, v.w};
#pragma unroll
        for (int q = 0; q < 8; ++q)
          scr[((lane & 1) * 8 + q) * 40 + (lane >> 1)] = static_cast<uint16_t>(wv[q >> 1] >> ((q & 1) * 16));
        asm volatile("s_waitcnt lgkmcnt(0)" ::: "memory");
        wa[f][s] = *reinterpret_cast<const u32x4*>(scr + (lane & 15) * 40 + (lane >> 4) * 8);
        asm volatile("s_waitcnt lgkmcnt(0)" ::: "memory");
      }
    __syncthreads();
  }
#pragma unroll
  for (int f = 0; f < C::FC; ++f)
#pragma unroll
    for (int s = 0; s < C::KS; ++s) asm volatile("" ::"v"(wa[f][s]));

  auto issue = [&](int t, int st) {
    char* sb = smem + st * C::STAGE;
    constexpr int NI = EXT ? (C::TI + 7) / 8 : C::LPT;
#pragma unroll
    for (int j = 0; j < NI; ++j) {
      const int i = j * 8 + wid;
      if (EXT && i >= C::TI) break;
      const int byte = (i * 64 + lane) * 16;
      const int row = byte / C::ROWB;
      const int slot = (byte % C::ROWB) / 16;
      const int chunk = slot ^ (row & 7);
      const int p = t * C::BM + row;
      const T* src = p < M ? x + static_cast<int64_t>(p) * KIN + chunk * 8 : zero + (chunk & 7) * 8;
      __builtin_amdgcn_global_load_lds((gbl_void*)src, (lds_void*)(sb + i * 1024), 16, 0, 0);
    }
#pragma unroll
    for (int j = 0; j < (C::TA + 7) / 8; ++j) {
      const int i = j * 8 + wid;
      if (i >= C::TA) break;
      const int byte = (i * 64 + lane) * 16;
      const int row = byte / (NOUT * 2);
      const int p = t * C::BM + row;
      const T* src = p < M ? addend + static_cast<int64_t>(p) * NT + slice * NOUT + (byte % (NOUT * 2)) / 2 : zero;
      __builtin_amdgcn_global_load_lds((gbl_void*)src, (lds_void*)(sb + C::STAGE_IN + i * 1024), 16, 0, 0);
    }
#pragma unroll
    for (int j = 0; j < (C::TZ + 7) / 8; ++j) {
      const int i = j * 8 + wid;
      if (i >= C::TZ) break;
      const int byte = (i * 64 + lane) * 16;
      const int row = byte / (NOUT * 2);
      const int p = t * C::BM + row;
      const T* src = p < M ? static_cast<const T*>(bnb.z) + static_cast<int64_t>(p) * NT + slice * NOUT +
                                 (byte % (NOUT * 2)) / 2
                           : zero;
      __builtin_amdgcn_global_load_lds((gbl_void*)src, (lds_void*)(sb + C::STAGE_IN + C::STAGE_ADD + i * 1024), 16, 0,
                                       0);
    }
#pragma unroll
    for (int j = 0; j < (C::TM + 7) / 8; ++j) {
      const int i = j * 8 + wid;
      if (i >= C::TM) break;
      const int byte = (i * 64 + lane) * 16;
      const int row = byte / (NOUT / 8);
      const int p = t * C::BM + row;
      const void* src = (row < C::BM && p < M)
                            ? static_cast<const void*>(bnb.mask + (static_cast<int64_t>(p) * NT + slice * NOUT) / 8 +
                                                       byte % (NOUT / 8))
                            : static_cast<const void*>(zero);
      __builtin_amdgcn_global_load_lds((gbl_void*)src,
                                       (lds_void*)(sb + C::STAGE_IN + C::STAGE_ADD + C::STAGE_Z + i * 1024), 16, 0, 0);
    }
#pragma unroll
    for (int j = 0; j < (C::TAM + 7) / 8; ++j) {
      const int i = j * 8 + wid;
      if (i >= C::TAM) break;
      const int byte = (i * 64 + lane) * 16;
      const int row = byte / (NOUT / 8);
      const int p = t * C::BM + row;
      const void* src = (row < C::BM && p < M)
                            ? static_cast<const void*>(bnb.amask + (static_cast<int64_t>(p) * NT + slice * NOUT) / 8 +
                                                       byte % (NOUT / 8))
                            : static_cast<const void*>(zero);
      __builtin_amdgcn_global_load_lds(
          (gbl_void*)src, (lds_void*)(sb + C::STAGE_IN + C::STAGE_ADD + C::STAGE_Z + C::STAGE_M + i * 1024), 16, 0, 0);
    }
  };
  const int ops_per_tile = EXT ? (C::TI - wid + 7) / 8 + (C::TA - wid + 7) / 8 + (C::TZ - wid + 7) / 8 +
                                      (C::TM - wid + 7) / 8 + (C::TAM - wid + 7) / 8
                                : C::LPT;

  const int my_tiles = wg < ntiles ? (ntiles - wg + gs - 1) / gs : 0;
  for (int j = 0; j < C::D && j < my_tiles; ++j) issue(wg + j * gs, j);

  float s1[8], s2[8];
#pragma unroll
  for (int e = 0; e < 8; ++e) {
    s1[e] = 0.f;
    s2[e] = 0.f;
  }
  const int my_c8 = tid % C::OCH;
  char* epi = smem + C::NST * C::STAGE;
  float bmean[8], bsc[8], bsh[8];
#pragma unroll
  for (int q = 0; q < 8; ++q) {
    const int ch = slice * NOUT + my_c8 * 8 + q;
    bmean[q] = BNB ? bnb.mean[ch] : 0.f;
    bsc[q] = BNB == kPwBnbFromZ ? bnb.scale[ch] : 0.f;
    bsh[q] = BNB == kPwBnbFromZ ? bnb.shift[ch] : 0.f;
  }

  for (int it = 0; it < my_tiles; ++it) {
    const int t = wg + it * gs;
    const int st = it % C::NST;
    if (!EXT) {
      if (it + C::D < my_tiles) issue(wg + (it + C::D) * gs, (it + C::D) % C::NST);
      const int later = (my_tiles - 1 - it) < C::D ? (my_tiles - 1 - it) : C::D;
      const int epis = it < C::D ? it : C::D;
      if (later == C::D && epis == C::D) vm_wait<C::D*(C::LPT + C::SPT)>();
      else vm_wait_le(later * C::LPT + epis * C::SPT);
      lds_barrier();
    } else {
      const int later = (my_tiles - 1 - it) < C::D - 1 ? (my_tiles - 1 - it) : C::D - 1;
      const int epis = it < C::D ? it : C::D;
      vm_wait_n(later * ops_per_tile + epis * C::SPT);
      lds_barrier();
      if (it + C::D < my_tiles) issue(wg + (it + C::D) * gs, (it + C::D) % C::NST);
    }

    const char* sb = smem + st * C::STAGE;
    f4_t acc[C::FC][C::FP];
#pragma unroll
    for (int f = 0; f < C::FC; ++f)
#pragma unroll
      for (int p = 0; p < C::FP; ++p) acc[f][p] = f4_t{0.f, 0.f, 0.f, 0.f};
#pragma unroll
    for (int s = 0; s < C::KS; ++s) {
      u32x4 bf[C::FP];
#pragma unroll
      for (int p = 0; p < C::FP; ++p) {
        const int row = wp * C::FP * 16 + p * 16 + (lane & 15);
        const int chunk = s * 4 + (lane >> 4);
        bf[p] = *reinterpret_cast<const u32x4*>(sb + row * C::ROWB + ((chunk ^ (row & 7)) * 16));
      }
#pragma unroll
      for (int f = 0; f < C::FC; ++f)
#pragma unroll
        for (int p = 0; p < C::FP; ++p) acc[f][p] = PwM<T>::mma(wa[f][s], bf[p], acc[f][p]);
    }
#pragma unroll
    for (int f = 0; f < C::FC; ++f)
#pragma unroll
      for (int p = 0; p < C::FP; ++p) {
        const int pix = wp * C::FP * 16 + p * 16 + (lane & 15);
        const int co = wc * C::FC * 16 + f * 16 + (lane >> 4) * 4;
        const f4_t v = acc[f][p];
        *reinterpret_cast<uint2*>(epi + pix * C::PITCH + co * 2) = PwM<T>::pack4(v[0], v[1], v[2], v[3]);
      }
    lds_barrier();
    const __amdgpu_buffer_rsrc_t yrs = __builtin_amdgcn_make_buffer_rsrc(
        y, 0, static_cast<int>(static_cast<uint32_t>(M) * NT * sizeof(T)), 0x00020000);
#pragma unroll
    for (int k = 0; k < C::SPT; ++k) {
      const int e = tid + k * 512;
      const bool in_tile = e < C::BM * C::OCH;
      const int pix = in_tile ? e / C::OCH : 0;
      const int c8 = e % C::OCH;
      const int p = t * C::BM + pix;
      Vec8<T> v;
      v.raw = *reinterpret_cast<const uint4*>(epi + pix * C::PITCH + c8 * 16);
      if (ADD) {
        Vec8<T> a;
        a.raw = *reinterpret_cast<const uint4*>(sb + C::STAGE_IN + pix * (NOUT * 2) + c8 * 16);
        if (AMK) {
          const uint32_t amb = lds_byte(sb + C::STAGE_IN + C::STAGE_ADD + C::STAGE_Z + C::STAGE_M + pix * (NOUT / 8) + c8);
          auto m2 = [&](int j) -> uint32_t {
            const uint32_t b = (amb >> (2 * j)) & 3u;
            return (b & 1u) * 0xFFFFu | (b >> 1) * 0xFFFF0000u;
          };
          a.raw.x &= m2(0);
          a.raw.y &= m2(1);
          a.raw.z &= m2(2);
          a.raw.w &= m2(3);
        }
#pragma unroll
        for (int q = 0; q < 8; ++q) v.set(q, v.get(q) + a.get(q));
      }
      const bool live = in_tile && p < M;
      if (BNB && live) {
        Vec8<T> zv;
        zv.raw = *reinterpret_cast<const uint4*>(sb + C::STAGE_IN + C::STAGE_ADD + pix * (NOUT * 2) + c8 * 16);
        const uint32_t mb =
            BNB == kPwBnbMask ? lds_byte(sb + C::STAGE_IN + C::STAGE_ADD + C::STAGE_Z + pix * (NOUT / 8) + c8)
                              : 0xffu;
#pragma unroll
        for (int q = 0; q < 8; ++q) {
          const float zq = zv.get(q);
          bool keep = true;
          if (BNB == kPwBnbFromZ) keep = fmaf(zq, bsc[q], bsh[q]) > 0.f;
          if (BNB == kPwBnbMask) keep = (mb >> q) & 1u;
          const float dz = keep ? v.get(q) : 0.f;
          s1[q] += dz;
          s2[q] += dz * (zq - bmean[q]);
        }
      }
      const uint32_t off = live ? (static_cast<uint32_t>(p) * NT + slice * NOUT + c8 * 8) * sizeof(T) : 0xFFFFFFF0u;
      __builtin_amdgcn_raw_buffer_store_b128(__builtin_bit_cast(u32x4, v.raw), yrs, off, 0, 0);
      if (STATS && live) {
#pragma unroll
        for (int q = 0; q < 8; ++q) {
          const float z = v.get(q);
          s1[q] += z;
          s2[q] += z * z;
        }
      }
    }
    (void)my_c8;
  }
  if (STATS || BNB) {
    vm_wait<0>();
    lds_barrier();
    float* red = reinterpret_cast<float*>(smem);
    constexpr int ROWS = 512 / C::OCH;
#pragma unroll
    for (int q = 0; q < 8; ++q) {
      red[(tid / C::OCH) * NOUT + my_c8 * 8 + q] = s1[q];
      red[ROWS * NOUT + (tid / C::OCH) * NOUT + my_c8 * 8 + q] = s2[q];
    }
    lds_barrier();
    for (int qq = tid; qq < 2 * NOUT; qq += 512) {
      const int which = qq / NOUT, ch = qq - which * NOUT;
      const float* col = red + which * ROWS * NOUT + ch;
      float a = 0.f;
      for (int r = 0; r < ROWS; ++r) a += col[r * NOUT];
      part[static_cast<int64_t>(which) * NT * gs + static_cast<int64_t>(slice * NOUT + ch) * gs + wg] = a;
    }
  }
}

template <typename T, int KIN, int NOUT, int WPC, int S, bool STATS, bool ADD, int BNB = kPwBnbNone, bool AMK = false>
void launch_pw_v(const void* x, const void* w, void* y, const void* zero, int M, float* part, const void* addend,
                 int grid, hipStream_t s, int wt, const PwBnb& bnb = PwBnb{}) {
  using C = PwCfg<KIN, NOUT, WPC, ADD, BNB, AMK>;
  static_assert(C::SMEM <= C::LDS && C::NST >= 2, "LDS budget / ring depth");
  static bool set = false;
  if (!set) {
    hipFuncSetAttribute(
        reinterpret_cast<const void*>(&conv_pw_stream_kernel<T, KIN, NOUT, STATS, ADD, WPC, S, BNB, AMK>),
        hipFuncAttributeMaxDynamicSharedMemorySize, C::SMEM);
    set = true;
  }
  const int ntiles = (M + C::BM - 1) / C::BM;
  hipLaunchKernelGGL((conv_pw_stream_kernel<T, KIN, NOUT, STATS, ADD, WPC, S, BNB, AMK>), dim3(grid), dim3(512), C::SMEM,
                     s, static_cast<const T*>(x), static_cast<const T*>(w), static_cast<T*>(y),
                     static_cast<const T*>(zero), M, ntiles, part, static_cast<const T*>(addend), wt, bnb);
}

template <int KIN, int NOUT>
constexpr bool pw_bnb_built(bool add, int mode) {
  return add ? (mode == kPwBnbMask && (NOUT / 8) % 16 == 0) : mode == kPwBnbFromZ;
}

template <typename T, int KIN, int NOUT, int S>
bool launch_pw_bnb(const void* x, const void* w, void* y, const void* zero, int M, float* part, const void* addend,
                   int grid, hipStream_t s, int wt, const PwBnb& bnb, int mode) {
  if constexpr ((NOUT / 8) % 16 == 0) {
    if (addend && mode == kPwBnbMask) {
      if (bnb.amask)
        launch_pw_v<T, KIN, NOUT, 1, S, false, true, kPwBnbMask, true>(x, w, y, zero, M, part, addend, grid, s, wt,
                                                                        bnb);
      else
        launch_pw_v<T, KIN, NOUT, 1, S, false, true, kPwBnbMask>(x, w, y, zero, M, part, addend, grid, s, wt, bnb);
      return true;
    }
  }
  if (!addend && mode == kPwBnbFromZ) {
    launch_pw_v<T, KIN, NOUT, 1, S, false, false, kPwBnbFromZ>(x, w, y, zero, M, part, addend, grid, s, wt, bnb);
    return true;
  }
  return false;
}

template <typename T, int KIN, int NOUT, int WPC, int S>
void launch_pw(const void* x, const void* w, void* y, const void* zero, int M, float* part, const void* addend,
               int grid, hipStream_t s, int wt, const PwBnb* bnb, int mode) {
  if (bnb) {
    MXAMD_HOST_CHECK((launch_pw_bnb<T, KIN, NOUT, S>(x, w, y, zero, M, part, addend, grid, s, wt, *bnb, mode)),
                     "conv_pw_stream: BN-backward variant not built");
    return;
  }
  using C = PwCfg<KIN, NOUT, WPC>;
  using CA = PwCfg<KIN, NOUT, 1, true>;
  static_assert(C::SMEM <= C::LDS && CA::SMEM <= CA::LDS, "workgroups per CU");
  static_assert(C::NST >= 2 && CA::NST >= 2, "ring depth");
  if (part) {
    if (addend) launch_pw_v<T, KIN, NOUT, 1, S, true, true>(x, w, y, zero, M, part, addend, grid, s, wt);
    else launch_pw_v<T, KIN, NOUT, WPC, S, true, false>(x, w, y, zero, M, part, addend, grid, s, wt);
  } else {
    if (addend) launch_pw_v<T, KIN, NOUT, 1, S, false, true>(x, w, y, zero, M, part, addend, grid, s, wt);
    else launch_pw_v<T, KIN, NOUT, WPC, S, false, false>(x, w, y, zero, M, part, addend, grid, s, wt);
  }
}

#define MXAMD_PW_SHAPES(X)                                                                                  \
  X(64, 64, 2, 1) X(64, 128, 2, 1) X(64, 256, 2, 1) X(128, 128, 2, 1) X(128, 256, 2, 1) X(256, 64, 2, 1)     \
  X(256, 128, 2, 1) X(512, 128, 2, 1) X(128, 512, 1, 1) X(256, 512, 1, 1) X(512, 256, 1, 1) X(256, 512, 1, 2) \
  X(1024, 128, 1, 2) X(512, 256, 1, 8)

template <typename T>
bool dispatch_pw(int kin, int nout, const void* x, const void* w, void* y, const void* zero, int M, float* part,
                 const void* addend, int grid, hipStream_t s, int wt, const PwBnb* bnb, int mode) {
#define MXAMD_PW_CASE(K, N, W, SL)                                        \
  if (kin == K && nout == N * SL) {                                       \
    launch_pw<T, K, N, W, SL>(x, w, y, zero, M, part, addend, grid, s, wt, bnb, mode); \
    return true;                                                          \
  }
  MXAMD_PW_SHAPES(MXAMD_PW_CASE)
#undef MXAMD_PW_CASE
  return false;
}

}

int conv_pw_stream_ok(int kin, int nout) {
#define MXAMD_PW_OK(K, N, W, SL) \
  if (kin == K && nout == N * SL) return W;
  MXAMD_PW_SHAPES(MXAMD_PW_OK)
#undef MXAMD_PW_OK
  return 0;
}

int conv_pw_stream_slices(int kin, int nout) {
#define MXAMD_PW_SL(K, N, W, SL) \
  if (kin == K && nout == N * SL) return SL;
  MXAMD_PW_SHAPES(MXAMD_PW_SL)
#undef MXAMD_PW_SL
  return 0;
}

int conv_pw_stream_bnb_ok(int kin, int nout, int add, int mode) {
#define MXAMD_PW_BOK(K, N, W, SL) \
  if (kin == K && nout == N * SL) return pw_bnb_built<K, N>(add != 0, mode) ? 1 : 0;
  MXAMD_PW_SHAPES(MXAMD_PW_BOK)
#undef MXAMD_PW_BOK
  return 0;
}

int conv_pw_stream_grid(int M, int kin, int nout, int ncu, int add) {
  const int sl = conv_pw_stream_slices(kin, nout);
  if (sl == 0) return 0;
  const int bm = pw_bm(kin, nout / sl, add != 0);
  const int ntiles = (M + bm - 1) / bm;
  const int wpc = add ? 1 : conv_pw_stream_ok(kin, nout);
  int per = (wpc * ncu + sl - 1) / sl;
  if (per > ntiles) per = ntiles;
  return per * sl;
}

void conv_pw_stream(int dtype, const void* x, const void* w, void* y, const void* zero, int M, int kin, int nout,
                    float* part, int grid, hipStream_t s, const void* addend, int wt, const void* bn_z,
                    const uint8_t* bn_mask, const float* bn_mean, const float* bn_scale, const float* bn_shift,
                    int bn_mode, const uint8_t* addend_mask) {
  MXAMD_HOST_CHECK(conv_pw_stream_ok(kin, nout), "conv_pw_stream: unsupported (Cin, Cout)");
  MXAMD_HOST_CHECK(grid >= 1 && grid % conv_pw_stream_slices(kin, nout) == 0 &&
                   (int64_t)M * nout * 2 < (1ll << 31) - 64 && (int64_t)M * kin < (1ll << 31),
                   "conv_pw_stream: tensor too large for 32-bit offsets");
  PwBnb bnb{bn_z, bn_mask, bn_mean, bn_scale, bn_shift, addend_mask};
  MXAMD_HOST_CHECK(addend_mask == nullptr || (addend && bn_z && bn_mode == kPwBnbMask),
                   "conv_pw_stream: the addend mask is built for the tee data gradient with the tail's BN statistics");
  const PwBnb* pb = nullptr;
  if (bn_z) {
    MXAMD_HOST_CHECK(part && bn_mean && conv_pw_stream_bnb_ok(kin, nout, addend != nullptr, bn_mode) &&
                         (bn_mode != kPwBnbFromZ || (bn_scale && bn_shift)) && (bn_mode != kPwBnbMask || bn_mask),
                     "conv_pw_stream: BN-backward statistics need partials, mean, a built mode and its mask source");
    pb = &bnb;
  }
  bool ok = false;
  if (dtype == kF16) ok = dispatch_pw<__half>(kin, nout, x, w, y, zero, M, part, addend, grid, s, wt, pb, bn_mode);
  else if (dtype == kBF16)
    ok = dispatch_pw<__hip_bfloat16>(kin, nout, x, w, y, zero, M, part, addend, grid, s, wt, pb, bn_mode);
  MXAMD_HOST_CHECK(ok, "conv_pw_stream: dtype must be f16 or bf16");
}

}
```

Baseline: 12320 images/sec.

## Defer BN-add-ReLU tail apply into the next ConvolutionTee pointwise conv prologue

The BatchNormAddReLU at the end of a bottleneck block, when the next block starts with a ConvolutionTee, now computes only its statistics and records a pending token. The normalize+add+ReLU apply is then fused into the next 1x1 conv kernel's prologue, which also writes the side output and ReLU mask. Every other consumer triggers a flush that runs the apply on its own. This saves one full read-write pass over the activation, at the cost of global deferred state, flush hooks across the executor, invoke and autograd paths, and an autotuned choice between the fused and unfused candidates.

```diff
diff --git a/mxnet_maintenance_amd/_state.py b/mxnet_maintenance_amd/_state.py
--- a/mxnet_maintenance_amd/_state.py
+++ b/mxnet_maintenance_amd/_state.py
@@ -16,6 +16,16 @@
 DIRECT_GRAD = [0]
 
 
+TAIL_FLUSH = [None]
+TAIL_CONSUMERS = ('_contrib_ConvolutionTee', 'ConvolutionTee')
+
+
+def flush_deferred(opname=None):
+    f = TAIL_FLUSH[0]
+    if f is not None and opname not in TAIL_CONSUMERS:
+        f()
+
+
 def is_recording():
     return STATE.recording
 
diff --git a/mxnet_maintenance_amd/autograd.py b/mxnet_maintenance_amd/autograd.py
--- a/mxnet_maintenance_amd/autograd.py
+++ b/mxnet_maintenance_amd/autograd.py
@@ -211,6 +211,7 @@
                 setattr(h._data, _RELEASED_ATTR, True)
     leaves = _collect_leaves(retain_graph)
     _prepare_leaves(leaves)
+    _state.flush_deferred()
     prev_train = set_training(train_mode)
     prev_rec = set_recording(False)
     direct = not create_graph
diff --git a/mxnet_maintenance_amd/executor.py b/mxnet_maintenance_amd/executor.py
--- a/mxnet_maintenance_amd/executor.py
+++ b/mxnet_maintenance_amd/executor.py
@@ -81,6 +81,8 @@
         try:
             for si, (fn, ins, attrs, outs, name, opname) in enumerate(self.steps):
                 args = [vals[i] for i in ins]
+                if _state.TAIL_FLUSH[0] is not None:
+                    _state.flush_deferred(opname)
                 if sched is not None:
                     sched.before(si, args)
                 if _amp.active:
@@ -129,6 +131,7 @@
                     for o, t in zip(outs, r):
                         vals[o] = t
                 if monitor is not None:
+                    _state.flush_deferred()
                     op = registry.get(opname)
                     onames = op.output_names or (['output'] if len(outs) == 1 else
                                                  ['output%d' % k for k in range(len(outs))])
@@ -138,6 +141,7 @@
         finally:
             if sched is not None:
                 torch.cuda.set_stream(sched.main)
+        _state.flush_deferred()
         self.out_idts = [islot.get(s) for s in self.out_slots] if islot else None
         if sched is not None:
             sched.finish([vals[s] for s in self.out_slots])
diff --git a/mxnet_maintenance_amd/gluon/model_zoo/vision/resnet.py b/mxnet_maintenance_amd/gluon/model_zoo/vision/resnet.py
--- a/mxnet_maintenance_amd/gluon/model_zoo/vision/resnet.py
+++ b/mxnet_maintenance_amd/gluon/model_zoo/vision/resnet.py
@@ -46,14 +46,16 @@
     def __init__(self, layout, fuse, **kwargs):
         super().__init__(axis=_bn_axis(layout), **kwargs)
         self._fuse_add = fuse
+        self._defer_apply = False
 
     def _alias(self):
         return 'batchnorm'
 
     def hybrid_forward(self, F, x, shortcut, gamma, beta, running_mean, running_var):
         if self._fuse_add:
+            extra = {'defer_apply': True} if self._defer_apply else {}
             return F.contrib.BatchNormAddReLU(x, shortcut, gamma, beta, running_mean, running_var, name='fwd',
-                                              **self._kwargs)
+                                              **extra, **self._kwargs)
         return F.BatchNorm(x, gamma, beta, running_mean, running_var, name='fwd', **self._kwargs)
 
 
@@ -178,6 +180,14 @@
         return x + shortcut
 
 
+def _mark_tee_tails(features):
+    blocks = [b for stage in features._children.values() if isinstance(stage, nn.HybridSequential)
+              for b in stage._children.values() if hasattr(b, 'tail')]
+    for prev, nxt in zip(blocks, blocks[1:]):
+        if getattr(nxt, '_tee', False) and prev.tail._fuse_add:
+            prev.tail._defer_apply = True
+
+
 class _ResNetBase(HybridBlock):
     def _stage(self, block, n, channels, stride, index, in_channels, layout, fuse):
         stage = nn.HybridSequential(prefix='stage%d_' % index)
@@ -206,6 +216,8 @@
             for i, n in enumerate(layers):
                 self.features.add(self._stage(block, n, channels[i + 1], 1 if i == 0 else 2, i + 1,
                                               channels[i], layout, fuse))
+            if fuse and layout == 'NHWC':
+                _mark_tee_tails(self.features)
             self.features.add(nn.GlobalAvgPool2D(layout=layout))
             self.output = nn.Dense(classes, in_units=channels[-1])
 
diff --git a/mxnet_maintenance_amd/ndarray/ndarray.py b/mxnet_maintenance_amd/ndarray/ndarray.py
--- a/mxnet_maintenance_amd/ndarray/ndarray.py
+++ b/mxnet_maintenance_amd/ndarray/ndarray.py
@@ -231,6 +231,7 @@
     def asnumpy(self):
         _engine.join_workers()
         self._rethrow()
+        _state.flush_deferred()
         t = self._data.detach()
         idt = getattr(self, '_idt', None)
         if idt is not None:
diff --git a/mxnet_maintenance_amd/ndarray/register.py b/mxnet_maintenance_amd/ndarray/register.py
--- a/mxnet_maintenance_amd/ndarray/register.py
+++ b/mxnet_maintenance_amd/ndarray/register.py
@@ -178,6 +178,8 @@
 
 def invoke(op, inputs, attrs, out=None):
     tin = [None if x is None else x._data for x in inputs]
+    if _state.TAIL_FLUSH[0] is not None:
+        _state.flush_deferred(op.name)
     if _engine._JOIN_HOOKS and not _engine._workers.depth:
         _engine.run_join_hooks()
     _note_leaves(inputs)
diff --git a/mxnet_maintenance_amd/ops/hip_ops.py b/mxnet_maintenance_amd/ops/hip_ops.py
--- a/mxnet_maintenance_amd/ops/hip_ops.py
+++ b/mxnet_maintenance_amd/ops/hip_ops.py
@@ -4,6 +4,7 @@
 import torch.nn.functional as F
 
 from ..base import MXNetError
+from .. import _state
 from . import kernels as _K
 
 _ALLOW_FALLBACK = os.environ.get('MXAMD_ALLOW_TORCH_FALLBACK', '0') == '1'
@@ -112,6 +113,7 @@
 def conv_tee(data, weight, inplace_grad=False):
     if _use_hip(data) and hasattr(_K, 'ConvTeeNHWC') and _K.conv_tee_ok(data, weight):
         return _K.ConvTeeNHWC.apply(data, weight, bool(inplace_grad))
+    _state.flush_deferred()
     return conv(data, weight, None, (1, 1), (0, 0), (1, 1), 1, True), data
 
 
@@ -129,7 +131,7 @@
 
 
 def batch_norm(data, gamma, beta, moving_mean, moving_var, eps, momentum, fix_gamma, training,
-               axis, act_type, addend=None, invstd_out=False):
+               axis, act_type, addend=None, invstd_out=False, defer=False):
     nd = data.dim()
     axis = axis % nd
     channel_last = (axis == nd - 1) and nd > 2
@@ -143,7 +145,7 @@
             return out.permute(0, 3, 1, 2), m, v
     if channel_last and _use_hip(data) and _K.bn_ok(data):
         return _K.BatchNormNHWC.apply(data, g, beta, addend, eps, training, act_type == 'relu',
-                                      moving_mean, moving_var, momentum, invstd_out)
+                                      moving_mean, moving_var, momentum, invstd_out, None, bool(defer))
     if channel_last:
         x = _nd_to_ncx(data)
     elif axis != 1:
diff --git a/mxnet_maintenance_amd/ops/kernel_fns.py b/mxnet_maintenance_amd/ops/kernel_fns.py
--- a/mxnet_maintenance_amd/ops/kernel_fns.py
+++ b/mxnet_maintenance_amd/ops/kernel_fns.py
@@ -73,11 +73,56 @@
         self.lazy = None
 
 
+class _TailFwd:
+    __slots__ = ('y', 'z', 'addend', 'scale', 'shift', 'mask', 'version')
+
+    def __init__(self, y, z, addend, scale, shift, mask):
+        self.y, self.z, self.addend, self.scale, self.shift, self.mask = y, z, addend, scale, shift, mask
+        self.version = y._version
+
+
+_TAIL_PENDING = [None]
+_TAIL_FUSED = [0]
+
+
+def _tail_materialize(tok):
+    C = tok.z.shape[-1]
+    _K.lib().bn_nhwc_forward(_DT[tok.z.dtype], tok.z.data_ptr(), tok.addend.data_ptr(), tok.y.data_ptr(),
+                             tok.mask.data_ptr(), 0, 0, 0, 0, 0, 0, 0, tok.scale.data_ptr(), tok.shift.data_ptr(),
+                             tok.z.numel() // C, C, 0.0, 0, 1, 0, 0.0, 0, 0, 0, _stream())
+
+
+def _set_pending(tok):
+    _TAIL_PENDING[0] = tok
+    _state.TAIL_FLUSH[0] = flush_tail if tok is not None else None
+
+
+def flush_tail():
+    tok = _TAIL_PENDING[0]
+    if tok is not None:
+        _set_pending(None)
+        tok.y._mxamd_tail_fwd = None
+        _tail_materialize(tok)
+
+
+def _take_tail(x):
+    tok = _TAIL_PENDING[0]
+    if tok is None:
+        return None
+    if tok.y is x and getattr(x, '_mxamd_tail_fwd', None) is tok and x._version == tok.version:
+        _set_pending(None)
+        x._mxamd_tail_fwd = None
+        return tok
+    flush_tail()
+    return None
+
+
 class BatchNormNHWC(torch.autograd.Function):
 
     @staticmethod
     def forward(ctx, x, gamma, beta, addend, eps, training, relu, moving_mean, moving_var, momentum=None,
-                invstd_out=False, pool=None):
+                invstd_out=False, pool=None, defer=False):
+        flush_tail()
         lib = _K.lib()
         C = x.shape[-1]
         R = x.numel() // C
@@ -113,7 +158,10 @@
                and moving_var.is_contiguous())
         mask = (torch.empty(x.numel() // 8, dtype=torch.uint8, device=dev)
                 if (addend is not None and relu and _RELU_FROM_X[0]) else None)
-        lib.bn_nhwc_forward(_DT[x.dtype], x.data_ptr(), _p(addend), _p(y), _p(mask), g.data_ptr(),
+        defer = bool(defer and training and mask is not None and pool is None and x.is_contiguous()
+                     and x.dtype in (torch.float16, torch.bfloat16) and hasattr(lib, 'conv_pw_stream_tail_ok'))
+        lib.bn_nhwc_forward(_DT[x.dtype], x.data_ptr(), _p(addend), 0 if defer else _p(y),
+                            0 if defer else _p(mask), g.data_ptr(),
                             b.data_ptr(),
                             center.data_ptr(), _p(part), mean.data_ptr(), invstd.data_ptr(), var.data_ptr(),
                             scale.data_ptr(), shift.data_ptr(), R, C, float(eps), int(bool(training)),
@@ -123,6 +171,9 @@
             with torch.no_grad():
                 moving_mean.mul_(momentum).add_(mean.to(moving_mean.dtype), alpha=1 - momentum)
                 moving_var.mul_(momentum).add_(var.to(moving_var.dtype), alpha=1 - momentum)
+        if defer:
+            y._mxamd_tail_fwd = _TailFwd(y, x, addend, scale, shift, mask)
+            _set_pending(y._mxamd_tail_fwd)
         ctx.pool = None
         if pool is not None:
             (kh, kw), (sh, sw), (ph, pw) = pool
@@ -165,7 +216,7 @@
         relu_mode, training, has_add, gdt, bdt = ctx.cfg
         gamma_ref, beta_ref = ctx.refs
         if gy is None:
-            return (None,) * 12
+            return (None,) * 13
         gy = gy.contiguous()
         C = x.shape[-1]
         R = x.numel() // C
@@ -216,9 +267,9 @@
                                  ppart.data_ptr(), dg_ptr, db_ptr, out[2].data_ptr(), N_, H_, W_, C_, Ho_, Wo_, kh, kw,
                                  sh, sw, ph, pw, 0, int(training), accum, _stream())
             if direct:
-                return dx, None, None, None, None, None, None, None, None, None, None, None
+                return dx, None, None, None, None, None, None, None, None, None, None, None, None
             return (dx, out[0].to(gdt) if need_g else None, out[1].to(bdt) if need_b else None,
-                    None, None, None, None, None, None, None, None, None)
+                    None, None, None, None, None, None, None, None, None, None)
         ymask = y if relu_mode == 3 else None
         y = y if relu_mode == 1 else None
         ds = ctx.add_src if dz is not None else None
@@ -257,7 +308,7 @@
         else:
             dgamma = out[0].to(gdt) if need_g else None
             dbeta = out[1].to(bdt) if need_b else None
-        return dx, dgamma, dbeta, dz, None, None, None, None, None, None, None, None
+        return dx, dgamma, dbeta, dz, None, None, None, None, None, None, None, None, None
 
 
 def bnrelu_pool_ok(x, kernel, stride, pad):
@@ -1046,7 +1097,12 @@
             and bool(_K.lib().conv_pw_stream_bnb_ok(int(kin), int(nout), int(bool(add)), int(bn_src[5]))))
 
 
-def conv_pw(x, w2, bn_stats=False, addend=None, bn_bwd=None, addend_mask=None):
+def pw_tail_ok(x, kin, nout):
+    return (pw_ok(x, kin, nout) and hasattr(_K.lib(), 'conv_pw_stream_tail_ok')
+            and bool(_K.lib().conv_pw_stream_tail_ok(int(kin), int(nout), 1)))
+
+
+def conv_pw(x, w2, bn_stats=False, addend=None, bn_bwd=None, addend_mask=None, tail=None):
     C = x.shape[-1]
     K = w2.shape[0]
     M = x.numel() // C
@@ -1060,8 +1116,12 @@
         if tuple(addend.shape) != tuple(y.shape) or addend.dtype != y.dtype or addend.data_ptr() % 16:
             raise ValueError('conv_pw: addend must match the output (shape, dtype, 16-byte alignment)')
     lib = _K.lib()
-    grid = lib.conv_pw_stream_grid(M, C, K, _num_cus(x.device), int(addend is not None or bn_bwd is not None))
-    nparts = grid // max(1, lib.conv_pw_stream_slices(C, K))
+    if tail is not None:
+        grid = lib.conv_pw_stream_tail_grid(M, C, K, _num_cus(x.device))
+        nparts = lib.conv_pw_stream_tail_parts(M, C, K, grid)
+    else:
+        grid = lib.conv_pw_stream_grid(M, C, K, _num_cus(x.device), int(addend is not None or bn_bwd is not None))
+        nparts = grid // max(1, lib.conv_pw_stream_slices(C, K))
     part = torch.empty(2 * K * nparts, dtype=torch.float32, device=x.device) if (bn_stats or bn_bwd) else None
     bkw = {}
     if bn_bwd is not None:
@@ -1074,6 +1134,16 @@
         assert bn_bwd is not None and addend is not None and addend_mask.dtype == torch.uint8
         assert addend_mask.numel() * 8 == addend.numel() and addend_mask.is_contiguous()
         bkw['addend_mask'] = addend_mask.data_ptr()
+    if tail is not None:
+        ta, tb, c0, c1, tmask = tail
+        assert addend is None and bn_bwd is None
+        for t in (ta, tb):
+            assert t.shape == x.shape and t.dtype == x.dtype and t.is_contiguous() and t.data_ptr() % 16 == 0
+        assert tmask.dtype == torch.uint8 and tmask.numel() * 8 == x.numel() and tmask.is_contiguous()
+        bkw.update(pro_mode=1, pro_a=ta.data_ptr(), pro_b=tb.data_ptr(), pro_c0=c0.data_ptr(),
+                   pro_c1=c1.data_ptr(), pro_side=x.data_ptr(), pro_mask=tmask.data_ptr(),
+                   part_len=0 if part is None else part.numel())
+        _TAIL_FUSED[0] += 1
     lib.conv_pw_stream(_DT[x.dtype], x.data_ptr(), w2.data_ptr(), y.data_ptr(), _zero_page(x.device).data_ptr(), M, C,
                        K, _p(part), grid, _stream(), _p(addend), wt, **bkw)
     if bn_bwd is not None:
@@ -1390,6 +1460,7 @@
 
     @staticmethod
     def forward(ctx, x, w, bias, stride, pad, dilate):
+        flush_tail()
         key = ('fwd', tuple(x.shape), tuple(w.shape), tuple(stride), tuple(pad), x.dtype, bias is not None)
         cands = _fwd_candidates(x, w, stride, pad, bias)
         y = _select(key, cands, _fwd_default(x, w, stride), timing=_fwd_timing(cands))
@@ -1434,8 +1505,24 @@
     def forward(ctx, x, w, inplace_grad=False):
         stride, pad = (1, 1), (0, 0)
         key = ('fwd', tuple(x.shape), tuple(w.shape), stride, pad, x.dtype, False)
-        cands = _fwd_candidates(x, w, stride, pad, None)
-        y = _select(key, cands, _fwd_default(x, w, stride), timing=_fwd_timing(cands))
+
+        def plain():
+            cands = _fwd_candidates(x, w, stride, pad, None)
+            return _select(key, cands, _fwd_default(x, w, stride), timing=_fwd_timing(cands))
+        tok = _take_tail(x)
+        if tok is None:
+            y = plain()
+        else:
+            def unfused():
+                _tail_materialize(tok)
+                return plain()
+            tcands = [('apply+conv', unfused)]
+            K, C = w.shape[0], w.shape[3]
+            if pw_tail_ok(x, C, K):
+                tcands.append(('pwtail', lambda: conv_pw(
+                    x, w.reshape(K, C), bn_stats=bool(_state.STATE.training),
+                    tail=(tok.z, tok.addend, tok.scale, tok.shift, tok.mask))))
+            y = _select(('tailfwd', tuple(x.shape), tuple(w.shape), x.dtype), tcands, 'apply+conv')
         ctx.save_for_backward(x, w)
         ctx.w_ref = w
         ctx.inplace_grad = inplace_grad
diff --git a/mxnet_maintenance_amd/ops/nn.py b/mxnet_maintenance_amd/ops/nn.py
--- a/mxnet_maintenance_amd/ops/nn.py
+++ b/mxnet_maintenance_amd/ops/nn.py
@@ -240,13 +240,14 @@
           arg_names=('data', 'addend', 'gamma', 'beta'), aux_names=('moving_mean', 'moving_var'),
           num_outputs=3, num_visible_outputs=_bn_nvis,
           infer_params=lambda s, a: {k + 1: v for k, v in _bn_infer(s, a).items() if k + 1 <= 5 and k > 0},
-          params=_BN_PARAMS)
+          params=dict(_BN_PARAMS, defer_apply=('bool', False)))
 def batch_norm_add_relu(data, addend, gamma, beta, moving_mean, moving_var, eps=1e-3, momentum=0.9,
                         fix_gamma=True, use_global_stats=False, output_mean_var=False, axis=1,
-                        cudnn_off=False, act_type=None, min_calib_range=None, max_calib_range=None):
+                        cudnn_off=False, act_type=None, min_calib_range=None, max_calib_range=None,
+                        defer_apply=False):
     training = _state.STATE.training and not use_global_stats
     return hip_ops.batch_norm(data, gamma, beta, moving_mean, moving_var, eps, momentum, fix_gamma,
-                              training, axis, 'relu', addend=addend)
+                              training, axis, 'relu', addend=addend, defer=bool(defer_apply))
 
 
 
diff --git a/mxnet_maintenance_amd/symbol/symbol.py b/mxnet_maintenance_amd/symbol/symbol.py
--- a/mxnet_maintenance_amd/symbol/symbol.py
+++ b/mxnet_maintenance_amd/symbol/symbol.py
@@ -98,6 +98,8 @@
         return attrs[key[2:-2]]
     return None
 
+
+_UNSERIALISED_ATTRS = ('defer_apply',)
 
 class Symbol:
     __array_priority__ = 1000.0
@@ -465,8 +467,9 @@
         for i, n in enumerate(order):
             d = {'op': 'null' if n.op is None else n.op, 'name': n.name,
                  'inputs': [[index[id(a)], j, 0] for a, j in n.inputs]}
-            if n.attrs:
-                d['attrs'] = {k: str(v) for k, v in n.attrs.items()}
+            attrs = {k: str(v) for k, v in n.attrs.items() if k not in _UNSERIALISED_ATTRS}
+            if attrs:
+                d['attrs'] = attrs
             nodes.append(d)
             if n.op is None:
                 arg_nodes.append(i)
diff --git a/src/kernels/bindings.cc b/src/kernels/bindings.cc
--- a/src/kernels/bindings.cc
+++ b/src/kernels/bindings.cc
@@ -189,8 +189,12 @@
 void conv_pw_stream(int dtype, const void* x, const void* w, void* y, const void* zero, int M, int kin, int nout,
                     float* part, int grid, hipStream_t s, const void* addend, int wt, const void* bn_z,
                     const uint8_t* bn_mask, const float* bn_mean, const float* bn_scale, const float* bn_shift,
-                    int bn_mode, const uint8_t* addend_mask);
+                    int bn_mode, const uint8_t* addend_mask, int pro_mode, const void* pro_a, const void* pro_b,
+                    const float* pro_c0, const float* pro_c1, void* pro_side, uint8_t* pro_mask, int64_t part_len);
+int conv_pw_stream_tail_grid(int M, int kin, int nout, int ncu);
+int conv_pw_stream_tail_parts(int M, int kin, int nout, int grid);
 int conv_pw_stream_bnb_ok(int kin, int nout, int add, int mode);
+int conv_pw_stream_tail_ok(int kin, int nout, int pro_mode);
 void conv_gen(int dtype, int mode, const void* src, const void* wsrc, const float* bias, void* dst, const int* geom,
               int splits, hipStream_t s);
 void rnn_fwd_seq(int dtype, int mode, const float* gx, const void* h0, const float* c0, const void* whh,
@@ -294,18 +298,26 @@
   m.def("conv_pw_stream", [](int dt, uintptr_t x, uintptr_t w, uintptr_t y, uintptr_t zero, int M, int kin, int nout,
                              uintptr_t part, int grid, uintptr_t s, uintptr_t addend, int wt, uintptr_t bn_z,
                              uintptr_t bn_mask, uintptr_t bn_mean, uintptr_t bn_scale, uintptr_t bn_shift, int bn_mode,
-                             uintptr_t addend_mask) {
+                             uintptr_t addend_mask, int pro_mode, uintptr_t pro_a, uintptr_t pro_b, uintptr_t pro_c0,
+                             uintptr_t pro_c1, uintptr_t pro_side, uintptr_t pro_mask, int64_t part_len) {
     conv_pw_stream(dt, P<const void>(x), P<const void>(w), P<void>(y), P<const void>(zero), M, kin, nout,
                    P<float>(part), grid, S(s), P<const void>(addend), wt, P<const void>(bn_z), P<const uint8_t>(bn_mask),
                    P<const float>(bn_mean), P<const float>(bn_scale), P<const float>(bn_shift), bn_mode,
-                   P<const uint8_t>(addend_mask));
+                   P<const uint8_t>(addend_mask), pro_mode, P<const void>(pro_a), P<const void>(pro_b),
+                   P<const float>(pro_c0), P<const float>(pro_c1), P<void>(pro_side), P<uint8_t>(pro_mask), part_len);
     check_launch("conv_pw_stream");
   }, pybind11::arg("dt"), pybind11::arg("x"), pybind11::arg("w"), pybind11::arg("y"), pybind11::arg("zero"),
      pybind11::arg("M"), pybind11::arg("kin"), pybind11::arg("nout"), pybind11::arg("part"), pybind11::arg("grid"),
      pybind11::arg("s"), pybind11::arg("addend"), pybind11::arg("wt") = 0, pybind11::arg("bn_z") = 0,
      pybind11::arg("bn_mask") = 0, pybind11::arg("bn_mean") = 0, pybind11::arg("bn_scale") = 0,
-     pybind11::arg("bn_shift") = 0, pybind11::arg("bn_mode") = 0, pybind11::arg("addend_mask") = 0);
+     pybind11::arg("bn_shift") = 0, pybind11::arg("bn_mode") = 0, pybind11::arg("addend_mask") = 0,
+     pybind11::arg("pro_mode") = 0, pybind11::arg("pro_a") = 0, pybind11::arg("pro_b") = 0, pybind11::arg("pro_c0") = 0,
+     pybind11::arg("pro_c1") = 0, pybind11::arg("pro_side") = 0, pybind11::arg("pro_mask") = 0,
+     pybind11::arg("part_len") = 0);
   m.def("conv_pw_stream_bnb_ok", &conv_pw_stream_bnb_ok);
+  m.def("conv_pw_stream_tail_ok", &conv_pw_stream_tail_ok);
+  m.def("conv_pw_stream_tail_grid", &conv_pw_stream_tail_grid);
+  m.def("conv_pw_stream_tail_parts", &conv_pw_stream_tail_parts);
   m.def("conv_gen", [](int dt, int mode, uintptr_t src, uintptr_t wsrc, uintptr_t bias, uintptr_t dst,
                        std::vector<int> geom, int splits, uintptr_t s) {
     if (geom.size() != 22) throw std::runtime_error("conv_gen: geometry needs 22 ints");
diff --git a/src/kernels/bn_apply.h b/src/kernels/bn_apply.h
--- /dev/null
+++ b/src/kernels/bn_apply.h
@@ -0,0 +1,18 @@
+#pragma once
+
+#include <hip/hip_runtime.h>
+
+#include <cstdint>
+
+namespace mxamd {
+
+template <bool ADD, bool RELU, bool MASK>
+__device__ __forceinline__ float bn_apply_elem(float x, float sc, float sh, float addend, int i, uint32_t& bits) {
+  float r = x * sc + sh;
+  if (ADD) r += addend;
+  if (MASK) bits |= (r > 0.f ? 1u : 0u) << i;
+  if (RELU) r = r > 0.f ? r : 0.f;
+  return r;
+}
+
+}
diff --git a/src/kernels/bn_nhwc.hip b/src/kernels/bn_nhwc.hip
--- a/src/kernels/bn_nhwc.hip
+++ b/src/kernels/bn_nhwc.hip
@@ -3,6 +3,7 @@
 
 #include <algorithm>
 
+#include "bn_apply.h"
 #include "common.h"
 
 namespace mxamd {
@@ -239,11 +240,7 @@
     uint32_t bits = 0;
 #pragma unroll
     for (int i = 0; i < 8; ++i) {
-      float r = vx.get(i) * sc[i] + sh[i];
-      if (ADD) r += va.get(i);
-      if (MASK) bits |= (r > 0.f ? 1u : 0u) << i;
-      if (RELU) r = r > 0.f ? r : 0.f;
-      out.set(i, r);
+      out.set(i, bn_apply_elem<ADD, RELU, MASK>(vx.get(i), sc[i], sh[i], ADD ? va.get(i) : 0.f, i, bits));
     }
     vstore(out, y + vv * 8, nt == 2 ? 2 : 0);
     if (MASK) mask[vv] = static_cast<uint8_t>(bits);
diff --git a/src/kernels/conv_pw.hip b/src/kernels/conv_pw.hip
--- a/src/kernels/conv_pw.hip
+++ b/src/kernels/conv_pw.hip
@@ -1,9 +1,14 @@
 #include <stdexcept>
 
+#include "bn_apply.h"
 #include "common.h"
 #include "mfma.h"
 
 namespace mxamd {
+
+int conv_pw_stream_ok(int kin, int nout);
+int conv_pw_stream_grid(int M, int kin, int nout, int ncu, int add);
+int conv_pw_stream_tail_parts(int M, int kin, int nout, int grid);
 
 namespace {
 
@@ -60,9 +65,24 @@
   const uint8_t* amask;
 };
 
-template <int KIN, int NOUT, int WPC = 2, bool ADD = false, int BNB = kPwBnbNone, bool AMK = false>
+constexpr int kPwProNone = 0;
+constexpr int kPwProTailFwd = 1;
+
+constexpr int kPwTailWalkers = 2;
+
+struct PwProArgs {
+  const void* a;
+  const void* b;
+  const float* c0;
+  const float* c1;
+  void* side;
+  uint8_t* mask;
+};
+
+template <int KIN, int NOUT, int WPC = 2, bool ADD = false, int BNB = kPwBnbNone, bool AMK = false,
+          int PRO = kPwProNone>
 struct PwCfg {
-  static constexpr bool EXT = ADD || BNB != kPwBnbNone;
+  static constexpr bool EXT = ADD || BNB != kPwBnbNone || PRO != kPwProNone;
   static constexpr int BM = pw_bm(KIN, NOUT, EXT);
   static constexpr int WC = NOUT / 16 < 8 ? NOUT / 16 : 8;
   static constexpr int WP = 8 / WC;
@@ -75,7 +95,10 @@
   static constexpr int STAGE_Z = BNB ? BM * NOUT * 2 : 0;
   static constexpr int STAGE_M = BNB == kPwBnbMask ? (BM * NOUT / 8 + 1023) / 1024 * 1024 : 0;
   static constexpr int STAGE_AM = AMK ? (BM * NOUT / 8 + 1023) / 1024 * 1024 : 0;
-  static constexpr int STAGE = STAGE_IN + STAGE_ADD + STAGE_Z + STAGE_M + STAGE_AM;
+  static constexpr int STAGE_P2 = PRO ? BM * ROWB : 0;
+  static constexpr int OFF_P2 = STAGE_IN + STAGE_ADD + STAGE_Z + STAGE_M + STAGE_AM;
+  static constexpr int IMG = PRO ? BM * ROWB : 0;
+  static constexpr int STAGE = STAGE_IN + STAGE_ADD + STAGE_Z + STAGE_M + STAGE_AM + STAGE_P2;
   static constexpr int LPT = STAGE_IN / (512 * 16);
   static constexpr int APT = STAGE_ADD / (512 * 16);
   static constexpr int TI = STAGE_IN / 1024;
@@ -83,17 +106,23 @@
   static constexpr int TZ = STAGE_Z / 1024;
   static constexpr int TM = STAGE_M / 1024;
   static constexpr int TAM = STAGE_AM / 1024;
+  static constexpr int TP2 = STAGE_P2 / 1024;
+  static constexpr int CPR = KIN / 8;
+  static constexpr int RPP = 512 / CPR;
+  static constexpr int NPASS = PRO ? BM / RPP : 0;
+  static constexpr int SO = NPASS * 2;
   static constexpr int PITCH = NOUT * 2 + 16;
   static constexpr int EPI = BM * PITCH;
   static constexpr int OCH = NOUT / 8;
   static constexpr int SPT = (BM * OCH + 511) / 512;
   static constexpr int LDS = WPC == 1 ? 156 * 1024 : 80 * 1024;
   static constexpr int NMAX = EXT ? 6 : 4;
-  static constexpr int NST = (NMAX * STAGE + EPI <= LDS) ? NMAX
-                           : ((NMAX - 1) * STAGE + EPI <= LDS) ? NMAX - 1
-                           : ((NMAX - 2) * STAGE + EPI <= LDS) ? NMAX - 2 : 2;
+  static constexpr int NST = (NMAX * STAGE + EPI + IMG <= LDS) ? NMAX
+                           : ((NMAX - 1) * STAGE + EPI + IMG <= LDS) ? NMAX - 1
+                           : ((NMAX - 2) * STAGE + EPI + IMG <= LDS) ? NMAX - 2
+                           : (PRO && (NMAX - 3) * STAGE + EPI + IMG <= LDS) ? NMAX - 3 : 2;
   static constexpr int D = NST - 1;
-  static constexpr int SMEM = NST * STAGE + EPI;
+  static constexpr int SMEM = NST * STAGE + EPI + IMG;
   static_assert(FC >= 1 && FP >= 1, "at least one fragment pair per wave");
   static_assert(EXT || (LPT >= 1 && STAGE_IN % (512 * 16) == 0), "whole LDS-DMA instructions per tile");
   static_assert(!EXT || (STAGE_IN % 1024 == 0 && STAGE_ADD % 1024 == 0 && STAGE_Z % 1024 == 0),
@@ -102,9 +131,16 @@
   static_assert(BNB != kPwBnbMask || (NOUT / 8) % 16 == 0, "mask rows of whole 16-byte chunks");
   static_assert((BM * OCH) % 512 == 0 || BM * OCH < 512, "whole store rounds, or a single partial one");
   static_assert(512 % OCH == 0, "a thread keeps one output chunk");
-  static_assert(D * ((TI + 7) / 8 + (TA + 7) / 8 + (TZ + 7) / 8 + (TM + 7) / 8 + (TAM + 7) / 8 + SPT) <
+  static_assert(D * ((TI + 7) / 8 + (TA + 7) / 8 + (TZ + 7) / 8 + (TM + 7) / 8 + (TAM + 7) / 8 + (TP2 + 7) / 8 +
+                     SPT + SO) <
                     (EXT ? 40 : 64),
                 "vmcnt range (vm_wait_n covers < 40)");
+  static_assert(!PRO || (WPC == 1 && !ADD && !AMK && BNB == kPwBnbNone),
+                "tail prologue: one workgroup per CU, no other extra stream");
+  static_assert(!PRO || (512 % CPR == 0 && BM % RPP == 0 && NPASS >= 1 && STAGE_P2 % 1024 == 0),
+                "tail prologue: whole transform passes over the tile");
+  static_assert(!PRO || FC * KS * 4 + FC * FP * 4 + 8 * 2 + 16 <= 200,
+                "tail prologue: register budget");
   static_assert(!AMK || (ADD && (NOUT / 8) % 16 == 0), "the addend mask rides with an addend, whole 16-byte rows");
   static_assert(FC * KS * 4 <= (WPC == 1 ? 128 : 64), "resident weights exceed the register budget");
   static_assert(ROWB % 128 == 0, "rows of whole 128-byte swizzle groups");
@@ -143,11 +179,17 @@
   else vm_wait<0>();
 }
 
-template <typename T, int KIN, int NOUT, bool STATS, bool ADD, int WPC, int S, int BNB, bool AMK = false>
+template <typename T, int KIN, int NOUT, bool STATS, bool ADD, int WPC, int S, int BNB, bool AMK = false,
+          int PRO = kPwProNone, typename... PA>
 __global__ void __launch_bounds__(512) __attribute__((amdgpu_waves_per_eu(2 * WPC))) conv_pw_stream_kernel(
     const T* __restrict__ x, const T* __restrict__ w, T* __restrict__ y, const T* __restrict__ zero, int M, int ntiles,
-    float* __restrict__ part, const T* __restrict__ addend, int wt, PwBnb bnb) {
-  using C = PwCfg<KIN, NOUT, WPC, ADD, BNB, AMK>;
+    float* __restrict__ part, const T* __restrict__ addend, int wt, PwBnb bnb, PA... pro_args) {
+  static_assert(sizeof...(PA) == (PRO != kPwProNone ? 1 : 0), "one PwProArgs with a prologue, none without");
+  [[maybe_unused]] const auto pro = [&]() {
+    if constexpr (PRO != kPwProNone) return PwProArgs{pro_args...};
+    else return 0;
+  }();
+  using C = PwCfg<KIN, NOUT, WPC, ADD, BNB, AMK, PRO>;
   constexpr bool EXT = C::EXT;
   extern __shared__ __attribute__((aligned(1024))) char smem[];
   const int tid = threadIdx.x;
@@ -183,7 +225,21 @@
       }
   }
 
+  [[maybe_unused]] float pc0[8], pc1[8];
+  if constexpr (PRO != kPwProNone) {
+    const int ch = (tid % C::CPR) * 8;
+#pragma unroll
+    for (int q = 0; q < 8; ++q) {
+      pc0[q] = pro.c0[ch + q];
+      pc1[q] = pro.c1[ch + q];
+    }
+  }
+
   vm_wait<0>();
+  if constexpr (PRO != kPwProNone) {
+#pragma unroll
+    for (int q = 0; q < 8; ++q) asm volatile("" : "+v"(pc0[q]), "+v"(pc1[q]));
+  }
   if (wt) {
     uint16_t* scr = reinterpret_cast<uint16_t*>(smem + wid * 1280);
 #pragma unroll
@@ -216,10 +272,18 @@
       const int byte = (i * 64 + lane) * 16;
       const int row = byte / C::ROWB;
       const int slot = (byte % C::ROWB) / 16;
-      const int chunk = slot ^ (row & 7);
-      const int p = t * C::BM + row;
-      const T* src = p < M ? x + static_cast<int64_t>(p) * KIN + chunk * 8 : zero + (chunk & 7) * 8;
-      __builtin_amdgcn_global_load_lds((gbl_void*)src, (lds_void*)(sb + i * 1024), 16, 0, 0);
+      if constexpr (PRO != kPwProNone) {
+        const int p = t * C::BM + row;
+        const T* sa = p < M ? static_cast<const T*>(pro.a) + static_cast<int64_t>(p) * KIN + slot * 8 : zero;
+        const T* sb2 = p < M ? static_cast<const T*>(pro.b) + static_cast<int64_t>(p) * KIN + slot * 8 : zero;
+        __builtin_amdgcn_global_load_lds((gbl_void*)sa, (lds_void*)(sb + i * 1024), 16, 0, 0);
+        __builtin_amdgcn_global_load_lds((gbl_void*)sb2, (lds_void*)(sb + C::OFF_P2 + i * 1024), 16, 0, 0);
+      } else {
+        const int chunk = slot ^ (row & 7);
+        const int p = t * C::BM + row;
+        const T* src = p < M ? x + static_cast<int64_t>(p) * KIN + chunk * 8 : zero + (chunk & 7) * 8;
+        __builtin_amdgcn_global_load_lds((gbl_void*)src, (lds_void*)(sb + i * 1024), 16, 0, 0);
+      }
     }
 #pragma unroll
     for (int j = 0; j < (C::TA + 7) / 8; ++j) {
@@ -274,11 +338,20 @@
     }
   };
   const int ops_per_tile = EXT ? (C::TI - wid + 7) / 8 + (C::TA - wid + 7) / 8 + (C::TZ - wid + 7) / 8 +
-                                      (C::TM - wid + 7) / 8 + (C::TAM - wid + 7) / 8
+                                      (C::TM - wid + 7) / 8 + (C::TAM - wid + 7) / 8 +
+                                      (PRO ? (C::TP2 - wid + 7) / 8 : 0)
                                 : C::LPT;
 
-  const int my_tiles = wg < ntiles ? (ntiles - wg + gs - 1) / gs : 0;
-  for (int j = 0; j < C::D && j < my_tiles; ++j) issue(wg + j * gs, j);
+  constexpr bool VW2 = PRO != kPwProNone;
+  [[maybe_unused]] const int nwalk = 2 * gs < ntiles ? 2 * gs : ntiles;
+  [[maybe_unused]] auto tile_vw2 = [&](int i) { return wg + (i & 1) * gs + (i >> 1) * nwalk; };
+  [[maybe_unused]] auto tiles_vw2 = [&]() {
+    const int wb = wg + gs;
+    return (wg < ntiles ? (ntiles - wg + nwalk - 1) / nwalk : 0) +
+           (wb < nwalk && wb < ntiles ? (ntiles - wb + nwalk - 1) / nwalk : 0);
+  };
+  const int my_tiles = VW2 ? tiles_vw2() : wg < ntiles ? (ntiles - wg + gs - 1) / gs : 0;
+  for (int j = 0; j < C::D && j < my_tiles; ++j) issue(VW2 ? tile_vw2(j) : wg + j * gs, j);
 
   float s1[8], s2[8];
 #pragma unroll
@@ -286,8 +359,17 @@
     s1[e] = 0.f;
     s2[e] = 0.f;
   }
+  [[maybe_unused]] float s1b[8], s2b[8];
+  if constexpr (VW2) {
+#pragma unroll
+    for (int e = 0; e < 8; ++e) {
+      s1b[e] = 0.f;
+      s2b[e] = 0.f;
+    }
+  }
   const int my_c8 = tid % C::OCH;
   char* epi = smem + C::NST * C::STAGE;
+  [[maybe_unused]] char* img = epi + C::EPI;
   float bmean[8], bsc[8], bsh[8];
 #pragma unroll
   for (int q = 0; q < 8; ++q) {
@@ -298,10 +380,10 @@
   }
 
   for (int it = 0; it < my_tiles; ++it) {
-    const int t = wg + it * gs;
+    const int t = VW2 ? tile_vw2(it) : wg + it * gs;
     const int st = it % C::NST;
     if (!EXT) {
-      if (it + C::D < my_tiles) issue(wg + (it + C::D) * gs, (it + C::D) % C::NST);
+      if (it + C::D < my_tiles) issue(VW2 ? tile_vw2(it + C::D) : wg + (it + C::D) * gs, (it + C::D) % C::NST);
       const int later = (my_tiles - 1 - it) < C::D ? (my_tiles - 1 - it) : C::D;
       const int epis = it < C::D ? it : C::D;
       if (later == C::D && epis == C::D) vm_wait<C::D*(C::LPT + C::SPT)>();
@@ -310,12 +392,39 @@
     } else {
       const int later = (my_tiles - 1 - it) < C::D - 1 ? (my_tiles - 1 - it) : C::D - 1;
       const int epis = it < C::D ? it : C::D;
-      vm_wait_n(later * ops_per_tile + epis * C::SPT);
+      vm_wait_n(later * ops_per_tile + epis * (C::SPT + C::SO));
       lds_barrier();
-      if (it + C::D < my_tiles) issue(wg + (it + C::D) * gs, (it + C::D) % C::NST);
+      if (it + C::D < my_tiles) issue(VW2 ? tile_vw2(it + C::D) : wg + (it + C::D) * gs, (it + C::D) % C::NST);
     }
 
     const char* sb = smem + st * C::STAGE;
+    if constexpr (PRO != kPwProNone) {
+      const __amdgpu_buffer_rsrc_t srs = __builtin_amdgcn_make_buffer_rsrc(
+          pro.side, 0, static_cast<int>(static_cast<uint32_t>(M) * KIN * sizeof(T)), 0x00020000);
+      const __amdgpu_buffer_rsrc_t mrs = __builtin_amdgcn_make_buffer_rsrc(
+          pro.mask, 0, static_cast<int>(static_cast<uint32_t>(M) * C::CPR), 0x00020000);
+      const int chunk = tid % C::CPR;
+#pragma unroll
+      for (int k = 0; k < C::NPASS; ++k) {
+        const int row = tid / C::CPR + k * C::RPP;
+        const int p = t * C::BM + row;
+        Vec8<T> va, vb, out;
+        va.raw = *reinterpret_cast<const uint4*>(sb + row * C::ROWB + chunk * 16);
+        vb.raw = *reinterpret_cast<const uint4*>(sb + C::OFF_P2 + row * C::ROWB + chunk * 16);
+        uint32_t bits = 0;
+#pragma unroll
+        for (int q = 0; q < 8; ++q)
+          out.set(q, bn_apply_elem<true, true, true>(va.get(q), pc0[q], pc1[q], vb.get(q), q, bits));
+        const bool live = p < M;
+        const uint32_t off = live ? (static_cast<uint32_t>(p) * KIN + chunk * 8) * sizeof(T) : 0xFFFFFFF0u;
+        __builtin_amdgcn_raw_buffer_store_b128(__builtin_bit_cast(u32x4, out.raw), srs, off, 0, 0);
+        __builtin_amdgcn_raw_buffer_store_b8(static_cast<uint8_t>(bits), mrs,
+                                             live ? static_cast<uint32_t>(p) * C::CPR + chunk : 0xFFFFFFF0u, 0, 0);
+        *reinterpret_cast<uint4*>(img + row * C::ROWB + ((chunk ^ (row & 7)) * 16)) = out.raw;
+      }
+      lds_barrier();
+    }
+    const char* mb_src = PRO != kPwProNone ? img : sb;
     f4_t acc[C::FC][C::FP];
 #pragma unroll
     for (int f = 0; f < C::FC; ++f)
@@ -328,7 +437,7 @@
       for (int p = 0; p < C::FP; ++p) {
         const int row = wp * C::FP * 16 + p * 16 + (lane & 15);
         const int chunk = s * 4 + (lane >> 4);
-        bf[p] = *reinterpret_cast<const u32x4*>(sb + row * C::ROWB + ((chunk ^ (row & 7)) * 16));
+        bf[p] = *reinterpret_cast<const u32x4*>(mb_src + row * C::ROWB + ((chunk ^ (row & 7)) * 16));
       }
 #pragma unroll
       for (int f = 0; f < C::FC; ++f)
@@ -393,12 +502,22 @@
       }
       const uint32_t off = live ? (static_cast<uint32_t>(p) * NT + slice * NOUT + c8 * 8) * sizeof(T) : 0xFFFFFFF0u;
       __builtin_amdgcn_raw_buffer_store_b128(__builtin_bit_cast(u32x4, v.raw), yrs, off, 0, 0);
-      if (STATS && live) {
+      if (STATS && live && !(VW2 && (it & 1))) {
 #pragma unroll
         for (int q = 0; q < 8; ++q) {
           const float z = v.get(q);
           s1[q] += z;
           s2[q] += z * z;
+        }
+      }
+      if constexpr (VW2) {
+        if (STATS && live && (it & 1)) {
+#pragma unroll
+          for (int q = 0; q < 8; ++q) {
+            const float z = v.get(q);
+            s1b[q] += z;
+            s2b[q] += z * z;
+          }
         }
       }
     }
@@ -420,9 +539,51 @@
       const float* col = red + which * ROWS * NOUT + ch;
       float a = 0.f;
       for (int r = 0; r < ROWS; ++r) a += col[r * NOUT];
-      part[static_cast<int64_t>(which) * NT * gs + static_cast<int64_t>(slice * NOUT + ch) * gs + wg] = a;
-    }
-  }
+      part[static_cast<int64_t>(which) * NT * (VW2 ? nwalk : gs) +
+           static_cast<int64_t>(slice * NOUT + ch) * (VW2 ? nwalk : gs) + wg] = a;
+    }
+    if constexpr (VW2) {
+      if (wg + gs < nwalk) {
+        lds_barrier();
+#pragma unroll
+        for (int q = 0; q < 8; ++q) {
+          red[(tid / C::OCH) * NOUT + my_c8 * 8 + q] = s1b[q];
+          red[ROWS * NOUT + (tid / C::OCH) * NOUT + my_c8 * 8 + q] = s2b[q];
+        }
+        lds_barrier();
+        for (int qq = tid; qq < 2 * NOUT; qq += 512) {
+          const int which = qq / NOUT, ch = qq - which * NOUT;
+          const float* col = red + which * ROWS * NOUT + ch;
+          float a = 0.f;
+          for (int r = 0; r < ROWS; ++r) a += col[r * NOUT];
+          part[static_cast<int64_t>(which) * NT * nwalk + static_cast<int64_t>(ch) * nwalk + wg + gs] = a;
+        }
+      }
+    }
+  }
+}
+
+template <typename T, int KIN, int NOUT, bool STATS, int PRO>
+void launch_pw_tail(const void* w, void* y, const void* zero, int M, float* part, int grid, hipStream_t s, int wt,
+                    const PwProArgs& pro) {
+  constexpr int BNB = kPwBnbNone;
+  using C = PwCfg<KIN, NOUT, 1, false, BNB, false, PRO>;
+  static_assert(C::SMEM <= C::LDS && C::NST >= 2, "LDS budget / ring depth");
+  static_assert(C::BM == pw_bm(KIN, NOUT, false), "the tile height of the launch without a prologue");
+  MXAMD_HOST_CHECK(conv_pw_stream_ok(KIN, NOUT) == kPwTailWalkers,
+                   "conv_pw_stream: tail prologue walkers per workgroup must match the plain launch's workgroups per CU");
+  static bool set = false;
+  if (!set) {
+    hipFuncSetAttribute(
+        reinterpret_cast<const void*>(
+            &conv_pw_stream_kernel<T, KIN, NOUT, STATS, false, 1, 1, BNB, false, PRO, PwProArgs>),
+        hipFuncAttributeMaxDynamicSharedMemorySize, C::SMEM);
+    set = true;
+  }
+  const int ntiles = (M + C::BM - 1) / C::BM;
+  hipLaunchKernelGGL((conv_pw_stream_kernel<T, KIN, NOUT, STATS, false, 1, 1, BNB, false, PRO, PwProArgs>), dim3(grid),
+                     dim3(512), C::SMEM, s, static_cast<const T*>(nullptr), static_cast<const T*>(w), static_cast<T*>(y),
+                     static_cast<const T*>(zero), M, ntiles, part, static_cast<const T*>(nullptr), wt, PwBnb{}, pro);
 }
 
 template <typename T, int KIN, int NOUT, int WPC, int S, bool STATS, bool ADD, int BNB = kPwBnbNone, bool AMK = false>
@@ -443,6 +604,26 @@
                      static_cast<const T*>(zero), M, ntiles, part, static_cast<const T*>(addend), wt, bnb);
 }
 
+#define MXAMD_PW_TAILFWD_SHAPES(X) X(256, 64) X(256, 128)
+
+template <typename T>
+bool dispatch_pw_pro(int pro_mode, int kin, int nout, const void* w, void* y, const void* zero, int M, float* part,
+                     int grid, hipStream_t s, int wt, const PwProArgs& pro) {
+  if (pro_mode == kPwProTailFwd) {
+#define MXAMD_PW_CASE(K, N)                                                                                        \
+  if (kin == K && nout == N) {                                                                                     \
+    if (part)                                                                                                      \
+      launch_pw_tail<T, K, N, true, kPwProTailFwd>(w, y, zero, M, part, grid, s, wt, pro);                         \
+    else                                                                                                           \
+      launch_pw_tail<T, K, N, false, kPwProTailFwd>(w, y, zero, M, part, grid, s, wt, pro);                        \
+    return true;                                                                                                   \
+  }
+    MXAMD_PW_TAILFWD_SHAPES(MXAMD_PW_CASE)
+#undef MXAMD_PW_CASE
+  }
+  return false;
+}
+
 template <int KIN, int NOUT>
 constexpr bool pw_bnb_built(bool add, int mode) {
   return add ? (mode == kPwBnbMask && (NOUT / 8) % 16 == 0) : mode == kPwBnbFromZ;
@@ -533,6 +714,29 @@
   return 0;
 }
 
+int conv_pw_stream_tail_ok(int kin, int nout, int pro_mode) {
+#define MXAMD_PW_TOK(K, N) \
+  if (kin == K && nout == N) return 1;
+  if (pro_mode == kPwProTailFwd) {
+    MXAMD_PW_TAILFWD_SHAPES(MXAMD_PW_TOK)
+  }
+#undef MXAMD_PW_TOK
+  return 0;
+}
+
+int conv_pw_stream_tail_grid(int M, int kin, int nout, int ncu) {
+  const int walkers = conv_pw_stream_grid(M, kin, nout, ncu, 0);
+  return (walkers + kPwTailWalkers - 1) / kPwTailWalkers;
+}
+
+int conv_pw_stream_tail_parts(int M, int kin, int nout, int grid) {
+  if (!conv_pw_stream_tail_ok(kin, nout, kPwProTailFwd) || grid < 1) return 0;
+  const int bm = pw_bm(kin, nout, true);
+  const int ntiles = (M + bm - 1) / bm;
+  if (grid > ntiles) return 0;
+  return kPwTailWalkers * grid < ntiles ? kPwTailWalkers * grid : ntiles;
+}
+
 int conv_pw_stream_grid(int M, int kin, int nout, int ncu, int add) {
   const int sl = conv_pw_stream_slices(kin, nout);
   if (sl == 0) return 0;
@@ -547,8 +751,26 @@
 void conv_pw_stream(int dtype, const void* x, const void* w, void* y, const void* zero, int M, int kin, int nout,
                     float* part, int grid, hipStream_t s, const void* addend, int wt, const void* bn_z,
                     const uint8_t* bn_mask, const float* bn_mean, const float* bn_scale, const float* bn_shift,
-                    int bn_mode, const uint8_t* addend_mask) {
+                    int bn_mode, const uint8_t* addend_mask, int pro_mode, const void* pro_a, const void* pro_b,
+                    const float* pro_c0, const float* pro_c1, void* pro_side, uint8_t* pro_mask, int64_t part_len) {
   MXAMD_HOST_CHECK(conv_pw_stream_ok(kin, nout), "conv_pw_stream: unsupported (Cin, Cout)");
+  if (pro_mode != kPwProNone) {
+    MXAMD_HOST_CHECK(conv_pw_stream_tail_ok(kin, nout, pro_mode), "conv_pw_stream: tail prologue not built for (Cin, Cout)");
+    MXAMD_HOST_CHECK((int64_t)M * nout * 2 < (1ll << 31) - 64 && (int64_t)M * kin * 2 < (1ll << 31) - 64,
+                     "conv_pw_stream: tensor too large for 32-bit offsets");
+    MXAMD_HOST_CHECK(part_len == (part ? 2ll * nout * conv_pw_stream_tail_parts(M, kin, nout, grid) : 0),
+                     "conv_pw_stream: tail prologue statistics buffer must hold conv_pw_stream_tail_parts partials");
+    MXAMD_HOST_CHECK(pro_a && pro_b && pro_c0 && pro_c1 && pro_side && pro_mask && !addend && !addend_mask && !bn_z,
+                     "conv_pw_stream: tail prologue needs its operands, coefficients, side output and mask; no addend, "
+                     "no BN-backward statistics");
+    const PwProArgs pa{pro_a, pro_b, pro_c0, pro_c1, pro_side, pro_mask};
+    bool okp = false;
+    if (dtype == kF16) okp = dispatch_pw_pro<__half>(pro_mode, kin, nout, w, y, zero, M, part, grid, s, wt, pa);
+    else if (dtype == kBF16)
+      okp = dispatch_pw_pro<__hip_bfloat16>(pro_mode, kin, nout, w, y, zero, M, part, grid, s, wt, pa);
+    MXAMD_HOST_CHECK(okp, "conv_pw_stream: tail prologue needs f16 or bf16");
+    return;
+  }
   MXAMD_HOST_CHECK(grid >= 1 && grid % conv_pw_stream_slices(kin, nout) == 0 &&
                    (int64_t)M * nout * 2 < (1ll << 31) - 64 && (int64_t)M * kin < (1ll << 31),
                    "conv_pw_stream: tensor too large for 32-bit offsets");
```

After: 12490 images/sec, median of 6. +1.4%, better.
